# caesar-one/audio-classification-using-a-deep-cnn-combined-with-multi-level-attention

Measured on AMD Instinct MI355X. Metric: 0.96 s clips/sec wave->logits (VGGish+attn), higher is better.
Workload: dtype bf16; 1 GPU; BASELINE config 3: wave->logits forward, 1024 bags x 10 s 16 kHz PCM per GPU = 10240 x 0.96 s clips per step, VGGish + MLA [2,1], random-init portable-seeded weights; f32 front-end/head, bf16 conv+FC; bags_per_gpu=1024, parallelism=dp1 (no collective: independent bags)

## Files before the change

### audio-classification-using-a-deep-cnn-combined-with-multi-level-attention_amd/_lib.py

```python

import ctypes
import os
import re

HERE = os.path.dirname(os.path.abspath(__file__))
LIB_PATH = os.environ.get("MLA_HIP_LIB") or os.path.join(HERE, "libmla_hip.so")
HEADER = os.path.join(os.path.dirname(HERE), "include", "mla_hip.h")

F32, BF16, I16, BF16X3, F64, I32, U8, I24 = 0, 1, 2, 3, 4, 5, 6, 7
E_SHORT = -3

_lib = None


class MlaError(RuntimeError):
    def __init__(self, code, msg):
        super().__init__("libmla_hip error %d: %s" % (code, msg))
        self.code = code


def declared_symbols():
    text = open(HEADER).read()
    text = re.sub(r"/\*.*?\*/", "", text, flags=re.S)
    return sorted(set(re.findall(r"\b(mla_[a-z0-9_]+)\s*\(", text)))


def lib():
    global _lib
    if _lib is None:
        if not os.path.exists(LIB_PATH):
            raise RuntimeError(
                "%s is missing: build it with `python __graft_entry__.py` (hipcc --offload-arch=gfx950). "
                "There is no fallback path." % LIB_PATH)
        import torch
        L = ctypes.CDLL(LIB_PATH)
        L.mla_last_error.restype = ctypes.c_char_p
        L.mla_logmel_table_floats.restype = ctypes.c_int64
        i64, vp, ci = ctypes.c_int64, ctypes.c_void_p, ctypes.c_int
        L.mla_logmel_counts.argtypes = [i64, ctypes.POINTER(i64), ctypes.POINTER(i64)]
        L.mla_logmel_build_tables.argtypes = [vp]
        L.mla_logmel_reference_tables.argtypes = [vp, vp]
        L.mla_logmel_examples.argtypes = [vp, ci, i64, i64, i64, vp, vp, ci, vp]
        L.mla_logmel_conv1.argtypes = [vp, ci, i64, i64, i64, vp, vp, vp, vp, vp]
        L.mla_logmel_bags.argtypes = [vp, ci, i64, i64, i64, vp, vp, ci, ci, vp, vp, ci, vp]
        L.mla_timeline_counts.argtypes = [i64, i64, ctypes.POINTER(i64), ctypes.POINTER(i64), ctypes.POINTER(i64)]
        L.mla_logmel_timeline.argtypes = [vp, ci, i64, i64, i64, vp, vp, i64, vp, vp, ci, vp]
        L.mla_gather_bags.argtypes = [vp, i64, i64, vp, vp, i64, ci, i64, vp, vp]
        cf = ctypes.c_float
        L.mla_stft_magnitude.argtypes = [vp, i64, vp, vp, i64, i64, i64, vp, vp]
        L.mla_mel_log.argtypes = [vp, vp, i64, i64, i64, cf, vp, vp]
        L.mla_dataset_frames.argtypes = [vp, i64, ci, ci, ci, ci, vp, vp]
        L.mla_melspec_frames.restype = i64
        L.mla_melspec_frames.argtypes = [i64, i64]
        L.mla_melspec_table_floats.restype = i64
        L.mla_melspec_table_floats.argtypes = [ctypes.c_double, i64]
        L.mla_melspec_build_tables.argtypes = [ctypes.c_double, i64, vp]
        L.mla_melspec_workspace_bytes.restype = i64
        L.mla_melspec_workspace_bytes.argtypes = [i64, i64, i64]
        L.mla_melspec_db.argtypes = [vp, i64, i64, i64, i64, i64, cf, vp, vp, vp, vp]
        L.mla_melspec_images.argtypes = [vp, vp, i64, i64, i64, i64, cf, i64, i64, i64, vp, vp]
        L.mla_melspec_track_counts.argtypes = [i64, i64] + [ctypes.POINTER(i64)] * 4
        L.mla_melspec_track_db.argtypes = [vp, i64, i64, i64, vp, vp, i64, cf, vp, vp, vp, vp, vp]
        L.mla_melspec_track_images.argtypes = [vp, vp, i64, vp, vp, i64, cf, i64, i64, vp, vp]
        cd = ctypes.c_double
        L.mla_melspec_band_table_floats.restype = i64
        L.mla_melspec_band_table_floats.argtypes = [cd, i64, cd, cd, ci]
        L.mla_melspec_build_band_tables.argtypes = [cd, i64, cd, cd, ci, vp]
        L.mla_melspec_nopad_frames.restype = i64
        L.mla_melspec_nopad_frames.argtypes = [i64, i64]
        L.mla_melspec_nopad_workspace_bytes.restype = i64
        L.mla_melspec_nopad_workspace_bytes.argtypes = [i64, i64, i64]
        L.mla_melspec_nopad_db.argtypes = [vp, i64, i64, i64, i64, i64, cf, vp, i64, vp, vp, vp]
        L.mla_melspec_nopad_bags.argtypes = [vp, vp, i64, i64, i64, i64, cf, i64, i64, i64, vp, ci, vp]
        L.mla_postprocess.argtypes = [vp, vp, vp, i64, vp, vp]
        L.mla_mono_mix.argtypes = [vp, ci, i64, ci, vp, vp]
        L.mla_split_bf16x3.argtypes = [vp, i64, i64, i64, vp, i64, i64, ci, vp]
        L.mla_merge_bf16x3.argtypes = [vp, i64, i64, i64, i64, vp, vp]
        L.mla_linear_bf16x3.argtypes = [vp, i64, vp, i64, vp, vp, i64, i64, i64, i64, i64, ci, ci, vp]
        L.mla_conv_repack_weights.argtypes = [vp, i64, i64, vp, ci, vp]
        L.mla_convert_f32.argtypes = [vp, vp, i64, ci, vp]
        L.mla_convert_bf16_to_f32.argtypes = [vp, vp, i64, vp]
        L.mla_vggish_conv1.argtypes = [vp, ci, i64, vp, vp, vp, ci, vp]
        L.mla_vggish_conv.argtypes = [ci, vp, vp, vp, vp, i64, ci, vp]
        L.mla_linear.argtypes = [vp, i64, vp, i64, vp, vp, i64, i64, i64, i64, ci, ci, ci, vp]
        L.mla_linear_small.argtypes = [vp, i64, vp, i64, vp, vp, i64, i64, i64, i64, vp]
        L.mla_linear_narrow.argtypes = [vp, i64, vp, i64, vp, vp, i64, i64, i64, i64, vp]
        L.mla_linear_splitk.argtypes = [vp, i64, vp, i64, vp, vp, i64, i64, i64, i64, ci, ci, vp, i64, vp]
        L.mla_linear_ksplit.argtypes = [vp, i64, vp, i64, vp, vp, i64, i64, i64, i64, ci, ci, ci, ci, vp, i64, vp]
        L.mla_bn_stats_workspace_bytes.restype = i64
        L.mla_bn_stats.argtypes = [vp, i64, i64, i64, ci, ci, vp, vp, vp, vp, vp, cf, vp]
        L.mla_bn_apply.argtypes = [vp, i64, vp, i64, i64, i64, ci, ci, vp, vp, vp, vp, cf, ci, vp, cf, vp]
        L.mla_attention_pool.argtypes = [vp, i64, ci, ci, vp, vp, vp, vp, vp, vp, vp, vp, cf, vp, i64, vp, vp, vp]
        cd = ctypes.c_double
        L.mla_bn_stats_sums.argtypes = [vp, i64, i64, i64, ci, ci, vp, vp, vp]
        L.mla_bn_stats_finish.argtypes = [vp, ci, cd, vp, vp, vp, vp, cf, vp, vp]
        L.mla_bn_stats_fused.argtypes = [vp, i64, i64, i64, ci, ci, vp, vp, vp, vp, vp, vp, cf, vp, vp]
        L.mla_bn_bwd_sums.argtypes = [vp, i64, vp, i64, vp, i64, ci, cf, i64, i64, ci, ci, vp, vp, cf, vp, vp, vp]
        L.mla_bn_bwd_apply.argtypes = [vp, i64, vp, i64, vp, i64, ci, cf, i64, i64, ci, ci, vp, vp, vp, cf, vp, vp, cd,
                                       vp, i64, ci, vp, vp, vp]
        L.mla_bn_bwd_sums_wide.argtypes = [vp, i64, vp, i64, vp, i64, ci, cf, i64, i64, vp, vp, cf, vp, vp, vp]
        L.mla_bn_bwd_apply_wide.argtypes = [vp, i64, vp, i64, vp, i64, ci, cf, i64, i64, vp, vp, vp, cf, vp, vp, cd,
                                            vp, i64, ci, vp, vp, vp]
        L.mla_attention_pool_bwd.argtypes = [vp, i64, vp, vp, i64, ci, ci, vp, vp, vp]
        L.mla_linear_small_bwd.argtypes = [vp, i64, vp, i64, vp, i64, i64, i64, i64, vp, i64, vp, vp, vp]
        L.mla_transpose_f32.argtypes = [vp, i64, vp, i64, i64, i64, vp]
        L.mla_col_sum.argtypes = [vp, i64, i64, i64, vp, vp, vp]
        L.mla_axpy.argtypes = [cf, vp, vp, i64, vp]
        L.mla_cross_entropy.argtypes = [vp, i64, vp, i64, ci, cf, vp, vp, i64, vp, vp]
        L.mla_adam_step.argtypes = [vp, vp, vp, vp, i64, cf, cf, cf, cf, i64, vp]
        L.mla_conv3x3.argtypes = [vp, vp, vp, vp, i64, ci, ci, ci, ci, ci, ci, ci, vp]
        L.mla_conv3x3_train.argtypes = [vp, vp, vp, vp, vp, i64, ci, ci, ci, ci, ci, vp]
        L.mla_conv_repack_dgrad.argtypes = [vp, i64, i64, vp, vp]
        L.mla_maxpool2x2.argtypes = [vp, vp, i64, ci, ci, ci, vp]
        L.mla_relu_pool_bwd.argtypes = [vp, vp, vp, i64, ci, ci, ci, ci, vp]
        L.mla_relu_pool_bwd_bias.argtypes = [vp, vp, vp, i64, ci, ci, ci, ci, vp, vp, vp]
        L.mla_relu_pool_bwd_bias_workspace_bytes.restype = ctypes.c_int64
        L.mla_conv_wgrad_workspace_floats.restype = i64
        L.mla_conv_wgrad.argtypes = [vp, vp, i64, ci, ci, ci, ci, vp, i64, vp, vp]
        L.mla_conv1_bwd.argtypes = [vp, vp, vp, vp, i64, vp, vp, vp, vp]
        L.mla_conv_repack_dgrad_bf16.argtypes = [vp, i64, i64, vp, vp]
        L.mla_maxpool2x2_bf16.argtypes = [vp, vp, i64, ci, ci, ci, vp]
        L.mla_relu_pool_bwd_bf16_workspace_bytes.restype = i64
        L.mla_relu_pool_bwd_bf16.argtypes = [vp, ci, vp, ci, vp, i64, ci, ci, ci, ci, vp, vp, vp]
        L.mla_conv_wgrad_bf16.argtypes = [vp, vp, i64, ci, ci, ci, ci, vp, i64, vp, vp]
        L.mla_conv1_bwd_bf16.argtypes = [vp, vp, vp, vp, i64, vp, vp, vp, vp]
        L.mla_conv3x3_train_codes.argtypes = [vp, vp, vp, vp, vp, i64, ci, ci, ci, ci, ci, vp]
        L.mla_pool_bwd_codes_bf16.argtypes = [vp, vp, vp, i64, ci, ci, ci, vp, vp, vp]
        L.mla_conv1_bwd_workspace_floats.argtypes = []
        L.mla_conv1_bwd_workspace_floats.restype = i64
        L.mla_conv1_dgrad.argtypes = [vp, vp, vp, vp, ci, i64, vp, vp]
        L.mla_transpose_bf16.argtypes = [vp, i64, vp, i64, i64, i64, vp]
        L.mla_col_sum_bf16.argtypes = [vp, i64, i64, i64, vp, vp, vp]
        L.mla_resample_length.restype = i64
        L.mla_resample_length.argtypes = [i64, cd, cd]
        L.mla_resample.argtypes = [vp, i64, cd, cd, vp, vp, ci, ci, vp, i64, vp]
        L.mla_clips_lds_bytes.restype = i64
        L.mla_clips_lds_bytes.argtypes = [vp, i64, cd, ci, ci]
        L.mla_clips_prepare.argtypes = [vp, ci, i64, i64, vp, vp, vp, vp, vp, vp, vp, vp, vp, vp, cd, i64, vp, i64, ci, ci, vp, vp]
        L.mla_clips_prepare_raw.argtypes = [vp, i64, i64, vp, vp, vp, vp, vp, vp, vp, vp, vp, vp, vp, vp, cd, i64, vp, i64, ci, ci, vp, vp]
        u64 = ctypes.c_uint64
        L.mla_dropout_mask.argtypes = [vp, i64, u64, u64, u64, cf, vp]
        L.mla_dropout_mask_dev.argtypes = [vp, i64, u64, u64, vp, u64, cf, vp]
        L.mla_adam_step_dev.argtypes = [vp, vp, vp, vp, i64, cf, cf, cf, vp, vp]
        L.mla_adam_prepare.argtypes = [vp, cf, cf, cf, i64, vp]
        L.mla_counter_add.argtypes = [vp, i64, vp]
        L.mla_comm_unique_id.argtypes = [vp]
        L.mla_comm_init_rank.argtypes = [ctypes.POINTER(vp), ci, vp, ci]
        L.mla_comm_destroy.argtypes = [vp]
        L.mla_comm_count.argtypes = [vp, ctypes.POINTER(ci)]
        L.mla_comm_library_origin.restype = ctypes.c_char_p
        L.mla_allreduce_flat.argtypes = [vp, i64, ci, vp, vp]
        L.mla_rn_repack.argtypes = [vp, i64, i64, i64, vp, ci, vp]
        L.mla_rn_stem.argtypes = [vp, i64, i64, i64, ci, vp, vp, vp, ci, vp, ci, vp]
        L.mla_rn_conv.argtypes = [vp, i64, i64, i64, i64, vp, i64, i64, i64, vp, vp, vp, ci, vp, ci, vp]
        L.mla_rn_bn_workspace_bytes.restype = i64
        L.mla_rn_bn_workspace_bytes.argtypes = [i64]
        L.mla_rn_bn_stats.argtypes = [vp, i64, i64, ci, vp, vp, vp, cf, cf, vp, vp, vp, vp, vp, vp, vp]
        L.mla_rn_bn_sums.argtypes = [vp, i64, i64, ci, vp, vp, vp]
        L.mla_rn_bn_finish.argtypes = [vp, i64, vp, vp, cf, cf, vp, vp, vp, vp, vp, vp, vp]
        L.mla_rn_bn_eval_coeffs.argtypes = [vp, vp, vp, vp, cf, i64, vp, vp, vp]
        L.mla_rn_bn_apply.argtypes = [vp, i64, i64, vp, vp, vp, ci, vp, ci, vp]
        L.mla_rn_maxpool.argtypes = [vp, i64, i64, i64, i64, vp, ci, vp]
        L.mla_rn_avgpool.argtypes = [vp, i64, i64, i64, vp, ci, vp]
        L.mla_rn_repack_dgrad.argtypes = [vp, i64, i64, i64, vp, ci, vp]
        L.mla_rn_conv_dgrad.argtypes = [vp, i64, i64, i64, i64, vp, i64, i64, i64, i64, i64, vp, vp, ci, vp]
        L.mla_rn_conv_wgrad_workspace_floats.restype = i64
        L.mla_rn_conv_wgrad_workspace_floats.argtypes = [i64, i64, i64, i64, i64, i64, ci]
        L.mla_rn_conv_wgrad.argtypes = [vp, vp, i64, i64, i64, i64, i64, i64, i64, vp, i64, vp, ci, vp]
        L.mla_rn_stem_wgrad_workspace_floats.restype = i64
        L.mla_rn_stem_wgrad_workspace_floats.argtypes = [i64]
        L.mla_rn_stem_wgrad.argtypes = [vp, i64, ci, vp, vp, i64, vp, ci, vp]
        L.mla_rn_bn_bwd_workspace_bytes.restype = i64
        L.mla_rn_bn_bwd_workspace_bytes.argtypes = [i64]
        L.mla_rn_bn_bwd.argtypes = [vp, vp, vp, i64, i64, vp, vp, vp, cf, vp, vp, vp, vp, vp, ci, vp]
        L.mla_rn_bn_bwd_sums.argtypes = [vp, vp, vp, i64, i64, vp, vp, cf, vp, vp, vp, vp, ci, vp]
        L.mla_rn_bn_bwd_apply.argtypes = [vp, vp, vp, i64, i64, vp, vp, vp, cf, vp, vp, vp, vp, ci, vp]
        L.mla_rn_maxpool_bwd.argtypes = [vp, vp, i64, i64, i64, i64, vp, ci, vp]
        L.mla_rn_avgpool_bwd.argtypes = [vp, i64, i64, i64, vp, ci, vp]
        L.mla_rn_act_bwd.argtypes = [vp, vp, vp, i64, i64, vp, vp, ci, vp]
        L.mla_rn_stem_dgrad.argtypes = [vp, i64, vp, vp, vp, ci, vp, ci, vp]
        _lib = L
    return _lib


def check(rc):
    if rc != 0:
        raise MlaError(rc, lib().mla_last_error().decode("utf-8", "replace"))


def stream_ptr():
    import torch
    return ctypes.c_void_p(torch.cuda.current_stream().cuda_stream)
```

### audio-classification-using-a-deep-cnn-combined-with-multi-level-attention_amd/csrc/gemm.hip

```cpp
#include <type_traits>

#include "common.h"
#include "mma_core.h"

namespace {

using namespace mma;

constexpr int kThreads = 512;

#ifndef MLA_GEMM_STAMPS
#define MLA_GEMM_STAMPS 0
#endif
#if MLA_GEMM_STAMPS
__device__ unsigned long long g_gemm_stamps[8][2][8];
#define MLA_GSTAMP(k) do { if (stamp_on) stamps[k] = __builtin_amdgcn_s_memtime(); } while (0)
#else
#define MLA_GSTAMP(k) do { } while (0)
#endif
#ifndef MLA_GEMM_PRIO
#define MLA_GEMM_PRIO 3
#endif
#ifndef MLA_GEMM_STAGGER
#define MLA_GEMM_STAGGER 1
#endif

#ifndef MLA_GEMM_TILE320
#define MLA_GEMM_TILE320 1
#endif
#ifndef MLA_GEMM_RING
#define MLA_GEMM_RING 1
#endif
#ifdef MLA_GEMM_KWRAP
#define MLA_GEMM_KW(s) ((s) & (MLA_GEMM_KWRAP - 1))
#else
#define MLA_GEMM_KW(s) (s)
#endif
template <typename T, typename TO, int MS, int NS, bool RELU, bool DMA = false>
__global__ __launch_bounds__(kThreads, 2) void gemm_kernel(const T* __restrict__ A, int64_t lda,
                                                            const T* __restrict__ W, int64_t ldw,
                                                            const float* __restrict__ bias, TO* __restrict__ out,
                                                            int64_t ldo, int M, int N, int K, float* __restrict__ partial,
                                                            int seg, int osplit) {
    constexpr int PER = Elem<T>::kPerChunk, KC = Elem<T>::kPerRow;
    constexpr int kMS = MS, kBM = 2 * MS * 16;
    constexpr int BN = 4 * NS * 16;
    constexpr int A_BYTES = kBM * kRowBytes, B_BYTES = BN * kRowBytes;
    constexpr int AP = kBM * 8 / kThreads;
    extern __shared__ __attribute__((aligned(16))) char smem[];
    char* sA = smem;
    char* sB = smem + 2 * A_BYTES;

    const int t = threadIdx.x, lane = t & 63, wave = t >> 6, wm = wave >> 2, wn = wave & 3;
    const int r = lane & 15, q = lane >> 4;
    const int m0 = blockIdx.x * kBM, n0 = blockIdx.y * BN;
    const int abase = tile_off(wm * kMS * 16 + r, q);
    const int bbase = tile_off(wn * NS * 16 + r, q);

    f32x4 acc[kMS][NS];
    _Pragma("unroll") for (int i = 0; i < kMS; ++i)
        _Pragma("unroll") for (int j = 0; j < NS; ++j) acc[i][j] = f32x4{0.f, 0.f, 0.f, 0.f};

    constexpr uint32_t ESZ = sizeof(T);
    const int a_rows = M - m0 < kBM ? M - m0 : kBM, w_rows = N - n0 < BN ? N - n0 : BN;
    const __amdgpu_buffer_rsrc_t ra = __builtin_amdgcn_make_buffer_rsrc(const_cast<T*>(A) + size_t(m0) * lda, 0,
                                                                          uint32_t(a_rows) * uint32_t(lda) * ESZ, 0x00020000);
    const __amdgpu_buffer_rsrc_t rw = __builtin_amdgcn_make_buffer_rsrc(const_cast<T*>(W) + size_t(n0) * ldw, 0,
                                                                          uint32_t(w_rows) * uint32_t(ldw) * ESZ, 0x00020000);
    u32x4 areg[AP], breg[NS];
    auto gload = [&](int s) {
        int sa = s;
        if (seg) {
            const int blk = s / (3 * seg), rr = s - blk * 3 * seg;
            sa = blk * 2 * seg + (rr < seg ? rr : rr - seg);
        }
        _Pragma("unroll") for (int p = 0; p < AP; ++p) {
            const int piece = t + kThreads * p, row = piece >> 3, ch = piece & 7;
            const int k = sa * KC + ch * PER;
            const bool ok = m0 + row < M && s * KC + ch * PER < K;
            areg[p] = __builtin_amdgcn_raw_buffer_load_b128(ra, ok ? int((uint32_t(row) * uint32_t(lda) + k) * sizeof(T)) : int(0x7fffff00), 0, 0);
        }
        _Pragma("unroll") for (int p = 0; p < NS; ++p) {
            const int piece = t + kThreads * p, n = piece >> 3, ch = piece & 7;
            const int k = s * KC + ch * PER;
            const bool ok = n0 + n < N && k < K;
            breg[p] = __builtin_amdgcn_raw_buffer_load_b128(rw, ok ? int((uint32_t(n) * uint32_t(ldw) + k) * sizeof(T)) : int(0x7fffff00), 0, 0);
        }
    };
    auto lwrite = [&](int buf) {
        _Pragma("unroll") for (int p = 0; p < AP; ++p) {
            const int piece = t + kThreads * p;
            lds_write16(sA, buf * A_BYTES + tile_off(piece >> 3, piece & 7), areg[p]);
        }
        _Pragma("unroll") for (int p = 0; p < NS; ++p) {
            const int piece = t + kThreads * p;
            lds_write16(sB, buf * B_BYTES + tile_off(piece >> 3, piece & 7), breg[p]);
        }
    };

    auto dma = [&](int s, int buf) {
        int sa = s;
        if (seg) {
            const int blk = s / (3 * seg), rr = s - blk * 3 * seg;
            sa = blk * 2 * seg + (rr < seg ? rr : rr - seg);
        }
        const int slot = lane & 7;
        _Pragma("unroll") for (int p = 0; p < kBM / 64; ++p) {
            const int row = 8 * (wave + 8 * p) + (lane >> 3);
            const int chunk = slot ^ (((row >> 1) & 3) << 1);
            __builtin_amdgcn_raw_ptr_buffer_load_lds(ra, (__attribute__((address_space(3))) void*)(sA + buf * A_BYTES + 8 * (wave + 8 * p) * kRowBytes),
                                                     16, int((uint32_t(row) * uint32_t(lda) + chunk * PER) * ESZ), int(MLA_GEMM_KW(sa) * KC * ESZ), 0, 0);
        }
        _Pragma("unroll") for (int p = 0; p < BN / 64; ++p) {
            const int row = 8 * (wave + 8 * p) + (lane >> 3);
            const int chunk = slot ^ (((row >> 1) & 3) << 1);
            __builtin_amdgcn_raw_ptr_buffer_load_lds(rw, (__attribute__((address_space(3))) void*)(sB + buf * B_BYTES + 8 * (wave + 8 * p) * kRowBytes),
                                                     16, int((uint32_t(row) * uint32_t(ldw) + chunk * PER) * ESZ), int(MLA_GEMM_KW(s) * KC * ESZ), 0, 0);
        }
    };

    const int all_stages = (K + KC - 1) / KC;
    const int per_split = (all_stages + int(gridDim.z) - 1) / int(gridDim.z);
    const int s_begin = int(blockIdx.z) * per_split;
    const int stages = (s_begin + per_split < all_stages ? s_begin + per_split : all_stages);
    if (DMA) {
        dma(s_begin, s_begin & 1);
        asm volatile("s_waitcnt vmcnt(0)" ::: "memory");
    } else {
        gload(s_begin);
        lwrite(s_begin & 1);
    }
    __syncthreads();
    constexpr bool STAGGER = DMA && MLA_GEMM_STAGGER;
    const bool late = STAGGER && __builtin_amdgcn_readfirstlane(wave) >= 4;
    if (STAGGER && late) __builtin_amdgcn_s_setprio(1);
#if MLA_GEMM_STAMPS
    unsigned long long stamps[8] = {0, 0, 0, 0, 0, 0, 0, 0};
#endif
    auto run = [&](auto late_c) {
        constexpr bool LATE = decltype(late_c)::value;
        u32x4 af[kMS], bf[NS];
        for (int s = s_begin; s < stages; ++s) {
            const int buf = s & 1;
#if MLA_GEMM_STAMPS
            const bool stamp_on = s == 100 && (wave == 0 || wave == 4) && blockIdx.x < 8 && blockIdx.y == 0 && kMS == 8;
#endif
            auto stage_next = [&]() {
                if (s + 1 < stages) {
                    if (DMA) dma(s + 1, buf ^ 1);
                    else gload(s + 1);
                }
            };
            auto rd = [&](int ks) {
                _Pragma("unroll") for (int i = 0; i < kMS; ++i)
                    af[i] = lds_read16(sA, buf * A_BYTES + (abase ^ (ks << 6)) + i * 16 * kRowBytes);
                _Pragma("unroll") for (int j = 0; j < NS; ++j)
                    bf[j] = lds_read16(sB, buf * B_BYTES + (bbase ^ (ks << 6)) + j * 16 * kRowBytes);
            };
            auto mm = [&]() {
                __builtin_amdgcn_sched_barrier(0);
                _Pragma("unroll") for (int i = 0; i < kMS; ++i)
                    _Pragma("unroll") for (int j = 0; j < NS; ++j) mma_step<T>(af[i], bf[j], acc[i][j]);
                __builtin_amdgcn_sched_barrier(0);
            };
            if constexpr (!LATE) {
                if (STAGGER && MLA_GEMM_PRIO == 3) __builtin_amdgcn_s_setprio(2);
                MLA_GSTAMP(0);
                rd(0);
                MLA_GSTAMP(1);
                stage_next();
                MLA_GSTAMP(2);
                mm();
                MLA_GSTAMP(3);
                if (STAGGER && MLA_GEMM_PRIO == 3) __builtin_amdgcn_s_setprio(0);
                rd(1);
                MLA_GSTAMP(4);
                mm();
                MLA_GSTAMP(5);
            } else {
                if (MLA_GEMM_PRIO == 3) __builtin_amdgcn_s_setprio(3);
                MLA_GSTAMP(0);
                if (s > s_begin) mm();
                MLA_GSTAMP(1);
                stage_next();
                MLA_GSTAMP(2);
                if (MLA_GEMM_PRIO == 3) __builtin_amdgcn_s_setprio(1);
                rd(0); mm();
                MLA_GSTAMP(3);
                rd(1);
                MLA_GSTAMP(4);
                asm volatile("s_waitcnt lgkmcnt(0)" ::: "memory");
                MLA_GSTAMP(5);
            }
            if (!DMA && s + 1 < stages) lwrite(buf ^ 1);
            if (DMA) asm volatile("s_waitcnt vmcnt(0)" ::: "memory");
            MLA_GSTAMP(6);
            __syncthreads();
            MLA_GSTAMP(7);
        }
        if constexpr (LATE) {
            if (stages > s_begin) {
                __builtin_amdgcn_sched_barrier(0);
                _Pragma("unroll") for (int i = 0; i < kMS; ++i)
                    _Pragma("unroll") for (int j = 0; j < NS; ++j) mma_step<T>(af[i], bf[j], acc[i][j]);
                __builtin_amdgcn_sched_barrier(0);
            }
        }
    };
    if constexpr (STAGGER) {
        if (late) run(std::true_type{});
        else run(std::false_type{});
    } else {
        run(std::false_type{});
    }

#if MLA_GEMM_STAMPS
    if ((wave == 0 || wave == 4) && lane == 0 && blockIdx.x < 8 && blockIdx.y == 0 && kMS == 8 && stages > 100)
        for (int k = 0; k < 8; ++k) g_gemm_stamps[blockIdx.x][wave >> 2][k] = stamps[k];
#endif
    if (partial) {
        float* pout = partial + size_t(blockIdx.z) * M * N;
        _Pragma("unroll") for (int j = 0; j < NS; ++j) {
            const int n = n0 + (wn * NS + j) * 16 + r;
            if (n >= N) continue;
            _Pragma("unroll") for (int i = 0; i < kMS; ++i) {
                const float v[4] = {acc[i][j].x, acc[i][j].y, acc[i][j].z, acc[i][j].w};
                _Pragma("unroll") for (int e = 0; e < 4; ++e) {
                    const int m = m0 + (wm * kMS + i) * 16 + 4 * q + e;
                    if (m < M) pout[size_t(m) * N + n] = v[e];
                }
            }
        }
        return;
    }
    _Pragma("unroll") for (int j = 0; j < NS; ++j) {
        const int n = n0 + (wn * NS + j) * 16 + r;
        if (n >= N) continue;
        const float b = bias ? bias[n] : 0.f;
        _Pragma("unroll") for (int i = 0; i < kMS; ++i) {
            const float v[4] = {acc[i][j].x, acc[i][j].y, acc[i][j].z, acc[i][j].w};
            _Pragma("unroll") for (int e = 0; e < 4; ++e) {
                const int m = m0 + (wm * kMS + i) * 16 + 4 * q + e;
                if (m < M) {
                    float y = v[e] + b;
                    if (RELU) y = mla::nan_relu(y);
                    if (sizeof(TO) == 2 && osplit) {
                        const float hi = bf2f(f2bf(y));
                        store_elem<TO>(out + size_t(m) * ldo + n, hi);
                        store_elem<TO>(out + size_t(m) * ldo + N + n, y - hi);
                    } else {
                        store_elem<TO>(out + size_t(m) * ldo + n, y);
                    }
                }
            }
        }
    }
}

template <typename T, typename TO, bool RELU>
__global__ __launch_bounds__(kThreads, 2) void gemm_ring_kernel(const T* __restrict__ A, int64_t lda, const T* __restrict__ W,
                                                                 int64_t ldw, const float* __restrict__ bias, TO* __restrict__ out,
                                                                 int64_t ldo, int M, int N, int K, float* __restrict__ partial, int seg,
                                                                 int osplit) {
    constexpr int PER = Elem<T>::kPerChunk, KC = Elem<T>::kPerRow;
    constexpr int kMS = 4, NS = 2, kBM = 128, BN = 128, RING = 4;
    constexpr int A_BYTES = kBM * kRowBytes, B_BYTES = BN * kRowBytes, STAGE_BYTES = A_BYTES + B_BYTES;
    extern __shared__ __attribute__((aligned(16))) char smem[];

    const int t = threadIdx.x, lane = t & 63, wave = t >> 6, wm = wave >> 2, wn = wave & 3;
    const int r = lane & 15, q = lane >> 4;
    int bx = blockIdx.x, by = blockIdx.y;
    if (gridDim.y % 8 == 0) {
        const int id = blockIdx.x + gridDim.x * blockIdx.y, per = gridDim.y / 8, j = id >> 3;
        by = (id & 7) * per + j % per;
        bx = j / per;
    }
    const int m0 = bx * kBM, n0 = by * BN;
    const int abase = tile_off(wm * kMS * 16 + r, q);
    const int bbase = tile_off(wn * NS * 16 + r, q);

    f32x4 acc[kMS][NS];
    _Pragma("unroll") for (int i = 0; i < kMS; ++i)
        _Pragma("unroll") for (int j = 0; j < NS; ++j) acc[i][j] = f32x4{0.f, 0.f, 0.f, 0.f};

    constexpr uint32_t ESZ = sizeof(T);
    const int a_rows = M - m0 < kBM ? M - m0 : kBM, w_rows = N - n0 < BN ? N - n0 : BN;
    const __amdgpu_buffer_rsrc_t ra = __builtin_amdgcn_make_buffer_rsrc(const_cast<T*>(A) + size_t(m0) * lda, 0,
                                                                          uint32_t(a_rows) * uint32_t(lda) * ESZ, 0x00020000);
    const __amdgpu_buffer_rsrc_t rw = __builtin_amdgcn_make_buffer_rsrc(const_cast<T*>(W) + size_t(n0) * ldw, 0,
                                                                          uint32_t(w_rows) * uint32_t(ldw) * ESZ, 0x00020000);
    auto dma = [&](int s, int buf) {
        int sa = s;
        if (seg) {
            const int blk = s / (3 * seg), rr = s - blk * 3 * seg;
            sa = blk * 2 * seg + (rr < seg ? rr : rr - seg);
        }
        char* sA = smem + buf * STAGE_BYTES;
        char* sB = sA + A_BYTES;
        const int slot = lane & 7;
        _Pragma("unroll") for (int p = 0; p < 2; ++p) {
            const int row = 8 * (wave + 8 * p) + (lane >> 3);
            const int chunk = slot ^ (((row >> 1) & 3) << 1);
            __builtin_amdgcn_raw_ptr_buffer_load_lds(ra, (__attribute__((address_space(3))) void*)(sA + 8 * (wave + 8 * p) * kRowBytes), 16,
                                                     int((uint32_t(row) * uint32_t(lda) + chunk * PER) * ESZ), int(sa * KC * ESZ), 0, 0);
        }
        _Pragma("unroll") for (int p = 0; p < 2; ++p) {
            const int row = 8 * (wave + 8 * p) + (lane >> 3);
            const int chunk = slot ^ (((row >> 1) & 3) << 1);
            __builtin_amdgcn_raw_ptr_buffer_load_lds(rw, (__attribute__((address_space(3))) void*)(sB + 8 * (wave + 8 * p) * kRowBytes), 16,
                                                     int((uint32_t(row) * uint32_t(ldw) + chunk * PER) * ESZ), int(s * KC * ESZ), 0, 0);
        }
    };

    const int all_stages = K / KC;
    const int per_split = (all_stages + int(gridDim.z) - 1) / int(gridDim.z);
    const int s_begin = int(blockIdx.z) * per_split;
    const int s_end = s_begin + per_split < all_stages ? s_begin + per_split : all_stages;
    _Pragma("unroll") for (int p = 0; p < RING - 1; ++p)
        if (s_begin + p < s_end) dma(s_begin + p, p);
    for (int s = s_begin; s < s_end; ++s) {
        const int left = s_end - 1 - s;
        if (left >= 2) asm volatile("s_waitcnt vmcnt(8)" ::: "memory");
        else if (left == 1) asm volatile("s_waitcnt vmcnt(4)" ::: "memory");
        else asm volatile("s_waitcnt vmcnt(0)" ::: "memory");
        __syncthreads();
        if (s + RING - 1 < s_end) dma(s + RING - 1, (s - s_begin + RING - 1) % RING);
        const char* sA = smem + ((s - s_begin) % RING) * STAGE_BYTES;
        const char* sB = sA + A_BYTES;
        _Pragma("unroll") for (int ks = 0; ks < 2; ++ks) {
            u32x4 af[kMS], bf[NS];
            _Pragma("unroll") for (int i = 0; i < kMS; ++i) af[i] = lds_read16(sA, (abase ^ (ks << 6)) + i * 16 * kRowBytes);
            _Pragma("unroll") for (int j = 0; j < NS; ++j) bf[j] = lds_read16(sB, (bbase ^ (ks << 6)) + j * 16 * kRowBytes);
            _Pragma("unroll") for (int i = 0; i < kMS; ++i)
                _Pragma("unroll") for (int j = 0; j < NS; ++j) mma_step<T>(af[i], bf[j], acc[i][j]);
        }
    }

    if (partial) {
        float* pout = partial + size_t(blockIdx.z) * M * N;
        _Pragma("unroll") for (int j = 0; j < NS; ++j) {
            const int n = n0 + (wn * NS + j) * 16 + r;
            if (n >= N) continue;
            _Pragma("unroll") for (int i = 0; i < kMS; ++i) {
                const float v[4] = {acc[i][j].x, acc[i][j].y, acc[i][j].z, acc[i][j].w};
                _Pragma("unroll") for (int e = 0; e < 4; ++e) {
                    const int m = m0 + (wm * kMS + i) * 16 + 4 * q + e;
                    if (m < M) pout[size_t(m) * N + n] = v[e];
                }
            }
        }
        return;
    }
    _Pragma("unroll") for (int j = 0; j < NS; ++j) {
        const int n = n0 + (wn * NS + j) * 16 + r;
        if (n >= N) continue;
        const float b = bias ? bias[n] : 0.f;
        _Pragma("unroll") for (int i = 0; i < kMS; ++i) {
            const float v[4] = {acc[i][j].x, acc[i][j].y, acc[i][j].z, acc[i][j].w};
            _Pragma("unroll") for (int e = 0; e < 4; ++e) {
                const int m = m0 + (wm * kMS + i) * 16 + 4 * q + e;
                if (m < M) {
                    float y = v[e] + b;
                    if (RELU) y = mla::nan_relu(y);
                    if (sizeof(TO) == 2 && osplit) {
                        const float hi = bf2f(f2bf(y));
                        store_elem<TO>(out + size_t(m) * ldo + n, hi);
                        store_elem<TO>(out + size_t(m) * ldo + N + n, y - hi);
                    } else {
                        store_elem<TO>(out + size_t(m) * ldo + n, y);
                    }
                }
            }
        }
    }
}

template <typename TO>
__global__ __launch_bounds__(256) void splitk_reduce_kernel(const float* __restrict__ partial, int splits, int64_t M, int N,
                                                            const float* __restrict__ bias, int relu, TO* __restrict__ out, int64_t ldo) {
    const int64_t total = M * N;
    for (int64_t i = int64_t(blockIdx.x) * 256 + threadIdx.x; i < total; i += int64_t(gridDim.x) * 256) {
        const int64_t m = i / N;
        const int n = int(i - m * N);
        float v = bias ? bias[n] : 0.f;
        for (int k = 0; k < splits; ++k) v += partial[size_t(k) * total + i];
        if (relu) v = mla::nan_relu(v);
        store_elem<TO>(out + m * ldo + n, v);
    }
}

template <typename T, typename TO, int MS, int NS, bool RELU>
int launch(const void* a, int64_t lda, const void* w, int64_t ldw, const float* bias, void* out, int64_t ldo,
           int64_t M, int64_t N, int64_t K, hipStream_t s, int splits = 1, float* partial = nullptr, int seg = 0, int osplit = 0) {
    constexpr int kBM = 2 * MS * 16, BN = 4 * NS * 16;
    constexpr int lds = 2 * (kBM + BN) * kRowBytes;
    constexpr int KCE = mma::Elem<T>::kPerRow;
    MLA_REQUIRE(uint64_t(kBM) * uint64_t(lda) * sizeof(T) < (1ull << 31) && uint64_t(BN) * uint64_t(ldw) * sizeof(T) < (1ull << 31), MLA_E_SHAPE,
                "GEMM row pitch too large for 32-bit buffer offsets (lda %lld, ldw %lld)", (long long)lda, (long long)ldw);
    const bool use_dma = K % KCE == 0;
    auto kern = use_dma ? gemm_kernel<T, TO, MS, NS, RELU, true> : gemm_kernel<T, TO, MS, NS, RELU, false>;
    MLA_HIP_OK(hipFuncSetAttribute(reinterpret_cast<const void*>(kern), hipFuncAttributeMaxDynamicSharedMemorySize, lds));
    const dim3 grid{unsigned((M + kBM - 1) / kBM), unsigned((N + BN - 1) / BN), unsigned(splits)};
    hipLaunchKernelGGL(kern, grid, dim3(kThreads), lds, s, static_cast<const T*>(a), lda, static_cast<const T*>(w), ldw,
                       bias, static_cast<TO*>(out), ldo, int(M), int(N), int(K), splits > 1 ? partial : nullptr, seg, osplit);
    MLA_LAUNCH_OK("gemm_kernel");
    if (splits > 1) {
        const int64_t total = M * N;
        hipLaunchKernelGGL(splitk_reduce_kernel<TO>, dim3(unsigned((total + 255) / 256 < 4096 ? (total + 255) / 256 : 4096)), dim3(256),
                           0, s, partial, splits, M, int(N), bias, int(RELU), static_cast<TO*>(out), ldo);
        MLA_LAUNCH_OK("splitk_reduce_kernel");
    }
    return MLA_OK;
}

template <typename T, typename TO, bool RELU>
int launch_ring(const void* a, int64_t lda, const void* w, int64_t ldw, const float* bias, void* out, int64_t ldo,
                int64_t M, int64_t N, int64_t K, hipStream_t s, int splits = 1, float* partial = nullptr, int seg = 0, int osplit = 0) {
    constexpr int lds = 4 * (128 + 128) * kRowBytes;
    MLA_REQUIRE(uint64_t(128) * uint64_t(lda) * sizeof(T) < (1ull << 31) && uint64_t(128) * uint64_t(ldw) * sizeof(T) < (1ull << 31), MLA_E_SHAPE,
                "GEMM row pitch too large for 32-bit buffer offsets (lda %lld, ldw %lld)", (long long)lda, (long long)ldw);
    MLA_REQUIRE(K % mma::Elem<T>::kPerRow == 0, MLA_E_SHAPE, "the ring GEMM stages whole %d-element K chunks", mma::Elem<T>::kPerRow);
    auto kern = gemm_ring_kernel<T, TO, RELU>;
    MLA_HIP_OK(hipFuncSetAttribute(reinterpret_cast<const void*>(kern), hipFuncAttributeMaxDynamicSharedMemorySize, lds));
    const dim3 grid{unsigned((M + 127) / 128), unsigned((N + 127) / 128), unsigned(splits)};
    hipLaunchKernelGGL(kern, grid, dim3(kThreads), lds, s, static_cast<const T*>(a), lda, static_cast<const T*>(w), ldw, bias,
                       static_cast<TO*>(out), ldo, int(M), int(N), int(K), splits > 1 ? partial : nullptr, seg, osplit);
    MLA_LAUNCH_OK("gemm_ring_kernel");
    if (splits > 1) {
        const int64_t total = M * N;
        hipLaunchKernelGGL(splitk_reduce_kernel<TO>, dim3(unsigned((total + 255) / 256 < 4096 ? (total + 255) / 256 : 4096)), dim3(256),
                           0, s, partial, splits, M, int(N), bias, int(RELU), static_cast<TO*>(out), ldo);
        MLA_LAUNCH_OK("splitk_reduce_kernel");
    }
    return MLA_OK;
}

template <typename Fn>
int by_relu(bool relu, Fn&& fn) {
    return relu ? fn(std::true_type{}) : fn(std::false_type{});
}

enum class Tile { k64x128, k128x128, kRing, k128x256, k256x256, k320x256 };

template <typename T>
Tile tile_form(int64_t M, int64_t N, int64_t K, int cus, int64_t& m_tall) {
    m_tall = M;
    const bool wide = N > 128 && (N % 256 == 0 || N % 256 > 128);
    const bool tall = wide && M >= 4096 && N >= 1024;
#if MLA_GEMM_TILE320
    if (tall && K % mma::Elem<T>::kPerRow == 0) {
        const int64_t n_tiles = (N + 255) / 256;
        const int64_t t256 = ((M + 255) / 256) * n_tiles, t320 = ((M + 319) / 320) * n_tiles;
        const int64_t full = t256 / cus, rest = t256 - full * cus;
        const double cost256 = 64.0 * double(full) + (rest == 0 ? 0.0 : (full >= 1 && 2 * rest <= cus && (full * cus) % n_tiles == 0 ? 48.0 : 64.0));
        const double cost320 = 72.0 * double((t320 + cus - 1) / cus);
        if (cost320 < cost256) return Tile::k320x256;
    }
#endif
    if (tall) {
        const int64_t n_tiles = (N + 255) / 256, m_tiles = (M + 255) / 256;
        const int64_t full_rounds = m_tiles * n_tiles / cus, rest = m_tiles * n_tiles - full_rounds * cus;
        if (full_rounds >= 1 && rest > 0 && 2 * rest <= cus && (full_rounds * cus) % n_tiles == 0) m_tall = full_rounds * cus / n_tiles * 256;
        return Tile::k256x256;
    }
    if (wide) {
        if (((M + 127) / 128) * ((N + 255) / 256) * 2 <= cus) {
#if MLA_GEMM_RING
            if (K % mma::Elem<T>::kPerRow == 0 && K / mma::Elem<T>::kPerRow >= 8)
                return Tile::kRing;
#endif
            return Tile::k128x128;
        }
        return Tile::k128x256;
    }
    if (((M + 127) / 128) * ((N + 127) / 128) < cus && M > 64)
        return Tile::k64x128;
    return Tile::k128x128;
}

template <typename T, typename TO>
int dispatch(const void* a, int64_t lda, const void* w, int64_t ldw, const float* bias, void* out, int64_t ldo,
             int64_t M, int64_t N, int64_t K, bool relu, hipStream_t s, int seg = 0, int osplit = 0) {
    int64_t m_tall;
    const Tile form = tile_form<T>(M, N, K, mla::cu_count(), m_tall);
    return by_relu(relu, [&](auto r) {
        constexpr bool R = decltype(r)::value;
        switch (form) {
            case Tile::k64x128: return launch<T, TO, 2, 2, R>(a, lda, w, ldw, bias, out, ldo, M, N, K, s, 1, nullptr, seg, osplit);
            case Tile::k128x128: return launch<T, TO, 4, 2, R>(a, lda, w, ldw, bias, out, ldo, M, N, K, s, 1, nullptr, seg, osplit);
#if MLA_GEMM_RING
            case Tile::kRing: return launch_ring<T, TO, R>(a, lda, w, ldw, bias, out, ldo, M, N, K, s, 1, nullptr, seg, osplit);
#endif
            case Tile::k128x256: return launch<T, TO, 4, 4, R>(a, lda, w, ldw, bias, out, ldo, M, N, K, s, 1, nullptr, seg, osplit);
#if MLA_GEMM_TILE320
            case Tile::k320x256: return launch<T, TO, 10, 4, R>(a, lda, w, ldw, bias, out, ldo, M, N, K, s, 1, nullptr, seg, osplit);
#endif
            default: break;
        }
        const int rc = launch<T, TO, 8, 4, R>(a, lda, w, ldw, bias, out, ldo, m_tall, N, K, s, 1, nullptr, seg, osplit);
        if (rc != MLA_OK || m_tall == M) return rc;
        const T* a2 = static_cast<const T*>(a) + m_tall * lda;
        TO* out2 = static_cast<TO*>(out) + m_tall * ldo;
        return launch<T, TO, 4, 4, R>(a2, lda, w, ldw, bias, out2, ldo, M - m_tall, N, K, s, 1, nullptr, seg, osplit);
    });
}

}

#if MLA_GEMM_STAMPS
extern "C" int mla_debug_gemm_stamps(unsigned long long* host_out) {
    return hipMemcpyFromSymbol(host_out, HIP_SYMBOL(g_gemm_stamps), sizeof(g_gemm_stamps)) == hipSuccess ? 0 : -4;
}
#endif

extern "C" int mla_linear_splitk(const float* a, int64_t lda, const float* w, int64_t ldw, const float* bias, float* out,
                                 int64_t ldo, int64_t M, int64_t N, int64_t K, int relu, int splits, float* workspace,
                                 int64_t workspace_floats, mla_stream_t stream) {
    MLA_REQUIRE(a && w && out && workspace && M > 0 && N > 0 && K > 0 && splits >= 1 && splits <= 64, MLA_E_ARG, "bad split-K GEMM arguments");
    MLA_REQUIRE(K % 4 == 0 && lda % 4 == 0 && ldw % 4 == 0 && lda >= K && ldw >= K && ldo >= N, MLA_E_SHAPE, "split-K GEMM: 16-byte rows required");
    MLA_REQUIRE(mla::aligned(a, 16) && mla::aligned(w, 16), MLA_E_ARG, "GEMM operands must be 16-byte aligned");
    MLA_REQUIRE(workspace_floats >= int64_t(splits) * M * N, MLA_E_ARG, "split-K workspace too small");
    hipStream_t s = static_cast<hipStream_t>(stream);
    return by_relu(relu != 0, [&](auto r) {
        return launch<float, float, 4, 2, decltype(r)::value>(a, lda, w, ldw, bias, out, ldo, M, N, K, s, splits, workspace);
    });
}

extern "C" int mla_linear_ksplit(const void* a, int64_t lda, const void* w, int64_t ldw, const float* bias, void* out, int64_t ldo,
                                 int64_t M, int64_t N, int64_t K, int dtype, int out_dtype, int relu, int splits, float* workspace,
                                 int64_t workspace_floats, mla_stream_t stream) {
    MLA_REQUIRE(M >= 0 && N > 0 && K > 0 && splits >= 1 && splits <= 64, MLA_E_ARG, "bad K-split GEMM arguments");
    if (M == 0) return MLA_OK;
    MLA_REQUIRE(a && w && out && workspace, MLA_E_ARG, "null GEMM operand");
    MLA_REQUIRE(dtype == MLA_F32 || dtype == MLA_BF16, MLA_E_DTYPE, "GEMM dtype %d", dtype);
    MLA_REQUIRE(out_dtype == MLA_F32 || (out_dtype == MLA_BF16 && dtype == MLA_BF16), MLA_E_DTYPE, "GEMM out dtype %d for compute dtype %d", out_dtype, dtype);
    const int kc = dtype == MLA_F32 ? 32 : 64;
    MLA_REQUIRE(K % (int64_t(kc) * splits) == 0 && lda % (kc / 8) == 0 && ldw % (kc / 8) == 0 && lda >= K && ldw >= K && ldo >= N, MLA_E_SHAPE,
                "K-split GEMM: K %lld must be a multiple of %d x splits %d (whole stages per range)", (long long)K, kc, splits);
    MLA_REQUIRE(mla::aligned(a, 16) && mla::aligned(w, 16), MLA_E_ARG, "GEMM operands must be 16-byte aligned");
    MLA_REQUIRE(workspace_floats >= int64_t(splits) * M * N, MLA_E_ARG, "K-split workspace too small");
    MLA_REQUIRE(M < (1ll << 31) && N < (1ll << 31) && K < (1ll << 31), MLA_E_SHAPE, "GEMM dimension overflow");
    hipStream_t s = static_cast<hipStream_t>(stream);
    const bool r = relu != 0;
    if (dtype == MLA_F32)
        return r ? launch<float, float, 4, 2, true>(a, lda, w, ldw, bias, out, ldo, M, N, K, s, splits, workspace)
                 : launch<float, float, 4, 2, false>(a, lda, w, ldw, bias, out, ldo, M, N, K, s, splits, workspace);
    if (out_dtype == MLA_F32)
        return r ? launch<mma::bf16_t, float, 4, 2, true>(a, lda, w, ldw, bias, out, ldo, M, N, K, s, splits, workspace)
                 : launch<mma::bf16_t, float, 4, 2, false>(a, lda, w, ldw, bias, out, ldo, M, N, K, s, splits, workspace);
    return r ? launch<mma::bf16_t, mma::bf16_t, 4, 2, true>(a, lda, w, ldw, bias, out, ldo, M, N, K, s, splits, workspace)
             : launch<mma::bf16_t, mma::bf16_t, 4, 2, false>(a, lda, w, ldw, bias, out, ldo, M, N, K, s, splits, workspace);
}

extern "C" int mla_linear(const void* a, int64_t lda, const void* w, int64_t ldw, const float* bias, void* out,
                          int64_t ldo, int64_t M, int64_t N, int64_t K, int dtype, int out_dtype, int relu,
                          mla_stream_t stream) {
    MLA_REQUIRE(M >= 0 && N > 0 && K > 0, MLA_E_ARG, "bad GEMM shape %lld x %lld x %lld", (long long)M, (long long)N, (long long)K);
    if (M == 0) return MLA_OK;
    MLA_REQUIRE(a && w && out, MLA_E_ARG, "null GEMM operand");
    MLA_REQUIRE(dtype == MLA_F32 || dtype == MLA_BF16, MLA_E_DTYPE, "GEMM dtype %d", dtype);
    MLA_REQUIRE(out_dtype == MLA_F32 || (out_dtype == MLA_BF16 && dtype == MLA_BF16), MLA_E_DTYPE,
                "GEMM out dtype %d for compute dtype %d", out_dtype, dtype);
    const int per = dtype == MLA_F32 ? 4 : 8;
    MLA_REQUIRE(K % per == 0 && lda % per == 0 && ldw % per == 0 && lda >= K && ldw >= K && ldo >= N, MLA_E_SHAPE,
                "K / lda / ldw must be multiples of %d elements (16-byte rows): K %lld lda %lld ldw %lld ldo %lld", per,
                (long long)K, (long long)lda, (long long)ldw, (long long)ldo);
    MLA_REQUIRE(mla::aligned(a, 16) && mla::aligned(w, 16), MLA_E_ARG, "GEMM operands must be 16-byte aligned");
    MLA_REQUIRE(M < (1ll << 31) && N < (1ll << 31) && K < (1ll << 31), MLA_E_SHAPE, "GEMM dimension overflow");
    hipStream_t s = static_cast<hipStream_t>(stream);
    if (dtype == MLA_F32) return dispatch<float, float>(a, lda, w, ldw, bias, out, ldo, M, N, K, relu != 0, s);
    if (out_dtype == MLA_F32) return dispatch<mma::bf16_t, float>(a, lda, w, ldw, bias, out, ldo, M, N, K, relu != 0, s);
    return dispatch<mma::bf16_t, mma::bf16_t>(a, lda, w, ldw, bias, out, ldo, M, N, K, relu != 0, s);
}

extern "C" int mla_linear_bf16x3(const void* a, int64_t lda, const void* w, int64_t ldw, const float* bias, void* out,
                                 int64_t ldo, int64_t M, int64_t N, int64_t K, int64_t seg, int out_dtype, int relu,
                                 mla_stream_t stream) {
    MLA_REQUIRE(M >= 0 && N > 0 && K > 0, MLA_E_ARG, "bad GEMM shape %lld x %lld x %lld", (long long)M, (long long)N, (long long)K);
    if (M == 0) return MLA_OK;
    MLA_REQUIRE(a && w && out, MLA_E_ARG, "null GEMM operand");
    MLA_REQUIRE(out_dtype == MLA_F32 || out_dtype == MLA_BF16X3, MLA_E_DTYPE, "split GEMM out dtype %d", out_dtype);
    MLA_REQUIRE(seg > 0 && seg % 64 == 0 && K % seg == 0 && lda >= 2 * K && ldw >= 3 * K && lda % 8 == 0 && ldw % 8 == 0 &&
                ldo >= (out_dtype == MLA_F32 ? N : 2 * N), MLA_E_SHAPE,
                "split GEMM: seg %lld must be a multiple of 64 dividing K %lld; lda %lld >= 2K, ldw %lld >= 3K", (long long)seg,
                (long long)K, (long long)lda, (long long)ldw);
    MLA_REQUIRE(mla::aligned(a, 16) && mla::aligned(w, 16), MLA_E_ARG, "GEMM operands must be 16-byte aligned");
    MLA_REQUIRE(M < (1ll << 31) && N < (1ll << 31) && 3 * K < (1ll << 31), MLA_E_SHAPE, "GEMM dimension overflow");
    hipStream_t s = static_cast<hipStream_t>(stream);
    if (out_dtype == MLA_F32)
        return dispatch<mma::bf16_t, float>(a, lda, w, ldw, bias, out, ldo, M, N, 3 * K, relu != 0, s, int(seg / 64), 0);
    return dispatch<mma::bf16_t, mma::bf16_t>(a, lda, w, ldw, bias, out, ldo, M, N, 3 * K, relu != 0, s, int(seg / 64), 1);
}
```

### audio-classification-using-a-deep-cnn-combined-with-multi-level-attention_amd/csrc/mla_head.hip

```cpp
#include "common.h"

namespace {

constexpr int kStatBlocks = 512;
constexpr int kMaxChannels = 64;
constexpr int kMaxWideChannels = 1024;
constexpr int kWideRowBlocks = 32;
constexpr int kMaxSlots = 64;
constexpr int kMaxClasses = 1024;

__device__ __forceinline__ double wave_sum(double v) {
    _Pragma("unroll") for (int o = 32; o > 0; o >>= 1) v += __shfl_xor(v, o);
    return v;
}

__device__ __forceinline__ float sigmoidf(float v) { return 1.f / (1.f + __expf(-v)); }

__device__ __forceinline__ float grad_through_act(float dy, float yout, int act, float drop_scale) {
    if (act == 1) return yout > 0.f ? dy * drop_scale : 0.f;
    if (act == 2) return dy * yout * (1.f - yout);
    return dy;
}

typedef float f32x4_t __attribute__((ext_vector_type(4)));

struct StatsOp {
    const float* x; int64_t ldx;
    __device__ __forceinline__ void operator()(int64_t r, int c, int, double& a, double& b) const {
        const double v = x[r * ldx + c];
        a = v; b = v * v;
    }
    __device__ __forceinline__ void quad(int64_t r, int c, int, double& a, double& b) const {
        const f32x4_t v = *reinterpret_cast<const f32x4_t*>(x + r * ldx + c);
        _Pragma("unroll") for (int e = 0; e < 4; ++e) { const double d = v[e]; a += d; b += d * d; }
    }
    __device__ __forceinline__ bool vec_ok(int cols) const { return cols % 4 == 0 && ldx % 4 == 0 && (reinterpret_cast<uintptr_t>(x) & 15) == 0; }
};

struct BwdOp {
    const float *x, *dy, *yout, *mean, *var;
    int64_t ldx, ld_dy, ld_y;
    int act;
    float drop_scale, eps;
    __device__ __forceinline__ void operator()(int64_t r, int c, int ch, double& a, double& b) const {
        const float g = grad_through_act(dy[r * ld_dy + c], yout ? yout[r * ld_y + c] : 0.f, act, drop_scale);
        const float xhat = (x[r * ldx + c] - mean[ch]) * (1.0f / sqrtf(var[ch] + eps));
        a = g; b = double(g) * xhat;
    }
    __device__ __forceinline__ void quad(int64_t r, int c, int ch, double& a, double& b) const {
        const f32x4_t d = *reinterpret_cast<const f32x4_t*>(dy + r * ld_dy + c);
        const f32x4_t xv = *reinterpret_cast<const f32x4_t*>(x + r * ldx + c);
        f32x4_t y = f32x4_t{0.f, 0.f, 0.f, 0.f};
        if (yout) y = *reinterpret_cast<const f32x4_t*>(yout + r * ld_y + c);
        const float m = mean[ch], inv = 1.0f / sqrtf(var[ch] + eps);
        _Pragma("unroll") for (int e = 0; e < 4; ++e) {
            const float g = grad_through_act(d[e], y[e], act, drop_scale);
            const float xhat = (xv[e] - m) * inv;
            a += g; b += double(g) * xhat;
        }
    }
    __device__ __forceinline__ bool vec_ok(int cols) const {
        return cols % 4 == 0 && ldx % 4 == 0 && ld_dy % 4 == 0 && (!yout || ld_y % 4 == 0) && (reinterpret_cast<uintptr_t>(x) & 15) == 0 &&
               (reinterpret_cast<uintptr_t>(dy) & 15) == 0 && (reinterpret_cast<uintptr_t>(yout) & 15) == 0;
    }
};

template <typename Op>
__global__ __launch_bounds__(256) void sums_rows_kernel(Op op, int64_t rows, int cols, int period, double* __restrict__ partial) {
    __shared__ double part[4][kMaxChannels][2];
    const int wave = threadIdx.x >> 6, lane = threadIdx.x & 63;
    const bool vec = op.vec_ok(cols);
    for (int i = threadIdx.x; i < 4 * kMaxChannels * 2; i += 256) (&part[0][0][0])[i] = 0.0;
    __syncthreads();
    const int64_t per_block = ((rows + gridDim.x - 1) / gridDim.x + period - 1) / period * period;
    const int64_t r0 = int64_t(blockIdx.x) * per_block;
    const int64_t r1 = r0 + per_block < rows ? r0 + per_block : rows;
    for (int64_t r = r0 + wave; r < r1; r += 4) {
        const int chan = int(r % period);
        double s = 0.0, ss = 0.0;
        if (vec) {
            for (int c = 4 * lane; c < cols; c += 256) op.quad(r, c, chan, s, ss);
        } else {
            for (int c = lane; c < cols; c += 64) {
                double a, b;
                op(r, c, chan, a, b);
                s += a;
                ss += b;
            }
        }
        s = wave_sum(s);
        ss = wave_sum(ss);
        if (lane == 0) {
            part[wave][chan][0] += s;
            part[wave][chan][1] += ss;
        }
    }
    __syncthreads();
    if (threadIdx.x < period) {
        double s = 0.0, ss = 0.0;
        for (int w = 0; w < 4; ++w) { s += part[w][threadIdx.x][0]; ss += part[w][threadIdx.x][1]; }
        partial[(int64_t(blockIdx.x) * period + threadIdx.x) * 2] = s;
        partial[(int64_t(blockIdx.x) * period + threadIdx.x) * 2 + 1] = ss;
    }
}

template <typename Op>
__global__ __launch_bounds__(256) void sums_cols_kernel(Op op, int64_t rows, int cols, double* __restrict__ partial) {
    __shared__ double part[256][2];
    const int groups = 256 / cols, g = threadIdx.x / cols, c = threadIdx.x % cols;
    double s = 0.0, ss = 0.0;
    if (g < groups) {
        const int64_t per_block = (rows + gridDim.x - 1) / gridDim.x;
        const int64_t r0 = int64_t(blockIdx.x) * per_block;
        const int64_t r1 = r0 + per_block < rows ? r0 + per_block : rows;
        for (int64_t r = r0 + g; r < r1; r += groups) {
            double a, b;
            op(r, c, c, a, b);
            s += a;
            ss += b;
        }
    }
    part[threadIdx.x][0] = s;
    part[threadIdx.x][1] = ss;
    __syncthreads();
    if (threadIdx.x < cols) {
        double a = 0.0, b = 0.0;
        for (int gg = 0; gg < groups; ++gg) { a += part[gg * cols + threadIdx.x][0]; b += part[gg * cols + threadIdx.x][1]; }
        partial[(int64_t(blockIdx.x) * cols + threadIdx.x) * 2] = a;
        partial[(int64_t(blockIdx.x) * cols + threadIdx.x) * 2 + 1] = b;
    }
}

template <typename Op>
__global__ __launch_bounds__(256) void sums_cols_wide_kernel(Op op, int64_t rows, int cols, double* __restrict__ partial) {
    __shared__ double part[4][64][2];
    const int g = threadIdx.x >> 6, lane = threadIdx.x & 63;
    const int c = int(blockIdx.x) * 64 + lane;
    double s = 0.0, ss = 0.0;
    if (c < cols) {
        const int64_t per_block = (rows + gridDim.y - 1) / gridDim.y;
        const int64_t r0 = int64_t(blockIdx.y) * per_block;
        const int64_t r1 = r0 + per_block < rows ? r0 + per_block : rows;
        for (int64_t r = r0 + g; r < r1; r += 4) {
            double a, b;
            op(r, c, c, a, b);
            s += a;
            ss += b;
        }
    }
    part[g][lane][0] = s;
    part[g][lane][1] = ss;
    __syncthreads();
    if (g == 0 && c < cols) {
        double a = 0.0, b = 0.0;
        for (int gg = 0; gg < 4; ++gg) { a += part[gg][lane][0]; b += part[gg][lane][1]; }
        partial[(int64_t(blockIdx.y) * cols + c) * 2] = a;
        partial[(int64_t(blockIdx.y) * cols + c) * 2 + 1] = b;
    }
}

__global__ __launch_bounds__(64) void partial_reduce_kernel(const double* __restrict__ partial, int blocks, int channels,
                                                            double* __restrict__ sums) {
    const int c = blockIdx.x, lane = threadIdx.x;
    double s = 0.0, ss = 0.0;
    for (int b = lane; b < blocks; b += 64) { s += partial[(int64_t(b) * channels + c) * 2]; ss += partial[(int64_t(b) * channels + c) * 2 + 1]; }
    s = wave_sum(s);
    ss = wave_sum(ss);
    if (lane == 0) { sums[2 * c] = s; sums[2 * c + 1] = ss; }
}

struct FinishArgs {
    double count; float* mean; float* var; float* run_mean; float* run_var; float momentum; int64_t* tracked;
};
__global__ __launch_bounds__(1024) void reduce_finish_kernel(const double* __restrict__ partial, int blocks, int channels,
                                                             double* __restrict__ sums, FinishArgs f) {
    const int c = threadIdx.x >> 6, lane = threadIdx.x & 63;
    if (threadIdx.x == 0 && f.tracked) *f.tracked += 1;
    if (c >= channels) return;
    double s = 0.0, ss = 0.0;
    for (int b = lane; b < blocks; b += 64) { s += partial[(int64_t(b) * channels + c) * 2]; ss += partial[(int64_t(b) * channels + c) * 2 + 1]; }
    s = wave_sum(s);
    ss = wave_sum(ss);
    if (lane != 0) return;
    sums[2 * c] = s;
    sums[2 * c + 1] = ss;
    const double m = s / f.count;
    double v = ss / f.count - m * m;
    if (v < 0.0) v = 0.0;
    f.mean[c] = float(m);
    f.var[c] = float(v);
    if (f.run_mean && f.momentum >= 0.f) {
        const double unbiased = f.count > 1.0 ? v * f.count / (f.count - 1.0) : v;
        f.run_mean[c] = float((1.0 - f.momentum) * f.run_mean[c] + f.momentum * m);
        f.run_var[c] = float((1.0 - f.momentum) * f.run_var[c] + f.momentum * unbiased);
    }
}

template <typename Op>
int channel_sums(Op op, int64_t rows, int64_t cols, int mode, int period, void* workspace, double* sums, hipStream_t s,
                 const FinishArgs* finish = nullptr) {
    double* partial = static_cast<double*>(workspace);
    const int channels = mode == 0 ? period : int(cols);
    int blocks;
    if (mode == 0) {
        const int64_t groups = rows / period;
        blocks = int(groups < kStatBlocks ? groups : kStatBlocks);
        hipLaunchKernelGGL(sums_rows_kernel<Op>, dim3(blocks), dim3(256), 0, s, op, rows, int(cols), period, partial);
    } else if (cols <= kMaxChannels) {
        blocks = int((rows + 63) / 64 < kStatBlocks ? (rows + 63) / 64 : kStatBlocks);
        hipLaunchKernelGGL(sums_cols_kernel<Op>, dim3(blocks), dim3(256), 0, s, op, rows, int(cols), partial);
    } else {
        blocks = int((rows + 63) / 64 < kWideRowBlocks ? (rows + 63) / 64 : kWideRowBlocks);
        hipLaunchKernelGGL(sums_cols_wide_kernel<Op>, dim3(unsigned((cols + 63) / 64), blocks), dim3(256), 0, s, op, rows, int(cols), partial);
    }
    MLA_LAUNCH_OK("channel sums");
    if (finish && channels <= 16) {
        hipLaunchKernelGGL(reduce_finish_kernel, dim3(1), dim3(64 * channels), 0, s, partial, blocks, channels, sums, *finish);
        MLA_LAUNCH_OK("channel sums reduce + finish");
        return 1;
    }
    hipLaunchKernelGGL(partial_reduce_kernel, dim3(channels), dim3(64), 0, s, partial, blocks, channels, sums);
    MLA_LAUNCH_OK("channel sums reduce");
    return MLA_OK;
}

__global__ void stats_finish_kernel(const double* __restrict__ sums, int channels, double count, float* __restrict__ mean,
                                    float* __restrict__ var, float* __restrict__ run_mean, float* __restrict__ run_var,
                                    float momentum, int64_t* __restrict__ num_batches_tracked) {
    const int c = threadIdx.x;
    if (c == 0 && num_batches_tracked) *num_batches_tracked += 1;
    if (c >= channels) return;
    const double m = sums[2 * c] / count;
    double v = sums[2 * c + 1] / count - m * m;
    if (v < 0.0) v = 0.0;
    mean[c] = float(m);
    var[c] = float(v);
    if (run_mean && momentum >= 0.f) {
        const double unbiased = count > 1.0 ? v * count / (count - 1.0) : v;
        run_mean[c] = float((1.0 - momentum) * run_mean[c] + momentum * m);
        run_var[c] = float((1.0 - momentum) * run_var[c] + momentum * unbiased);
    }
}

template <int MODE>
__global__ __launch_bounds__(256) void bn_apply_kernel(const float* __restrict__ x, int64_t ldx, float* __restrict__ y,
                                                       int64_t ldy, int64_t rows, int cols, int period,
                                                       const float* __restrict__ mean, const float* __restrict__ var,
                                                       const float* __restrict__ gamma, const float* __restrict__ beta,
                                                       float eps, int act, const uint8_t* __restrict__ keep,
                                                       float drop_scale) {
    const int64_t total = rows * cols;
    for (int64_t i = int64_t(blockIdx.x) * 256 + threadIdx.x; i < total; i += int64_t(gridDim.x) * 256) {
        const int64_t r = i / cols;
        const int c = int(i - r * cols);
        const int ch = MODE == 0 ? int(r % period) : c;
        const float inv = 1.0f / sqrtf(var[ch] + eps);
        float v = (x[r * ldx + c] - mean[ch]) * inv * gamma[ch] + beta[ch];
        if (act == 1) v = mla::nan_relu(v);
        else if (act == 2) v = sigmoidf(v);
        if (keep) v *= keep[i] ? drop_scale : 0.f;
        y[r * ldy + c] = v;
    }
}

template <int MODE>
__global__ __launch_bounds__(256) void bn_bwd_apply_kernel(BwdOp op, const float* __restrict__ gamma, int64_t rows, int cols,
                                                           int period, const double* __restrict__ sums_global,
                                                           const double* __restrict__ sums_local, double count,
                                                           float* __restrict__ dx, int64_t ld_dx, int accumulate,
                                                           float* __restrict__ dgamma, float* __restrict__ dbeta) {
    const int channels = MODE == 0 ? period : cols;
    if (blockIdx.x == 0 && dgamma) {
        for (int ch = threadIdx.x; ch < channels; ch += 256) {
            dbeta[ch] = float(sums_local[2 * ch]);
            dgamma[ch] = float(sums_local[2 * ch + 1]);
        }
    }
    if (!dx) return;
    const int64_t total = rows * cols;
    for (int64_t i = int64_t(blockIdx.x) * 256 + threadIdx.x; i < total; i += int64_t(gridDim.x) * 256) {
        const int64_t r = i / cols;
        const int c = int(i - r * cols);
        const int ch = MODE == 0 ? int(r % period) : c;
        double g, gx;
        op(r, c, ch, g, gx);
        const float inv = 1.0f / sqrtf(op.var[ch] + op.eps);
        const float xhat = (op.x[r * op.ldx + c] - op.mean[ch]) * inv;
        const float sg = float(sums_global[2 * ch] / count), sgx = float(sums_global[2 * ch + 1] / count);
        const float v = gamma[ch] * inv * (float(g) - sg - xhat * sgx);
        float* o = dx + r * ld_dx + c;
        *o = accumulate ? *o + v : v;
    }
}

struct BnParams { const float *mean, *var, *gamma, *beta; };

template <int KMAX>
__global__ __launch_bounds__(256) void attention_pool_kernel(const float* __restrict__ z, int64_t bags, int T, int K,
                                                             BnParams nv, BnParams nf, float eps, float* __restrict__ y,
                                                             int64_t ldy, float* __restrict__ att_out,
                                                             float* __restrict__ cla_out) {
    const int t = threadIdx.x & 15;
    const int64_t bag = int64_t(blockIdx.x) * 16 + (threadIdx.x >> 4);
    const bool live = bag < bags && t < T;
    float att[KMAX], cla[KMAX];
    if (live) {
        const float* row = z + (bag * T + t) * K;
        const float iv = 1.0f / sqrtf(nv.var[t] + eps), jf = 1.0f / sqrtf(nf.var[t] + eps);
        float mx = -3.0e38f;
        _Pragma("unroll") for (int k = 0; k < KMAX; ++k)
            if (k < K) {
                const float v = row[k];
                att[k] = (v - nv.mean[t]) * iv * nv.gamma[t] + nv.beta[t];
                cla[k] = sigmoidf((v - nf.mean[t]) * jf * nf.gamma[t] + nf.beta[t]);
                mx = fmaxf(mx, att[k]);
            }
        float den = 0.f;
        _Pragma("unroll") for (int k = 0; k < KMAX; ++k)
            if (k < K) { att[k] = __expf(att[k] - mx); den += att[k]; }
        const float inv = 1.0f / den;
        _Pragma("unroll") for (int k = 0; k < KMAX; ++k)
            if (k < K) {
                att[k] *= inv;
                if (att_out) att_out[(bag * T + t) * K + k] = att[k];
                if (cla_out) cla_out[(bag * T + t) * K + k] = cla[k];
            }
    } else {
        _Pragma("unroll") for (int k = 0; k < KMAX; ++k) { att[k] = 0.f; cla[k] = 0.f; }
    }
    _Pragma("unroll") for (int k = 0; k < KMAX; ++k) {
        if (k < K) {
            float s = att[k];
            _Pragma("unroll") for (int o = 8; o > 0; o >>= 1) s += __shfl_xor(s, o, 16);
            float num = live ? cla[k] * (att[k] / s) : 0.f;
            _Pragma("unroll") for (int o = 8; o > 0; o >>= 1) num += __shfl_xor(num, o, 16);
            if (t == 0 && bag < bags) y[bag * ldy + k] = num;
        }
    }
}

template <int KMAX>
__global__ __launch_bounds__(256) void attention_pool_bwd_kernel(const float* __restrict__ dy, int64_t ld_dy,
                                                                 const float* __restrict__ att_in, const float* __restrict__ cla_in,
                                                                 int64_t bags, int T, int K, float* __restrict__ du_v,
                                                                 float* __restrict__ du_f) {
    const int t = threadIdx.x & 15;
    const int64_t bag = int64_t(blockIdx.x) * 16 + (threadIdx.x >> 4);
    const bool live = bag < bags && t < T;
    float att[KMAX], cla[KMAX], datt[KMAX];
    _Pragma("unroll") for (int k = 0; k < KMAX; ++k) {
        att[k] = (live && k < K) ? att_in[(bag * T + t) * K + k] : 0.f;
        cla[k] = (live && k < K) ? cla_in[(bag * T + t) * K + k] : 0.f;
    }
    float dot = 0.f;
    _Pragma("unroll") for (int k = 0; k < KMAX; ++k) {
        datt[k] = 0.f;
        if (k < K) {
            float s = att[k];
            _Pragma("unroll") for (int o = 8; o > 0; o >>= 1) s += __shfl_xor(s, o, 16);
            float yk = live ? cla[k] * (att[k] / s) : 0.f;
            _Pragma("unroll") for (int o = 8; o > 0; o >>= 1) yk += __shfl_xor(yk, o, 16);
            if (live) {
                const float g = dy[bag * ld_dy + k];
                const float dcla = g * (att[k] / s);
                datt[k] = g * (cla[k] - yk) / s;
                du_f[(bag * T + t) * K + k] = dcla * cla[k] * (1.f - cla[k]);
                dot += datt[k] * att[k];
            }
        }
    }
    if (live) {
        _Pragma("unroll") for (int k = 0; k < KMAX; ++k)
            if (k < K) du_v[(bag * T + t) * K + k] = att[k] * (datt[k] - dot);
    }
}

struct SlotCoef { float mean_v, scale_v, gamma_v, beta_v, mean_f, scale_f, gamma_f, beta_f; };

__device__ __forceinline__ float wave_max_f(float v) {
    _Pragma("unroll") for (int o = 32; o > 0; o >>= 1) v = fmaxf(v, __shfl_xor(v, o));
    return v;
}
__device__ __forceinline__ float wave_sum_f(float v) {
    _Pragma("unroll") for (int o = 32; o > 0; o >>= 1) v += __shfl_xor(v, o);
    return v;
}

__global__ __launch_bounds__(256) void attention_pool_wide_kernel(const float* __restrict__ z, int T, int K, BnParams nv, BnParams nf,
                                                                  float eps, float* __restrict__ y, int64_t ldy,
                                                                  float* __restrict__ att_out, float* __restrict__ cla_out) {
    __shared__ SlotCoef coef[kMaxSlots];
    __shared__ float row_max[kMaxSlots], row_inv[kMaxSlots];
    const int64_t bag = blockIdx.x;
    const int wave = threadIdx.x >> 6, lane = threadIdx.x & 63;
    const float* tile = z + bag * T * K;
    if (threadIdx.x < T) {
        const int t = threadIdx.x;
        coef[t] = SlotCoef{nv.mean[t], 1.0f / sqrtf(nv.var[t] + eps), nv.gamma[t], nv.beta[t],
                           nf.mean[t], 1.0f / sqrtf(nf.var[t] + eps), nf.gamma[t], nf.beta[t]};
    }
    __syncthreads();
    for (int t = wave; t < T; t += 4) {
        const SlotCoef c = coef[t];
        const float* row = tile + int64_t(t) * K;
        float mx = -3.0e38f;
        for (int k = lane; k < K; k += 64) mx = fmaxf(mx, (row[k] - c.mean_v) * c.scale_v * c.gamma_v + c.beta_v);
        mx = wave_max_f(mx);
        float den = 0.f;
        for (int k = lane; k < K; k += 64) den += __expf(((row[k] - c.mean_v) * c.scale_v * c.gamma_v + c.beta_v) - mx);
        den = wave_sum_f(den);
        if (lane == 0) { row_max[t] = mx; row_inv[t] = 1.0f / den; }
    }
    __syncthreads();
    for (int k = threadIdx.x; k < K; k += 256) {
        float S = 0.f, num = 0.f;
        for (int t = 0; t < T; ++t) {
            const SlotCoef c = coef[t];
            const float v = tile[int64_t(t) * K + k];
            const float att = __expf(((v - c.mean_v) * c.scale_v * c.gamma_v + c.beta_v) - row_max[t]) * row_inv[t];
            const float cla = sigmoidf((v - c.mean_f) * c.scale_f * c.gamma_f + c.beta_f);
            if (att_out) att_out[(bag * T + t) * K + k] = att;
            if (cla_out) cla_out[(bag * T + t) * K + k] = cla;
            S += att;
            num = fmaf(cla, att, num);
        }
        y[bag * ldy + k] = num / S;
    }
}

__global__ __launch_bounds__(256) void attention_pool_bwd_wide_kernel(const float* __restrict__ dy, int64_t ld_dy,
                                                                      const float* __restrict__ att_in, const float* __restrict__ cla_in,
                                                                      int T, int K, float* __restrict__ du_v, float* __restrict__ du_f) {
    __shared__ float col_inv[kMaxClasses], col_y[kMaxClasses];
    const int64_t bag = blockIdx.x;
    const int wave = threadIdx.x >> 6, lane = threadIdx.x & 63;
    const int64_t base = bag * T * K;
    for (int k = threadIdx.x; k < K; k += 256) {
        float S = 0.f, num = 0.f;
        for (int t = 0; t < T; ++t) {
            const float a = att_in[base + int64_t(t) * K + k];
            S += a;
            num = fmaf(cla_in[base + int64_t(t) * K + k], a, num);
        }
        col_inv[k] = 1.0f / S;
        col_y[k] = num / S;
    }
    __syncthreads();
    for (int t = wave; t < T; t += 4) {
        const int64_t row = base + int64_t(t) * K;
        float dot = 0.f;
        for (int k = lane; k < K; k += 64) {
            const float g = dy[bag * ld_dy + k], a = att_in[row + k], c = cla_in[row + k];
            du_f[row + k] = g * (a * col_inv[k]) * c * (1.f - c);
            dot = fmaf(g * (c - col_y[k]) * col_inv[k], a, dot);
        }
        dot = wave_sum_f(dot);
        for (int k = lane; k < K; k += 64) {
            const float g = dy[bag * ld_dy + k], a = att_in[row + k], c = cla_in[row + k];
            du_v[row + k] = a * (g * (c - col_y[k]) * col_inv[k] - dot);
        }
    }
}

__global__ __launch_bounds__(256) void linear_small_kernel(const float* __restrict__ a, int64_t lda,
                                                           const float* __restrict__ w, int64_t ldw,
                                                           const float* __restrict__ bias, float* __restrict__ out,
                                                           int64_t ldo, int64_t M, int N, int K) {
    const int64_t i = int64_t(blockIdx.x) * 256 + threadIdx.x;
    if (i >= M * N) return;
    const int64_t m = i / N;
    const int n = int(i - m * N);
    float acc = bias ? bias[n] : 0.f;
    for (int k = 0; k < K; ++k) acc = fmaf(a[m * lda + k], w[int64_t(n) * ldw + k], acc);
    out[m * ldo + n] = acc;
}

__global__ __launch_bounds__(256) void linear_small_wide_kernel(const float* __restrict__ a, int64_t lda, const float* __restrict__ w,
                                                                int64_t ldw, const float* __restrict__ bias, float* __restrict__ out,
                                                                int64_t ldo, int64_t M, int N, int K) {
    extern __shared__ float s_w[];
    for (int i = threadIdx.x; i < N * K; i += 256) {
        const int n = i / K, kk = i - n * K;
        s_w[kk * N + n] = w[int64_t(n) * ldw + kk];
    }
    __syncthreads();
    const int quads = N / 4;
    const int64_t total = M * quads;
    for (int64_t i = int64_t(blockIdx.x) * 256 + threadIdx.x; i < total; i += int64_t(gridDim.x) * 256) {
        const int64_t m = i / quads;
        const int n = int(i - m * quads) * 4;
        float acc[4];
        _Pragma("unroll") for (int e = 0; e < 4; ++e) acc[e] = bias ? bias[n + e] : 0.f;
        for (int kk = 0; kk < K; ++kk) {
            const float av = a[m * lda + kk];
            const f32x4_t wv = *reinterpret_cast<const f32x4_t*>(s_w + kk * N + n);
            _Pragma("unroll") for (int e = 0; e < 4; ++e) acc[e] = fmaf(av, wv[e], acc[e]);
        }
        *reinterpret_cast<f32x4_t*>(out + m * ldo + n) = f32x4_t{acc[0], acc[1], acc[2], acc[3]};
    }
}

typedef float f4 __attribute__((ext_vector_type(4)));

template <int N>
__global__ __launch_bounds__(256) void linear_narrow_kernel(const float* __restrict__ a, int64_t lda, const float* __restrict__ w,
                                                            int64_t ldw, const float* __restrict__ bias, float* __restrict__ out,
                                                            int64_t ldo, int64_t M, int K) {
    extern __shared__ __attribute__((aligned(16))) float sw[];
    const int k4 = K / 4;
    for (int i = threadIdx.x; i < k4 * N; i += 256) {
        const int n = i % N, kk = i / N;
        reinterpret_cast<f4*>(sw)[kk * N + n] = *reinterpret_cast<const f4*>(w + int64_t(n) * ldw + 4 * kk);
    }
    __syncthreads();
    const int l = threadIdx.x & 15, grp = threadIdx.x >> 4;
    for (int64_t m = int64_t(blockIdx.x) * 16 + grp; m < M; m += int64_t(gridDim.x) * 16) {
        float acc[N];
        _Pragma("unroll") for (int n = 0; n < N; ++n) acc[n] = 0.f;
        const f4* row = reinterpret_cast<const f4*>(a + m * lda);
        for (int kk = l; kk < k4; kk += 16) {
            const f4 x = row[kk];
            _Pragma("unroll") for (int n = 0; n < N; ++n) {
                const f4 ww = reinterpret_cast<const f4*>(sw)[kk * N + n];
                acc[n] = fmaf(x.x, ww.x, acc[n]);
                acc[n] = fmaf(x.y, ww.y, acc[n]);
                acc[n] = fmaf(x.z, ww.z, acc[n]);
                acc[n] = fmaf(x.w, ww.w, acc[n]);
            }
        }
        _Pragma("unroll") for (int n = 0; n < N; ++n) {
            float v = acc[n];
            v += __shfl_xor(v, 8, 16);
            v += __shfl_xor(v, 4, 16);
            v += __shfl_xor(v, 2, 16);
            v += __shfl_xor(v, 1, 16);
            acc[n] = v;
        }
        if (l < N) {
            float v = 0.f;
            _Pragma("unroll") for (int n = 0; n < N; ++n) v = l == n ? acc[n] : v;
            out[m * ldo + l] = v + (bias ? bias[l] : 0.f);
        }
    }
}

__global__ __launch_bounds__(256) void linear_small_bwd_kernel(const float* __restrict__ a, int64_t lda,
                                                               const float* __restrict__ w, int64_t ldw,
                                                               const float* __restrict__ dz, int64_t ldz, int64_t M, int N, int K,
                                                               float* __restrict__ da, int64_t ldda, float* __restrict__ dw,
                                                               float* __restrict__ db) {
    const int64_t i = int64_t(blockIdx.x) * 256 + threadIdx.x;
    if (i < M * K) {
        const int64_t m = i / K;
        const int k = int(i - m * K);
        float acc = 0.f;
        for (int n = 0; n < N; ++n) acc = fmaf(dz[m * ldz + n], w[int64_t(n) * ldw + k], acc);
        da[m * ldda + k] = acc;
    }
    const int64_t wv = int64_t(blockIdx.x) * 4 + (threadIdx.x >> 6);
    const int lane = threadIdx.x & 63;
    if (wv < int64_t(N) * K + N) {
        double acc = 0.0;
        if (wv < int64_t(N) * K) {
            const int n = int(wv / K), k = int(wv % K);
            for (int64_t m = lane; m < M; m += 64) acc += double(dz[m * ldz + n]) * a[m * lda + k];
        } else {
            const int n = int(wv - int64_t(N) * K);
            for (int64_t m = lane; m < M; m += 64) acc += dz[m * ldz + n];
        }
        _Pragma("unroll") for (int o = 32; o > 0; o >>= 1) acc += __shfl_down(acc, o, 64);
        if (lane == 0) {
            if (wv < int64_t(N) * K) dw[wv] = float(acc);
            else db[wv - int64_t(N) * K] = float(acc);
        }
    }
}

template <int V>
__global__ __launch_bounds__(256) void gather_bags_kernel(const float* __restrict__ emb, int64_t ld, const int64_t* __restrict__ first_row,
                                                          int64_t windows, int T, int64_t M, float* __restrict__ out) {
    typedef float vec_t __attribute__((ext_vector_type(V)));
    const int64_t per_row = M / V, total = windows * T * per_row;
    for (int64_t i = int64_t(blockIdx.x) * 256 + threadIdx.x; i < total; i += int64_t(gridDim.x) * 256) {
        const int64_t r = i / per_row, p = i - r * per_row, w = r / T;
        const int t = int(r - w * T);
        *reinterpret_cast<vec_t*>(out + r * M + p * V) = *reinterpret_cast<const vec_t*>(emb + (first_row[w] + t) * ld + p * V);
    }
}

}

static_assert(kWideRowBlocks * kMaxWideChannels <= kStatBlocks * kMaxChannels, "the wide column partials must fit the partial area");
extern "C" int64_t mla_bn_stats_workspace_bytes(void) {
    return (int64_t(kStatBlocks) * kMaxChannels + kMaxWideChannels) * 2 * sizeof(double);
}

static inline int max_channels(int mode) { return mode == 0 ? kMaxChannels : kMaxWideChannels; }

extern "C" int mla_bn_stats_sums(const float* x, int64_t rows, int64_t cols, int64_t ldx, int mode, int period, void* workspace,
                                 double* sums, mla_stream_t stream) {
    MLA_REQUIRE(x && workspace && sums && rows > 0 && cols > 0 && ldx >= cols, MLA_E_ARG, "bad bn_stats arguments");
    MLA_REQUIRE(mode == 0 || mode == 1, MLA_E_ARG, "bn_stats mode %d", mode);
    const int channels = mode == 0 ? period : int(cols);
    MLA_REQUIRE(channels >= 1 && channels <= max_channels(mode), MLA_E_SHAPE, "bn_stats supports 1..%d channels (got %d)", max_channels(mode), channels);
    MLA_REQUIRE(mode == 1 || rows % period == 0, MLA_E_SHAPE, "rows %lld not a multiple of period %d", (long long)rows, period);
    return channel_sums(StatsOp{x, ldx}, rows, cols, mode, period, workspace, sums, static_cast<hipStream_t>(stream));
}

extern "C" int mla_bn_stats_finish(const double* sums, int channels, double count, float* mean, float* var_biased,
                                   float* running_mean, float* running_var, float momentum, int64_t* num_batches_tracked,
                                   mla_stream_t stream) {
    MLA_REQUIRE(sums && mean && var_biased && channels >= 1 && channels <= kMaxWideChannels && count > 0, MLA_E_ARG, "bad bn_stats_finish arguments");
    hipLaunchKernelGGL(stats_finish_kernel, dim3(1), dim3(channels <= 64 ? 64 : kMaxWideChannels), 0, static_cast<hipStream_t>(stream), sums, channels, count, mean,
                       var_biased, running_mean, running_var, momentum, num_batches_tracked);
    MLA_LAUNCH_OK("bn stats finish");
    return MLA_OK;
}

extern "C" int mla_bn_stats(const float* x, int64_t rows, int64_t cols, int64_t ldx, int mode, int period, void* workspace,
                            float* mean, float* var_biased, float* running_mean, float* running_var, float momentum,
                            mla_stream_t stream) {
    MLA_REQUIRE(workspace, MLA_E_ARG, "null workspace");
    double* sums = static_cast<double*>(workspace) + int64_t(kStatBlocks) * kMaxChannels * 2;
    const int rc = mla_bn_stats_sums(x, rows, cols, ldx, mode, period, workspace, sums, stream);
    if (rc != MLA_OK) return rc;
    const int channels = mode == 0 ? period : int(cols);
    const double count = mode == 0 ? double(rows / period) * double(cols) : double(rows);
    return mla_bn_stats_finish(sums, channels, count, mean, var_biased, running_mean, running_var, momentum, nullptr, stream);
}

extern "C" int mla_bn_stats_fused(const float* x, int64_t rows, int64_t cols, int64_t ldx, int mode, int period, void* workspace,
                                  double* sums_out, float* mean, float* var_biased, float* running_mean, float* running_var,
                                  float momentum, int64_t* num_batches_tracked, mla_stream_t stream) {
    MLA_REQUIRE(x && workspace && sums_out && mean && var_biased && rows > 0 && cols > 0 && ldx >= cols, MLA_E_ARG, "bad bn_stats arguments");
    MLA_REQUIRE(mode == 0 || mode == 1, MLA_E_ARG, "bn_stats mode %d", mode);
    const int channels = mode == 0 ? period : int(cols);
    MLA_REQUIRE(channels >= 1 && channels <= max_channels(mode), MLA_E_SHAPE, "bn_stats supports 1..%d channels (got %d)", max_channels(mode), channels);
    MLA_REQUIRE(mode == 1 || rows % period == 0, MLA_E_SHAPE, "rows %lld not a multiple of period %d", (long long)rows, period);
    const double count = mode == 0 ? double(rows / period) * double(cols) : double(rows);
    const FinishArgs f{count, mean, var_biased, running_mean, running_var, momentum, num_batches_tracked};
    const int rc = channel_sums(StatsOp{x, ldx}, rows, cols, mode, period, workspace, sums_out, static_cast<hipStream_t>(stream), &f);
    if (rc == 1) return MLA_OK;
    if (rc != MLA_OK) return rc;
    return mla_bn_stats_finish(sums_out, channels, count, mean, var_biased, running_mean, running_var, momentum, num_batches_tracked, stream);
}

extern "C" int mla_bn_apply(const float* x, int64_t ldx, float* y, int64_t ldy, int64_t rows, int64_t cols, int mode,
                            int period, const float* mean, const float* var, const float* gamma, const float* beta,
                            float eps, int act, const uint8_t* keep_mask, float drop_scale, mla_stream_t stream) {
    MLA_REQUIRE(x && y && mean && var && gamma && beta && rows >= 0 && cols > 0, MLA_E_ARG, "bad bn_apply arguments");
    MLA_REQUIRE((mode == 0 && period >= 1) || mode == 1, MLA_E_ARG, "bn_apply mode %d period %d", mode, period);
    MLA_REQUIRE(act >= 0 && act <= 2, MLA_E_ARG, "bn_apply act %d", act);
    if (rows == 0) return MLA_OK;
    const int64_t total = rows * cols;
    const unsigned grid = unsigned((total + 255) / 256 < 8192 ? (total + 255) / 256 : 8192);
    hipStream_t s = static_cast<hipStream_t>(stream);
    if (mode == 0)
        hipLaunchKernelGGL(bn_apply_kernel<0>, dim3(grid), dim3(256), 0, s, x, ldx, y, ldy, rows, int(cols), period, mean, var,
                           gamma, beta, eps, act, keep_mask, drop_scale);
    else
        hipLaunchKernelGGL(bn_apply_kernel<1>, dim3(grid), dim3(256), 0, s, x, ldx, y, ldy, rows, int(cols), period, mean, var,
                           gamma, beta, eps, act, keep_mask, drop_scale);
    MLA_LAUNCH_OK("bn_apply");
    return MLA_OK;
}

static int bn_bwd_sums(const float* x, int64_t ldx, const float* dy, int64_t ld_dy, const float* yout, int64_t ld_y,
                       int act, float drop_scale, int64_t rows, int64_t cols, int mode, int period, const float* mean,
                       const float* var, float eps, void* workspace, double* sums, mla_stream_t stream, int max_cols) {
    MLA_REQUIRE(x && dy && mean && var && workspace && sums && rows > 0 && cols > 0, MLA_E_ARG, "bad bn_bwd_sums arguments");
    MLA_REQUIRE(act == 0 || yout, MLA_E_ARG, "bn_bwd needs the forward output for act %d", act);
    MLA_REQUIRE((mode == 0 && period >= 1 && period <= kMaxChannels && rows % period == 0) || (mode == 1 && cols <= max_cols),
                MLA_E_SHAPE, "bn_bwd channel layout");
    BwdOp op{x, dy, yout, mean, var, ldx, ld_dy, ld_y, act, drop_scale, eps};
    return channel_sums(op, rows, cols, mode, period, workspace, sums, static_cast<hipStream_t>(stream));
}

static int bn_bwd_apply(const float* x, int64_t ldx, const float* dy, int64_t ld_dy, const float* yout, int64_t ld_y,
                        int act, float drop_scale, int64_t rows, int64_t cols, int mode, int period, const float* mean,
                        const float* var, const float* gamma, float eps, const double* sums_global,
                        const double* sums_local, double count, float* dx, int64_t ld_dx, int accumulate,
                        float* dgamma, float* dbeta, mla_stream_t stream, int max_cols) {
    MLA_REQUIRE(x && dy && mean && var && gamma && sums_global && sums_local && count > 0 && rows > 0 && cols > 0, MLA_E_ARG,
                "bad bn_bwd_apply arguments");
    MLA_REQUIRE((dgamma == nullptr) == (dbeta == nullptr), MLA_E_ARG, "dgamma and dbeta go together");
    MLA_REQUIRE(act == 0 || yout, MLA_E_ARG, "bn_bwd needs the forward output for act %d", act);
    MLA_REQUIRE((mode == 0 && period >= 1 && period <= kMaxChannels && rows % period == 0) || (mode == 1 && cols <= max_cols),
                MLA_E_SHAPE, "bn_bwd channel layout");
    BwdOp op{x, dy, yout, mean, var, ldx, ld_dy, ld_y, act, drop_scale, eps};
    const int64_t total = rows * cols;
    const unsigned grid = dx ? unsigned((total + 255) / 256 < 8192 ? (total + 255) / 256 : 8192) : 1u;
    hipStream_t s = static_cast<hipStream_t>(stream);
    if (mode == 0)
        hipLaunchKernelGGL(bn_bwd_apply_kernel<0>, dim3(grid), dim3(256), 0, s, op, gamma, rows, int(cols), period, sums_global,
                           sums_local, count, dx, ld_dx, accumulate, dgamma, dbeta);
    else
        hipLaunchKernelGGL(bn_bwd_apply_kernel<1>, dim3(grid), dim3(256), 0, s, op, gamma, rows, int(cols), period, sums_global,
                           sums_local, count, dx, ld_dx, accumulate, dgamma, dbeta);
    MLA_LAUNCH_OK("bn_bwd_apply");
    return MLA_OK;
}

extern "C" int mla_bn_bwd_sums(const float* x, int64_t ldx, const float* dy, int64_t ld_dy, const float* yout, int64_t ld_y,
                               int act, float drop_scale, int64_t rows, int64_t cols, int mode, int period, const float* mean,
                               const float* var, float eps, void* workspace, double* sums, mla_stream_t stream) {
    return bn_bwd_sums(x, ldx, dy, ld_dy, yout, ld_y, act, drop_scale, rows, cols, mode, period, mean, var, eps, workspace, sums, stream,
                       kMaxChannels);
}

extern "C" int mla_bn_bwd_apply(const float* x, int64_t ldx, const float* dy, int64_t ld_dy, const float* yout, int64_t ld_y,
                                int act, float drop_scale, int64_t rows, int64_t cols, int mode, int period, const float* mean,
                                const float* var, const float* gamma, float eps, const double* sums_global,
                                const double* sums_local, double count, float* dx, int64_t ld_dx, int accumulate,
                                float* dgamma, float* dbeta, mla_stream_t stream) {
    return bn_bwd_apply(x, ldx, dy, ld_dy, yout, ld_y, act, drop_scale, rows, cols, mode, period, mean, var, gamma, eps, sums_global,
                        sums_local, count, dx, ld_dx, accumulate, dgamma, dbeta, stream, kMaxChannels);
}

extern "C" int mla_bn_bwd_sums_wide(const float* x, int64_t ldx, const float* dy, int64_t ld_dy, const float* yout, int64_t ld_y,
                                    int act, float drop_scale, int64_t rows, int64_t cols, const float* mean, const float* var,
                                    float eps, void* workspace, double* sums, mla_stream_t stream) {
    return bn_bwd_sums(x, ldx, dy, ld_dy, yout, ld_y, act, drop_scale, rows, cols, 1, 0, mean, var, eps, workspace, sums, stream,
                       kMaxWideChannels);
}

extern "C" int mla_bn_bwd_apply_wide(const float* x, int64_t ldx, const float* dy, int64_t ld_dy, const float* yout, int64_t ld_y,
                                     int act, float drop_scale, int64_t rows, int64_t cols, const float* mean, const float* var,
                                     const float* gamma, float eps, const double* sums_global, const double* sums_local,
                                     double count, float* dx, int64_t ld_dx, int accumulate, float* dgamma, float* dbeta,
                                     mla_stream_t stream) {
    return bn_bwd_apply(x, ldx, dy, ld_dy, yout, ld_y, act, drop_scale, rows, cols, 1, 0, mean, var, gamma, eps, sums_global,
                        sums_local, count, dx, ld_dx, accumulate, dgamma, dbeta, stream, kMaxWideChannels);
}

extern "C" int mla_attention_pool(const float* z, int64_t bags, int T, int K, const float* v_mean, const float* v_var,
                                  const float* v_gamma, const float* v_beta, const float* f_mean, const float* f_var,
                                  const float* f_gamma, const float* f_beta, float eps, float* y, int64_t ldy,
                                  float* att_out, float* cla_out, mla_stream_t stream) {
    MLA_REQUIRE(z && y && v_mean && v_var && v_gamma && v_beta && f_mean && f_var && f_gamma && f_beta, MLA_E_ARG, "null attention_pool argument");
    MLA_REQUIRE(T >= 1 && T <= kMaxSlots && K >= 1 && K <= kMaxClasses && ldy >= K, MLA_E_SHAPE,
                "attention_pool supports T <= %d, K <= %d (got %d, %d)", kMaxSlots, kMaxClasses, T, K);
    MLA_REQUIRE(bags >= 0 && bags <= 0x7fffffff, MLA_E_ARG, "attention_pool: %lld bags", (long long)bags);
    if (bags == 0) return MLA_OK;
    BnParams nv{v_mean, v_var, v_gamma, v_beta}, nf{f_mean, f_var, f_gamma, f_beta};
    if (T > 16 || K > 16) {
        hipLaunchKernelGGL(attention_pool_wide_kernel, dim3(unsigned(bags)), dim3(256), 0, static_cast<hipStream_t>(stream), z, T, K, nv,
                           nf, eps, y, ldy, att_out, cla_out);
        MLA_LAUNCH_OK("attention_pool (wide)");
        return MLA_OK;
    }
    hipLaunchKernelGGL(attention_pool_kernel<16>, dim3(unsigned((bags + 15) / 16)), dim3(256), 0,
                       static_cast<hipStream_t>(stream), z, bags, T, K, nv, nf, eps, y, ldy, att_out, cla_out);
    MLA_LAUNCH_OK("attention_pool");
    return MLA_OK;
}

extern "C" int mla_attention_pool_bwd(const float* dy, int64_t ld_dy, const float* att, const float* cla, int64_t bags, int T,
                                      int K, float* du_v, float* du_f, mla_stream_t stream) {
    MLA_REQUIRE(dy && att && cla && du_v && du_f && ld_dy >= K, MLA_E_ARG, "bad attention_pool_bwd arguments");
    MLA_REQUIRE(T >= 1 && T <= kMaxSlots && K >= 1 && K <= kMaxClasses, MLA_E_SHAPE,
                "attention_pool_bwd supports T <= %d, K <= %d (got %d, %d)", kMaxSlots, kMaxClasses, T, K);
    MLA_REQUIRE(bags >= 0 && bags <= 0x7fffffff, MLA_E_ARG, "attention_pool_bwd: %lld bags", (long long)bags);
    if (bags == 0) return MLA_OK;
    if (T > 16 || K > 16) {
        hipLaunchKernelGGL(attention_pool_bwd_wide_kernel, dim3(unsigned(bags)), dim3(256), 0, static_cast<hipStream_t>(stream), dy, ld_dy,
                           att, cla, T, K, du_v, du_f);
        MLA_LAUNCH_OK("attention_pool_bwd (wide)");
        return MLA_OK;
    }
    hipLaunchKernelGGL(attention_pool_bwd_kernel<16>, dim3(unsigned((bags + 15) / 16)), dim3(256), 0,
                       static_cast<hipStream_t>(stream), dy, ld_dy, att, cla, bags, T, K, du_v, du_f);
    MLA_LAUNCH_OK("attention_pool_bwd");
    return MLA_OK;
}

extern "C" int mla_linear_small(const float* a, int64_t lda, const float* w, int64_t ldw, const float* bias, float* out,
                                int64_t ldo, int64_t M, int64_t N, int64_t K, mla_stream_t stream) {
    MLA_REQUIRE(a && w && out && M >= 0 && N > 0 && K > 0 && lda >= K && ldw >= K && ldo >= N, MLA_E_ARG, "bad linear_small arguments");
    if (M == 0) return MLA_OK;
    if (N % 4 == 0 && N >= 64 && K <= 64 && N * K * 4 <= 48 * 1024 && ldo % 4 == 0 && mla::aligned(out, 16) && M * N >= (1 << 16)) {
        const int64_t blocks = (M * (N / 4) + 255) / 256;
        hipLaunchKernelGGL(linear_small_wide_kernel, dim3(unsigned(blocks < 1024 ? blocks : 1024)), dim3(256), size_t(N) * K * 4,
                           static_cast<hipStream_t>(stream), a, lda, w, ldw, bias, out, ldo, M, int(N), int(K));
        MLA_LAUNCH_OK("linear_small (wide)");
        return MLA_OK;
    }
    hipLaunchKernelGGL(linear_small_kernel, dim3(unsigned((M * N + 255) / 256)), dim3(256), 0,
                       static_cast<hipStream_t>(stream), a, lda, w, ldw, bias, out, ldo, M, int(N), int(K));
    MLA_LAUNCH_OK("linear_small");
    return MLA_OK;
}

extern "C" int mla_linear_narrow(const float* a, int64_t lda, const float* w, int64_t ldw, const float* bias, float* out,
                                 int64_t ldo, int64_t M, int64_t N, int64_t K, mla_stream_t stream) {
    MLA_REQUIRE(a && w && out && M >= 0 && lda >= K && ldw >= K && ldo >= N, MLA_E_ARG, "bad linear_narrow arguments");
    MLA_REQUIRE(N >= 1 && N <= 16 && K >= 4 && K % 4 == 0 && lda % 4 == 0 && ldw % 4 == 0 && K * N * 4 <= 64 * 1024, MLA_E_SHAPE,
                "linear_narrow: N <= 16, K a multiple of 4 with 16-byte aligned rows (N %lld, K %lld)", (long long)N, (long long)K);
    MLA_REQUIRE(mla::aligned(a, 16) && mla::aligned(w, 16), MLA_E_ARG, "linear_narrow operands must be 16-byte aligned");
    if (M == 0) return MLA_OK;
    const unsigned grid = unsigned((M + 15) / 16 < 2048 ? (M + 15) / 16 : 2048);
    const size_t lds = size_t(K) * N * 4;
    hipStream_t s = static_cast<hipStream_t>(stream);
#define MLA_NARROW_CASE(NN) \
    if (N == NN) { hipLaunchKernelGGL(linear_narrow_kernel<NN>, dim3(grid), dim3(256), lds, s, a, lda, w, ldw, bias, out, ldo, M, int(K)); }
    MLA_NARROW_CASE(1) else MLA_NARROW_CASE(2) else MLA_NARROW_CASE(3) else MLA_NARROW_CASE(4) else MLA_NARROW_CASE(5) else
    MLA_NARROW_CASE(6) else MLA_NARROW_CASE(7) else MLA_NARROW_CASE(8) else MLA_NARROW_CASE(9) else MLA_NARROW_CASE(10) else
    MLA_NARROW_CASE(11) else MLA_NARROW_CASE(12) else MLA_NARROW_CASE(13) else MLA_NARROW_CASE(14) else MLA_NARROW_CASE(15) else
    MLA_NARROW_CASE(16)
#undef MLA_NARROW_CASE
    MLA_LAUNCH_OK("linear_narrow");
    return MLA_OK;
}

extern "C" int mla_gather_bags(const float* emb, int64_t rows, int64_t ld, const int64_t* first_row, const int64_t* host_first_row,
                               int64_t windows, int T, int64_t M, float* out, mla_stream_t stream) {
    MLA_REQUIRE(rows >= 0 && windows >= 0 && T >= 1 && M >= 1 && ld >= M, MLA_E_ARG, "bad gather_bags sizes (rows %lld, windows %lld, T %d, M %lld, ld %lld)",
                (long long)rows, (long long)windows, T, (long long)M, (long long)ld);
    if (windows == 0) return MLA_OK;
    MLA_REQUIRE(emb && first_row && host_first_row && out, MLA_E_ARG, "null emb/first_row/host_first_row/out");
    MLA_REQUIRE(mla::aligned(emb, 4) && mla::aligned(out, 4) && mla::aligned(first_row, 8), MLA_E_ARG, "gather_bags operands are misaligned");
    for (int64_t w = 0; w < windows; ++w) {
        MLA_REQUIRE(host_first_row[w] >= 0 && host_first_row[w] <= rows - T, MLA_E_ARG, "window %lld: rows %lld .. %lld leave emb (%lld rows)",
                    (long long)w, (long long)host_first_row[w], (long long)host_first_row[w] + T - 1, (long long)rows);
    }
    const bool vec = M % 4 == 0 && ld % 4 == 0 && mla::aligned(emb, 16) && mla::aligned(out, 16);
    const int64_t blocks = (windows * T * (vec ? M / 4 : M) + 255) / 256;
    const dim3 grid(unsigned(blocks < 4096 ? blocks : 4096));
    hipStream_t s = static_cast<hipStream_t>(stream);
    if (vec) hipLaunchKernelGGL(gather_bags_kernel<4>, grid, dim3(256), 0, s, emb, ld, first_row, windows, T, M, out);
    else hipLaunchKernelGGL(gather_bags_kernel<1>, grid, dim3(256), 0, s, emb, ld, first_row, windows, T, M, out);
    MLA_LAUNCH_OK("gather_bags");
    return MLA_OK;
}

extern "C" int mla_linear_small_bwd(const float* a, int64_t lda, const float* w, int64_t ldw, const float* dz, int64_t ldz,
                                    int64_t M, int64_t N, int64_t K, float* da, int64_t ldda, float* dw, float* db,
                                    mla_stream_t stream) {
    MLA_REQUIRE(a && w && dz && da && dw && db && M > 0 && N > 0 && K > 0, MLA_E_ARG, "bad linear_small_bwd arguments");
    const int64_t waves = N * K + N;
    const int64_t blocks_da = (M * K + 255) / 256, blocks_dw = (waves + 3) / 4;
    hipLaunchKernelGGL(linear_small_bwd_kernel, dim3(unsigned(blocks_da > blocks_dw ? blocks_da : blocks_dw)), dim3(256), 0,
                       static_cast<hipStream_t>(stream), a, lda, w, ldw, dz, ldz, M, int(N), int(K), da, ldda, dw, db);
    MLA_LAUNCH_OK("linear_small_bwd");
    return MLA_OK;
}
```

### audio-classification-using-a-deep-cnn-combined-with-multi-level-attention_amd/mla_train.py

```python

import torch

from . import ops
from .params import DR


class Ctx:

    def __init__(self, tape=False, dist=None, counter=None, bases=None):
        self.tape = [] if tape else None
        self.dist = dist or ops._local()
        self.counter, self.bases = counter, bases
        self.train = True


def _bn_stats(bn, z, mode, period, train, ctx):
    if train:
        return ops.bn_stats_sync(z, mode, period, ctx.dist, bn.running_mean, bn.running_var, bn.momentum, tracked=bn.num_batches_tracked)
    return bn.running_mean, bn.running_var


def embedded_mapping_forward(em, x, ctx=None):
    ctx = ctx or Ctx()
    B, T, H = x.shape[0], em.slots, em.hidden
    rows = x.detach().reshape(B * T, -1).float().contiguous()
    train = em.training
    mean, var = _bn_stats(em.norm0, rows, 0, T, train, ctx)
    h = ops.bn_apply(rows, 0, T, mean, var, em.norm0.weight.detach(), em.norm0.bias.detach())
    if ctx.tape is not None:
        ctx.tape.append(("norm0", em, rows, mean, var))
    for j in range(em.n_fc):
        if h.shape[1] % 4:
            z = ops.linear_small(h, em.fc[j].weight.detach().contiguous(), em.fc[j].bias.detach().contiguous())
        else:
            z = ops.linear(h, em.fc[j].weight.detach(), em.fc[j].bias.detach())
        mean, var = _bn_stats(em.norms[j], z, 0, T, train, ctx)
        if train and ctx.counter is not None:
            d = em.dropouts[j]
            keep = d.keep_mask_dev(z.numel(), z.device, ctx.dist.rank * z.numel(), ctx.counter, ctx.bases[id(d)])
        else:
            keep = em.dropouts[j].keep_mask(z.numel(), z.device, offset=ctx.dist.rank * z.numel()) if train else None
        h_in = h
        h = ops.bn_apply(z, 0, T, mean, var, em.norms[j].weight.detach(), em.norms[j].bias.detach(), act=1,
                         keep_mask=keep, drop_scale=1.0 / (1.0 - DR))
        if ctx.tape is not None:
            ctx.tape.append(("fc", em, j, h_in, z, mean, var, h))
    return h.reshape(B, T, H)


def attention_forward(am, h, y, ctx=None, level=0):
    ctx = ctx or Ctx()
    B, T, H, K = h.shape[0], am.slots, am.hidden, am.classes
    rows = h.reshape(B * T, H)
    z = ops.linear(rows, am.fcv.weight.detach(), am.fcv.bias.detach())
    if am.training:
        mean, var = ops.bn_stats_sync(z, 0, T, ctx.dist, am.normv.running_mean, am.normv.running_var, am.normv.momentum,
                                      also=((am.normf.running_mean, am.normf.running_var, am.normf.momentum, am.normf.num_batches_tracked),),
                                      tracked=am.normv.num_batches_tracked)
        nv = (mean, var, am.normv.weight.detach(), am.normv.bias.detach())
        nf = (mean, var, am.normf.weight.detach(), am.normf.bias.detach())
    else:
        nv = (am.normv.running_mean, am.normv.running_var, am.normv.weight.detach(), am.normv.bias.detach())
        nf = (am.normf.running_mean, am.normf.running_var, am.normf.weight.detach(), am.normf.bias.detach())
    att, cla = ops.attention_pool(z, B, T, K, nv, nf, y, save=ctx.tape is not None)
    if ctx.tape is not None:
        ctx.tape.append(("att", am, level, rows, z, nv, nf, att, cla))


def mla_forward(mla, x, ctx=None):
    ctx = ctx or Ctx()
    ctx.train = mla.training
    B, K = x.shape[0], mla.classes
    L = len(mla.model)
    conc = torch.empty((B, L * K), dtype=torch.float32, device=x.device)
    cur = x
    for lvl in range(L):
        cur = embedded_mapping_forward(mla.embedded_mappings[lvl], cur, ctx)
        attention_forward(mla.attention_modules[lvl], cur, conc[:, lvl * K:(lvl + 1) * K], ctx, lvl)
    z = ops.linear_small(conc, mla.fc.weight.detach(), mla.fc.bias.detach())
    mean, var = _bn_stats(mla.norm, z, 1, 0, mla.training, ctx)
    out = ops.bn_apply(z, 1, 0, mean, var, mla.norm.weight.detach(), mla.norm.bias.detach(), act=2)
    if ctx.tape is not None:
        ctx.tape.append(("head", mla, conc, z, mean, var, out))
    return out


def mla_apply(mla, x):
    return mla_forward(mla, x, None)


def _linear_backward(x_in, weight, dz, g_w, g_b, want_dx):
    if x_in.shape[1] % 4:
        g_w = g_w if g_w is not None else torch.empty(weight.shape, dtype=torch.float32, device=dz.device)
        g_b = g_b if g_b is not None else torch.empty(weight.shape[0], dtype=torch.float32, device=dz.device)
        dx = ops.linear_small_bwd(x_in.contiguous(), weight.contiguous(), dz.contiguous(), g_w, g_b)
        return dx if want_dx else None
    if g_w is not None:
        dzT = ops.transpose_padded(dz)
        xT = ops.transpose_padded(x_in)
        ops.linear(dzT, xT, None, out=g_w, split_k=True)
    if g_b is not None:
        ops.col_sum(dz, g_b)
    if not want_dx:
        return None
    wT = ops.transpose_padded(weight)
    if dz.shape[1] % 4:
        return ops.linear_small(dz, wT[:, :dz.shape[1]].contiguous(), None)
    return ops.linear(dz, wT, None)


def mla_backward(mla, ctx, dout, grads, need_input_grad=False):
    tape, dist = ctx.tape, ctx.dist
    T, K = mla.slots, mla.classes
    bs = ctx.train
    drop = 1.0 / (1.0 - DR) if bs else 1.0
    kind, _, conc, z, mean, var, out = tape[-1]
    assert kind == "head"
    dz = ops.bn_backward(z, dout, out, 2, 1.0, 1, 0, mean, var, mla.norm.weight.detach(), dist, grads["norm.weight"], grads["norm.bias"],
                         batch_stats=bs)
    dconc = ops.linear_small_bwd(conc, mla.fc.weight.detach(), dz, grads["fc.weight"], grads["fc.bias"])

    levels, cur = [], []
    for e in tape[:-1]:
        cur.append(e)
        if e[0] == "att":
            levels.append(cur)
            cur = []
    dh_next = None
    B = dconc.shape[0]
    for lvl in range(len(levels) - 1, -1, -1):
        entries = levels[lvl]
        _, am, _, h_rows, z_att, nv, nf, att, cla = entries[-1]
        pa = "attention_modules.%d." % lvl
        du_v, du_f = ops.attention_pool_bwd(dconc[:, lvl * K:(lvl + 1) * K], att, cla, B, T, K)
        dz_att = ops.bn_backward(z_att, du_v, None, 0, 1.0, 0, T, nv[0], nv[1], nv[2], dist, grads[pa + "normv.weight"], grads[pa + "normv.bias"],
                                 batch_stats=bs)
        ops.bn_backward(z_att, du_f, None, 0, 1.0, 0, T, nf[0], nf[1], nf[2], dist, grads[pa + "normf.weight"], grads[pa + "normf.bias"],
                        dx=dz_att, accumulate=True, batch_stats=bs)
        dh = _linear_backward(h_rows, am.fcv.weight.detach(), dz_att, grads[pa + "fcv.weight"], grads[pa + "fcv.bias"], True)
        if dh_next is not None:
            ops.axpy(1.0, dh_next, dh)
        em = entries[0][1]
        pe = "embedded_mappings.%d." % lvl
        for e in reversed(entries[1:-1]):
            _, _, j, h_in, z_j, mean_j, var_j, h_out = e
            dzj = ops.bn_backward(z_j, dh, h_out, 1, drop, 0, T, mean_j, var_j, em.norms[j].weight.detach(), dist,
                                  grads[pe + "norms.%d.weight" % j], grads[pe + "norms.%d.bias" % j], batch_stats=bs)
            dh = _linear_backward(h_in, em.fc[j].weight.detach(), dzj, grads[pe + "fc.%d.weight" % j], grads[pe + "fc.%d.bias" % j], True)
        _, _, rows_in, mean0, var0 = entries[0]
        want = lvl > 0 or need_input_grad
        dh_next = ops.bn_backward(rows_in, dh, None, 0, 1.0, 0, T, mean0, var0, em.norm0.weight.detach(), dist,
                                  grads[pe + "norm0.weight"], grads[pe + "norm0.bias"], want_dx=want, batch_stats=bs)
    return dh_next
```

### audio-classification-using-a-deep-cnn-combined-with-multi-level-attention_amd/ops.py

```python

import ctypes
import os

import torch

from . import _lib

DT = {torch.float32: _lib.F32, torch.bfloat16: _lib.BF16, torch.int16: _lib.I16}
BN_EPS = 1e-5

profile = None
_ws = {}


_event_pool = []


def reserve_events(n):
    while len(_event_pool) < n:
        e = torch.cuda.Event(enable_timing=True)
        e.record()
        _event_pool.append(e)
    torch.cuda.synchronize()


def _event():
    return _event_pool.pop() if _event_pool else torch.cuda.Event(enable_timing=True)


def _timed(name, fn, *args):
    if profile is None:
        return fn(*args)
    e0, e1 = _event(), _event()
    e0.record()
    rc = fn(*args)
    e1.record()
    profile.append((name, e0, e1))
    return rc


def _p(t):
    return ctypes.c_void_p(t.data_ptr()) if t is not None else None


def _chk(t, dtype=None):
    assert t.is_cuda and t.is_contiguous(), "HIP ops need contiguous CUDA tensors"
    if dtype is not None:
        assert t.dtype == dtype, (t.dtype, dtype)
    return t


def _chk_rows(t, dtype=None):
    assert t.is_cuda and t.dim() == 2 and (t.is_contiguous() or (t.stride(1) == 1 and t.stride(0) >= t.shape[1])), \
        "HIP ops need CUDA matrices with contiguous rows"
    if dtype is not None:
        assert t.dtype == dtype, (t.dtype, dtype)
    return t


def repack_conv_weight(w, dtype):
    _chk(w, torch.float32)
    cout, cin = w.shape[0], w.shape[1]
    out = torch.empty((cout, 9, cin), dtype=dtype, device=w.device)
    _lib.check(_lib.lib().mla_conv_repack_weights(_p(w), cout, cin, _p(out), DT[dtype], _lib.stream_ptr()))
    return out


def split_conv_weight(w):
    packed = repack_conv_weight(w, torch.float32)
    cout, _, cin = packed.shape
    out = torch.empty((cout, 9, 3 * cin), dtype=torch.bfloat16, device=w.device)
    _lib.check(_lib.lib().mla_split_bf16x3(_p(packed), cout * 9, cin, cin, _p(out), 3 * cin, 64, 3, _lib.stream_ptr()))
    return out


def split_linear_weight(w, seg):
    _chk(w, torch.float32)
    n, k = w.shape
    out = torch.empty((n, 3 * k), dtype=torch.bfloat16, device=w.device)
    _lib.check(_lib.lib().mla_split_bf16x3(_p(w), n, k, k, _p(out), 3 * k, seg, 3, _lib.stream_ptr()))
    return out


def merge_split(x, seg):
    _chk(x, torch.bfloat16)
    rows, c2 = x.shape
    out = torch.empty((rows, c2 // 2), dtype=torch.float32, device=x.device)
    _lib.check(_lib.lib().mla_merge_bf16x3(_p(x), rows, c2 // 2, c2, seg, _p(out), _lib.stream_ptr()))
    return out


def linear_split(a, w, b, seg, relu=True, out_split=True):
    _chk(a, torch.bfloat16); _chk(w, torch.bfloat16)
    M, K = a.shape[0], a.shape[1] // 2
    N = w.shape[0]
    assert w.shape[1] == 3 * K
    out = torch.empty((M, 2 * N), dtype=torch.bfloat16, device=a.device) if out_split else torch.empty((M, N), dtype=torch.float32, device=a.device)
    _lib.check(_timed("linear_%dx%d" % (K, N), _lib.lib().mla_linear_bf16x3, _p(a), a.stride(0), _p(w), w.stride(0), _p(b), _p(out),
                      out.stride(0), M, N, K, seg, _lib.BF16X3 if out_split else _lib.F32, int(relu), _lib.stream_ptr()))
    return out


def to_bf16(w):
    _chk(w, torch.float32)
    out = torch.empty(w.shape, dtype=torch.bfloat16, device=w.device)
    _lib.check(_lib.lib().mla_convert_f32(_p(w), _p(out), w.numel(), _lib.BF16, _lib.stream_ptr()))
    return out


def to_f32(x):
    _chk(x, torch.bfloat16)
    out = torch.empty(x.shape, dtype=torch.float32, device=x.device)
    _lib.check(_lib.lib().mla_convert_bf16_to_f32(_p(x), _p(out), x.numel(), _lib.stream_ptr()))
    return out


def conv1(x, w, b, dtype, split=False):
    _chk(x); _chk(w, torch.float32); _chk(b, torch.float32)
    n = x.shape[0]
    assert tuple(x.shape[1:]) == (96, 64) and tuple(w.shape) == (64, 1, 3, 3)
    out = torch.empty((n, 48, 32, 128 if split else 64), dtype=dtype, device=x.device)
    _lib.check(_timed("conv1", _lib.lib().mla_vggish_conv1, _p(x), DT[x.dtype], n, _p(w), _p(b), _p(out),
                      _lib.BF16X3 if split else DT[dtype], _lib.stream_ptr()))
    return out


FUSED_FRONT = os.environ.get("MLA_FUSED_FRONT", "1") != "0"


def logmel_conv1(pcm, w, b):
    from . import frontend
    assert pcm.dim() == 2 and pcm.is_cuda and pcm.stride(1) == 1 and pcm.dtype in (torch.float32, torch.int16)
    _chk(w, torch.float32); _chk(b, torch.float32)
    assert tuple(w.shape) == (64, 1, 3, 3)
    n_wave, n_samples = pcm.shape
    _, n_ex = frontend.counts(n_samples)
    out = torch.empty((n_wave * n_ex, 48, 32, 64), dtype=torch.bfloat16, device=pcm.device)
    if n_wave * n_ex == 0:
        return out
    tab = frontend.device_tables(pcm.device)
    _lib.check(_timed("logmel", _lib.lib().mla_logmel_conv1, _p(pcm), DT[pcm.dtype], n_wave, n_samples,
                      pcm.stride(0) if n_wave > 1 else n_samples, _p(tab), _p(w), _p(b), _p(out), _lib.stream_ptr()))
    return out


CONV_SHAPES = {2: ((48, 32, 64), (24, 16, 128)), 3: ((24, 16, 128), (24, 16, 256)), 4: ((24, 16, 256), (12, 8, 256)),
               5: ((12, 8, 256), (12, 8, 512)), 6: ((12, 8, 512), (6, 4, 512))}


def conv(layer, x, w_packed, b, split=False):
    _chk(x); _chk(w_packed, x.dtype); _chk(b, torch.float32)
    shp_in, shp_out = CONV_SHAPES[layer]
    ka, kw, ko = (2, 3, 2) if split else (1, 1, 1)
    assert tuple(x.shape[1:]) == shp_in[:2] + (ka * shp_in[2],), (x.shape, shp_in)
    assert tuple(w_packed.shape) == (shp_out[2], 9, kw * shp_in[2])
    n = x.shape[0]
    out = torch.empty((n,) + shp_out[:2] + (ko * shp_out[2],), dtype=x.dtype, device=x.device)
    _lib.check(_timed("conv%d" % layer, _lib.lib().mla_vggish_conv, layer, _p(x), _p(w_packed), _p(b), _p(out), n,
                      _lib.BF16X3 if split else DT[x.dtype], _lib.stream_ptr()))
    return out


KSPLIT = 8


def linear(a, w, b, relu=False, out_dtype=None, out=None, split_k=False):
    _chk(a); _chk(w, a.dtype)
    M, K = a.shape
    N = w.shape[0]
    assert w.shape[1] == K
    out_dtype = out_dtype or a.dtype
    if out is None:
        out = torch.empty((M, N), dtype=out_dtype, device=a.device)
    else:
        assert out.is_contiguous() and out.numel() == M * N and out.dtype == out_dtype
    if (N <= 16 and a.dtype == torch.float32 and out_dtype == torch.float32 and not relu and not split_k and K % 4 == 0
            and K * N * 4 <= 65536 and a.stride(0) % 4 == 0 and w.stride(0) % 4 == 0
            and a.data_ptr() % 16 == 0 and w.data_ptr() % 16 == 0):
        _lib.check(_timed("linear_%dx%d" % (K, N), _lib.lib().mla_linear_narrow, _p(a), a.stride(0), _p(w), w.stride(0), _p(b), _p(out), N,
                          M, N, K, _lib.stream_ptr()))
        return out
    kc = 64 if a.dtype == torch.bfloat16 else 32
    if N <= 128 and K >= 2048 and K % (kc * KSPLIT) == 0 and not split_k and a.stride(0) % 8 == 0 and w.stride(0) % 8 == 0:
        key = "ksplit/" + str(a.device)
        if key not in _ws or _ws[key].numel() < KSPLIT * M * N:
            _ws[key] = torch.empty(max(KSPLIT * M * N, 1 << 22), dtype=torch.float32, device=a.device)
        ws = _ws[key]
        _lib.check(_timed("linear_%dx%d" % (K, N), _lib.lib().mla_linear_ksplit, _p(a), a.stride(0), _p(w), w.stride(0), _p(b), _p(out), N,
                          M, N, K, DT[a.dtype], DT[out_dtype], int(relu), KSPLIT, _p(ws), ws.numel(), _lib.stream_ptr()))
        return out
    tiles = ((M + 127) // 128) * ((N + 127) // 128)
    if split_k and a.dtype == torch.float32 and out_dtype == torch.float32 and tiles <= 64 and K >= 2048:
        splits = int(min(64, max(2, 256 // tiles), K // 512))
        key = "splitk/" + str(a.device)
        if key not in _ws or _ws[key].numel() < splits * M * N:
            _ws[key] = torch.empty(max(splits * M * N, 1 << 22), dtype=torch.float32, device=a.device)
        ws = _ws[key]
        _lib.check(_timed("linear_splitk_%dx%d" % (K, N), _lib.lib().mla_linear_splitk, _p(a), a.stride(0), _p(w), w.stride(0), _p(b),
                          _p(out), N, M, N, K, int(relu), splits, _p(ws), ws.numel(), _lib.stream_ptr()))
        return out
    _lib.check(_timed("linear_%dx%d" % (K, N), _lib.lib().mla_linear, _p(a), a.stride(0), _p(w), w.stride(0), _p(b), _p(out), N,
                      M, N, K, DT[a.dtype], DT[out_dtype], int(relu), _lib.stream_ptr()))
    return out


def linear_small(a, w, b):
    _chk(a, torch.float32); _chk(w, torch.float32)
    M, K = a.shape
    N = w.shape[0]
    out = torch.empty((M, N), dtype=torch.float32, device=a.device)
    _lib.check(_lib.lib().mla_linear_small(_p(a), a.stride(0), _p(w), w.stride(0), _p(b), _p(out), N, M, N, K, _lib.stream_ptr()))
    return out


def _workspace(device):
    key = str(device)
    if key not in _ws:
        _ws[key] = torch.empty(int(_lib.lib().mla_bn_stats_workspace_bytes()) // 8, dtype=torch.float64, device=device)
    return _ws[key]


def bn_stats(x, mode, period, running_mean=None, running_var=None, momentum=-1.0):
    _chk(x, torch.float32)
    rows, cols = x.shape
    ch = period if mode == 0 else cols
    mean = torch.empty(ch, dtype=torch.float32, device=x.device)
    var = torch.empty(ch, dtype=torch.float32, device=x.device)
    _lib.check(_lib.lib().mla_bn_stats(_p(x), rows, cols, x.stride(0), mode, period, _p(_workspace(x.device)), _p(mean),
                                       _p(var), _p(running_mean), _p(running_var), float(momentum), _lib.stream_ptr()))
    return mean, var


def bn_apply(x, mode, period, mean, var, gamma, beta, act=0, keep_mask=None, drop_scale=1.0, out=None):
    _chk_rows(x, torch.float32)
    rows, cols = x.shape
    if out is None:
        out = torch.empty((rows, cols), dtype=torch.float32, device=x.device)
    if keep_mask is not None:
        _chk(keep_mask, torch.uint8)
        assert keep_mask.numel() == rows * cols
    _lib.check(_lib.lib().mla_bn_apply(_p(x), x.stride(0), _p(out), out.stride(0), rows, cols, mode, period, _p(mean), _p(var),
                                       _p(gamma), _p(beta), BN_EPS, act, _p(keep_mask), float(drop_scale), _lib.stream_ptr()))
    return out


def attention_pool(z, bags, T, K, nv, nf, y, save=False):
    _chk(z, torch.float32)
    assert y.dtype == torch.float32 and y.stride(1) == 1
    att = torch.empty_like(z) if save else None
    cla = torch.empty_like(z) if save else None
    _lib.check(_lib.lib().mla_attention_pool(_p(z), bags, T, K, _p(nv[0]), _p(nv[1]), _p(nv[2]), _p(nv[3]), _p(nf[0]), _p(nf[1]),
                                             _p(nf[2]), _p(nf[3]), BN_EPS, _p(y), y.stride(0), _p(att), _p(cla), _lib.stream_ptr()))
    return att, cla



def gather_bags(emb, first_rows, T):
    import numpy as np
    _chk_rows(emb, torch.float32)
    if isinstance(first_rows, torch.Tensor):
        first_rows = first_rows.detach().cpu().numpy()
    fr = np.ascontiguousarray(np.asarray(first_rows), dtype=np.int64).reshape(-1)
    W, (N, M) = fr.shape[0], emb.shape
    out = torch.empty((W * int(T), M), dtype=torch.float32, device=emb.device)
    if W == 0:
        return out
    host = torch.empty(W, dtype=torch.int64, pin_memory=True)
    host.numpy()[:] = fr
    d = host.to(emb.device, non_blocking=True)
    _lib.check(_timed("gather_bags", _lib.lib().mla_gather_bags, _p(emb), N, emb.stride(0) if N > 1 else M, _p(d),
                      fr.ctypes.data_as(ctypes.c_void_p), W, int(T), M, _p(out), _lib.stream_ptr()))
    return out


class Dist:

    def __init__(self, group=None, always=None, sync_bn=True):
        import os
        import torch.distributed as dist
        self.group, self.comm = group, None
        self.sync_bn, self.trace = sync_bn, None
        inited = dist.is_available() and dist.is_initialized()
        self.world = dist.get_world_size(group) if inited else 1
        self.rank = dist.get_rank(group) if inited else 0
        self.backend = dist.get_backend(group) if inited else None
        always = (os.environ.get("MLA_DIST_ALWAYS") == "1") if always is None else always
        self.active = inited and (self.world > 1 or always)
        self.via = None
        self.fallback = None
        if self.active and self.backend == "nccl":
            self.via = os.environ.get("MLA_DIST_COLLECTIVE", "abi")
            if self.via == "abi":
                err = None
                try:
                    self._init_comm(dist)
                except Exception as e:
                    err = "%s: %s" % (type(e).__name__, e)
                ok = torch.tensor([0 if err else 1], dtype=torch.int32, device=torch.device("cuda", torch.cuda.current_device()))
                dist.all_reduce(ok, op=dist.ReduceOp.MIN, group=self.group)
                if int(ok.item()) == 0:
                    self.close()
                    self.via = "torch"
                    self.fallback = err or "another rank could not create its communicator through the C ABI"
        elif self.active:
            self.via = "host"

    def _init_comm(self, dist):
        dev = torch.device("cuda", torch.cuda.current_device())
        uid, err0 = torch.zeros(128, dtype=torch.uint8), None
        if self.rank == 0:
            buf = (ctypes.c_char * 128)()
            try:
                _lib.check(_lib.lib().mla_comm_unique_id(ctypes.cast(buf, ctypes.c_void_p)))
                uid = torch.frombuffer(bytearray(buf.raw), dtype=torch.uint8).clone()
            except Exception as e:
                err0 = e
        uid = uid.to(dev)
        src = dist.get_global_rank(self.group, 0) if self.group is not None else 0
        dist.broadcast(uid, src=src, group=self.group)
        raw = bytes(uid.cpu().numpy().tobytes())
        if err0 is not None or not any(raw):
            raise err0 or RuntimeError("rank 0 could not obtain an RCCL unique id through the C ABI")
        comm = ctypes.c_void_p()
        _lib.check(_lib.lib().mla_comm_init_rank(ctypes.byref(comm), self.world, ctypes.c_char_p(raw), self.rank))
        self.comm = comm
        import atexit
        import weakref
        ref = weakref.ref(self)
        atexit.register(lambda: ref() is not None and ref().close())

    def close(self):
        if self.comm is not None:
            torch.cuda.synchronize()
            _lib.check(_lib.lib().mla_comm_destroy(self.comm))
            self.comm = None


    def _reduce(self, t):
        import torch.distributed as dist
        if self.via == "abi":
            assert t.is_cuda and t.is_contiguous()
            code = {torch.float32: _lib.F32, torch.float64: _lib.F64, torch.int32: _lib.I32}[t.dtype]
            _lib.check(_lib.lib().mla_allreduce_flat(_p(t), t.numel(), code, self.comm, _lib.stream_ptr()))
        elif self.via == "torch":
            dist.all_reduce(t, op=dist.ReduceOp.SUM, group=self.group)
        elif t.is_cuda:
            host = t.cpu()
            dist.all_reduce(host, op=dist.ReduceOp.SUM, group=self.group)
            t.copy_(host)
        else:
            dist.all_reduce(t, op=dist.ReduceOp.SUM, group=self.group)
        return t

    def all_reduce_sum(self, t, tag="other"):
        if not self.active:
            return t
        if self.trace is None:
            return self._reduce(t)
        e0, e1 = _event(), _event()
        e0.record()
        self._reduce(t)
        e1.record()
        self.trace.append((tag, t.numel() * t.element_size(), e0, e1))
        return t

    @property
    def bn_active(self):
        return self.active and self.sync_bn

    @property
    def bn_world(self):
        return self.world if self.bn_active else 1

    def ranks_reported(self):
        if self.comm is not None:
            n = ctypes.c_int(-1)
            _lib.check(_lib.lib().mla_comm_count(self.comm, ctypes.byref(n)))
            return int(n.value)
        import torch.distributed as dist
        return dist.get_world_size(self.group) if self.active else 1

    def describe(self):
        origin = _lib.lib().mla_comm_library_origin().decode() if self.via == "abi" else None
        return {"active": bool(self.active), "backend": self.backend, "transport": {"abi": "mla_allreduce_flat (C ABI -> ncclAllReduce)",
                "torch": "torch.distributed.all_reduce", "host": "torch.distributed.all_reduce through host copies (gloo rehearsal)",
                None: None}[self.via], "rccl_library_origin": origin, "ranks": self.ranks_reported(), "sync_bn": bool(self.sync_bn),
                "fallback": getattr(self, "fallback", None)}


LOCAL = None


def _local():
    global LOCAL
    if LOCAL is None:
        LOCAL = Dist.__new__(Dist)
        LOCAL.group, LOCAL.world, LOCAL.rank, LOCAL.active, LOCAL.comm, LOCAL.via = None, 1, 0, False, None, None
        LOCAL.sync_bn, LOCAL.trace, LOCAL.backend, LOCAL.fallback = True, None, None, None
    return LOCAL


def dropout_mask(n, seed, stream_id, offset, p_drop, device):
    out = torch.empty(n, dtype=torch.uint8, device=device)
    _lib.check(_lib.lib().mla_dropout_mask(_p(out), n, int(seed) & (2 ** 64 - 1), int(stream_id) & (2 ** 64 - 1), int(offset), float(p_drop),
                                           _lib.stream_ptr()))
    return out


def bn_stats_sync(x, mode, period, dist, running_mean=None, running_var=None, momentum=-1.0, also=(), tracked=None):
    _chk(x, torch.float32)
    rows, cols = x.shape
    ch = period if mode == 0 else cols
    sums = torch.empty(2 * ch, dtype=torch.float64, device=x.device)
    L = _lib.lib()
    mean = torch.empty(ch, dtype=torch.float32, device=x.device)
    var = torch.empty(ch, dtype=torch.float32, device=x.device)
    count = (rows // period * cols if mode == 0 else rows) * dist.bn_world
    if dist.bn_active:
        _lib.check(L.mla_bn_stats_sums(_p(x), rows, cols, x.stride(0), mode, period, _p(_workspace(x.device)), _p(sums), _lib.stream_ptr()))
        dist.all_reduce_sum(sums, "syncbn_fwd")
        _lib.check(L.mla_bn_stats_finish(_p(sums), ch, float(count), _p(mean), _p(var), _p(running_mean), _p(running_var),
                                         float(momentum), _p(tracked), _lib.stream_ptr()))
    else:
        _lib.check(L.mla_bn_stats_fused(_p(x), rows, cols, x.stride(0), mode, period, _p(_workspace(x.device)), _p(sums), _p(mean), _p(var),
                                        _p(running_mean), _p(running_var), float(momentum), _p(tracked), _lib.stream_ptr()))
    for rm, rv, mom, trk in also:
        scratch_m, scratch_v = torch.empty_like(mean), torch.empty_like(var)
        _lib.check(L.mla_bn_stats_finish(_p(sums), ch, float(count), _p(scratch_m), _p(scratch_v), _p(rm), _p(rv), float(mom), _p(trk),
                                         _lib.stream_ptr()))
    return mean, var


def bn_backward(x, dy, yout, act, drop_scale, mode, period, mean, var, gamma, dist, dgamma, dbeta, want_dx=True,
                dx=None, accumulate=False, batch_stats=True, count=None):
    _chk_rows(x, torch.float32); _chk_rows(dy, torch.float32)
    if yout is not None:
        _chk_rows(yout, torch.float32)
    rows, cols = x.shape
    ch = period if mode == 0 else cols
    L = _lib.lib()
    local = torch.empty(2 * ch, dtype=torch.float64, device=x.device)
    ld_y = yout.stride(0) if yout is not None else 0
    wide = mode == 1 and cols > 64
    if wide:
        _lib.check(L.mla_bn_bwd_sums_wide(_p(x), x.stride(0), _p(dy), dy.stride(0), _p(yout), ld_y, act, float(drop_scale), rows, cols,
                                          _p(mean), _p(var), BN_EPS, _p(_workspace(x.device)), _p(local), _lib.stream_ptr()))
    else:
        _lib.check(L.mla_bn_bwd_sums(_p(x), x.stride(0), _p(dy), dy.stride(0), _p(yout), ld_y, act, float(drop_scale), rows, cols, mode,
                                     period, _p(mean), _p(var), BN_EPS, _p(_workspace(x.device)), _p(local), _lib.stream_ptr()))
    glob = local
    if not batch_stats:
        glob = torch.zeros_like(local)
    elif dist.bn_active:
        glob = dist.all_reduce_sum(local.clone(), "syncbn_bwd")
    if count is None:
        count = (rows // period * cols if mode == 0 else rows) * dist.bn_world
    if want_dx and dx is None:
        dx = torch.empty((rows, cols), dtype=torch.float32, device=x.device)
    tail = (_p(mean), _p(var), _p(gamma), BN_EPS, _p(glob), _p(local), float(count), _p(dx) if want_dx else None,
            dx.stride(0) if want_dx else 0, int(accumulate), _p(dgamma), _p(dbeta), _lib.stream_ptr())
    head = (_p(x), x.stride(0), _p(dy), dy.stride(0), _p(yout), ld_y, act, float(drop_scale), rows, cols)
    _lib.check(L.mla_bn_bwd_apply_wide(*head, *tail) if wide else L.mla_bn_bwd_apply(*head, mode, period, *tail))
    return dx


def attention_pool_bwd(dy, att, cla, bags, T, K):
    du_v, du_f = torch.empty_like(att), torch.empty_like(att)
    _lib.check(_lib.lib().mla_attention_pool_bwd(_p(dy), dy.stride(0), _p(att), _p(cla), bags, T, K, _p(du_v), _p(du_f), _lib.stream_ptr()))
    return du_v, du_f


def linear_small_bwd(a, w, dz, dw, db):
    M, K = a.shape
    N = w.shape[0]
    da = torch.empty((M, K), dtype=torch.float32, device=a.device)
    _lib.check(_lib.lib().mla_linear_small_bwd(_p(a), a.stride(0), _p(w), w.stride(0), _p(dz), dz.stride(0), M, N, K, _p(da), K,
                                               _p(dw), _p(db), _lib.stream_ptr()))
    return da


def transpose_padded(x):
    _chk_rows(x)
    R, C = x.shape
    if x.dtype == torch.bfloat16:
        ld = (R + 7) // 8 * 8
        out = torch.empty((C, ld), dtype=torch.bfloat16, device=x.device)
        _lib.check(_lib.lib().mla_transpose_bf16(_p(x), x.stride(0), _p(out), ld, R, C, _lib.stream_ptr()))
        return out
    _chk_rows(x, torch.float32)
    ld = (R + 3) // 4 * 4
    out = torch.zeros((C, ld), dtype=torch.float32, device=x.device) if ld != R else torch.empty((C, ld), dtype=torch.float32, device=x.device)
    _lib.check(_lib.lib().mla_transpose_f32(_p(x), x.stride(0), _p(out), ld, R, C, _lib.stream_ptr()))
    return out


def col_sum(x, out):
    _chk_rows(x)
    rows, cols = x.shape
    key = "colsum/" + str(x.device)
    if key not in _ws or _ws[key].numel() < 64 * cols:
        _ws[key] = torch.empty(64 * max(cols, 4096), dtype=torch.float64, device=x.device)
    ws = _ws[key]
    fn = _lib.lib().mla_col_sum_bf16 if x.dtype == torch.bfloat16 else _lib.lib().mla_col_sum
    _lib.check(fn(_p(x), x.stride(0), rows, cols, _p(ws), _p(out), _lib.stream_ptr()))
    return out


def axpy(a, x, y):
    _lib.check(_lib.lib().mla_axpy(float(a), _p(x), _p(y), x.numel(), _lib.stream_ptr()))
    return y


def check_labels(labels, K):
    if not labels.is_cuda and labels.numel():
        lo, hi = int(labels.min()), int(labels.max())
        if lo < 0 or hi >= K:
            raise IndexError("Target %d is out of bounds." % (lo if lo < 0 else hi))


def raise_on_bad_labels(hits):
    n, bad = (int(v) for v in hits.tolist())
    if bad > 0:
        raise IndexError("Target out of bounds: %d label(s) outside [0, num_classes)." % bad)
    return n


def cross_entropy(scores, labels, inv_total, want_grad=True):
    _chk_rows(scores, torch.float32); _chk(labels, torch.int64)
    B, K = scores.shape
    loss = torch.empty(1, dtype=torch.float32, device=scores.device)
    hits = torch.empty(2, dtype=torch.int32, device=scores.device)
    d = torch.empty((B, K), dtype=torch.float32, device=scores.device) if want_grad else None
    _lib.check(_lib.lib().mla_cross_entropy(_p(scores), scores.stride(0), _p(labels), B, K, float(inv_total), _p(loss), _p(d),
                                            K, _p(hits), _lib.stream_ptr()))
    return loss, d, hits


def dropout_mask_dev(n, seed, stream_base, counter, offset, p_drop, device, out=None):
    assert counter.dtype == torch.int64 and counter.is_cuda
    if out is None:
        out = torch.empty(n, dtype=torch.uint8, device=device)
    _lib.check(_lib.lib().mla_dropout_mask_dev(_p(out), n, int(seed) & (2 ** 64 - 1), int(stream_base) & (2 ** 64 - 1), _p(counter), int(offset),
                                               float(p_drop), _lib.stream_ptr()))
    return out


def adam_prepare(scal, lr, beta1, beta2, step):
    assert scal.dtype == torch.float32 and scal.is_cuda and scal.numel() == 2
    _lib.check(_lib.lib().mla_adam_prepare(_p(scal), float(lr), float(beta1), float(beta2), int(step), _lib.stream_ptr()))


def adam_step_dev(p, g, m, v, beta1, beta2, eps, scal, counter):
    L = _lib.lib()
    _lib.check(L.mla_adam_step_dev(_p(p), _p(g), _p(m), _p(v), p.numel(), float(beta1), float(beta2), float(eps), _p(scal), _lib.stream_ptr()))
    _lib.check(L.mla_counter_add(_p(counter), 1, _lib.stream_ptr()))


def adam_step(p, g, m, v, lr, beta1, beta2, eps, step):
    _lib.check(_lib.lib().mla_adam_step(_p(p), _p(g), _p(m), _p(v), p.numel(), float(lr), float(beta1), float(beta2), float(eps),
                                        int(step), _lib.stream_ptr()))



def conv3x3(x, w_packed, b, cout, pool, act):
    _chk(x); _chk(w_packed, x.dtype)
    n, H, W_, cin = x.shape
    out = torch.empty((n, H // 2, W_ // 2, cout) if pool else (n, H, W_, cout), dtype=x.dtype, device=x.device)
    _lib.check(_timed("conv3x3_%d_%d" % (cin, cout), _lib.lib().mla_conv3x3, _p(x), _p(w_packed), _p(b), _p(out), n, H, W_, cin, cout,
                      int(pool), int(act), DT[x.dtype], _lib.stream_ptr()))
    return out


def conv3x3_train(x, w_packed, b, cout):
    _chk(x); _chk(w_packed, x.dtype)
    n, H, W_, cin = x.shape
    a = torch.empty((n, H, W_, cout), dtype=x.dtype, device=x.device)
    pooled = torch.empty((n, H // 2, W_ // 2, cout), dtype=x.dtype, device=x.device)
    _lib.check(_timed("conv3x3_%d_%d" % (cin, cout), _lib.lib().mla_conv3x3_train, _p(x), _p(w_packed), _p(b), _p(a), _p(pooled), n, H, W_,
                      cin, cout, DT[x.dtype], _lib.stream_ptr()))
    return a, pooled


def conv3x3_train_codes(x, w_packed, b, cout):
    _chk(x); _chk(w_packed, x.dtype)
    n, H, W_, cin = x.shape
    codes = torch.empty((n, H // 2, W_ // 2, cout), dtype=torch.uint8, device=x.device)
    pooled = torch.empty((n, H // 2, W_ // 2, cout), dtype=x.dtype, device=x.device)
    _lib.check(_timed("conv3x3_%d_%d" % (cin, cout), _lib.lib().mla_conv3x3_train_codes, _p(x), _p(w_packed), _p(b), _p(codes), _p(pooled),
                      n, H, W_, cin, cout, DT[x.dtype], _lib.stream_ptr()))
    return codes, pooled


def _bias_ws(bf16, device):
    key = ("biasws16/" if bf16 else "biasws/") + str(device)
    if key not in _ws:
        nbytes = _lib.lib().mla_relu_pool_bwd_bf16_workspace_bytes() if bf16 else _lib.lib().mla_relu_pool_bwd_bias_workspace_bytes()
        _ws[key] = torch.empty(int(nbytes) // 8, dtype=torch.float64, device=device)
    return _ws[key]


def pool_bwd_codes(codes, d_out, db=None):
    assert codes.dtype == torch.uint8 and codes.is_cuda and codes.is_contiguous()
    _chk(d_out, torch.bfloat16)
    n, HO, WO, C = codes.shape
    assert tuple(d_out.shape) == tuple(codes.shape)
    dz = torch.empty((n, 2 * HO, 2 * WO, C), dtype=torch.bfloat16, device=codes.device)
    _lib.check(_timed("relu_pool_bwd", _lib.lib().mla_pool_bwd_codes_bf16, _p(codes), _p(d_out), _p(dz), n, 2 * HO, 2 * WO, C,
                      _p(_bias_ws(True, codes.device)), _p(db), _lib.stream_ptr()))
    return dz


def repack_dgrad(w, dtype=torch.float32):
    _chk(w, torch.float32)
    cout, cin = w.shape[0], w.shape[1]
    out = torch.empty((cin, 9, cout), dtype=dtype, device=w.device)
    fn = _lib.lib().mla_conv_repack_dgrad_bf16 if dtype == torch.bfloat16 else _lib.lib().mla_conv_repack_dgrad
    _lib.check(fn(_p(w), cout, cin, _p(out), _lib.stream_ptr()))
    return out


def maxpool2x2(a):
    _chk(a)
    n, H, W_, C = a.shape
    out = torch.empty((n, H // 2, W_ // 2, C), dtype=a.dtype, device=a.device)
    fn = _lib.lib().mla_maxpool2x2_bf16 if a.dtype == torch.bfloat16 else _lib.lib().mla_maxpool2x2
    _lib.check(_timed("maxpool", fn, _p(a), _p(out), n, H, W_, C, _lib.stream_ptr()))
    return out


def relu_pool_bwd(a, d_out, pool, db=None, bf16=False):
    _chk(a); _chk(d_out, a.dtype)
    a4 = a if a.dim() == 4 else a.reshape(a.shape[0], 1, 1, -1)
    n, H, W_, C = a4.shape
    if bf16 or a.dtype == torch.bfloat16:
        dz = torch.empty(a.shape, dtype=torch.bfloat16, device=a.device)
        _lib.check(_timed("relu_pool_bwd", _lib.lib().mla_relu_pool_bwd_bf16, _p(a), DT[a.dtype], _p(d_out), DT[d_out.dtype], _p(dz), n, H, W_, C,
                          int(pool), _p(_bias_ws(True, a.device)), _p(db), _lib.stream_ptr()))
        return dz
    _chk(a, torch.float32)
    dz = torch.empty_like(a)
    if db is None:
        _lib.check(_lib.lib().mla_relu_pool_bwd(_p(a), _p(d_out), _p(dz), n, H, W_, C, int(pool), _lib.stream_ptr()))
        return dz
    _chk(db, torch.float32)
    _lib.check(_timed("relu_pool_bwd", _lib.lib().mla_relu_pool_bwd_bias, _p(a), _p(d_out), _p(dz), n, H, W_, C, int(pool),
                      _p(_bias_ws(False, a.device)), _p(db), _lib.stream_ptr()))
    return dz


_wg_ws = {}


def scratch(device):
    return {(i, k): t for i, d in enumerate((_ws, _wg_ws)) for k, t in d.items() if t.device == device}


def conv_wgrad(dz, a_in, dw):
    _chk(dz); _chk(a_in, dz.dtype)
    n, H, W_, cout = dz.shape
    cin = a_in.shape[3]
    key = str(dz.device)
    if key not in _wg_ws:
        _wg_ws[key] = torch.empty(int(_lib.lib().mla_conv_wgrad_workspace_floats()), dtype=torch.float32, device=dz.device)
    ws = _wg_ws[key]
    assert dw.is_contiguous() and tuple(dw.shape) == (cout, cin, 3, 3) and dw.dtype == torch.float32
    fn = _lib.lib().mla_conv_wgrad_bf16 if dz.dtype == torch.bfloat16 else _lib.lib().mla_conv_wgrad
    _lib.check(_timed("wgrad_%d_%d" % (cin, cout), fn, _p(dz), _p(a_in), n, H, W_, cin, cout, _p(ws), ws.numel(), _p(dw), _lib.stream_ptr()))


def conv1_bwd(x, w, b, d_pooled, dw, db):
    _chk(x, torch.float32); _chk(d_pooled)
    n = x.shape[0]
    ws = torch.empty(int(_lib.lib().mla_conv1_bwd_workspace_floats()), dtype=torch.float32, device=x.device)
    fn = _lib.lib().mla_conv1_bwd_bf16 if d_pooled.dtype == torch.bfloat16 else _lib.lib().mla_conv1_bwd
    _lib.check(_timed("conv1_bwd", fn, _p(x), _p(w), _p(b), _p(d_pooled), n, _p(ws), _p(dw), _p(db), _lib.stream_ptr()))


def conv1_dgrad(x, w, b, d_pooled):
    _chk(x, torch.float32); _chk(w, torch.float32); _chk(b, torch.float32); _chk(d_pooled)
    n = x.shape[0]
    assert tuple(x.shape) == (n, 96, 64) and tuple(d_pooled.shape) == (n, 48, 32, 64) and tuple(w.shape) == (64, 1, 3, 3) and b.numel() == 64
    dx = torch.empty((n, 96, 64), dtype=torch.float32, device=x.device)
    _lib.check(_timed("conv1_dgrad", _lib.lib().mla_conv1_dgrad, _p(x), _p(w), _p(b), _p(d_pooled), DT[d_pooled.dtype], n, _p(dx),
                      _lib.stream_ptr()))
    return dx



def rn_repack(w, dtype):
    _chk(w, torch.float32)
    cout, cin, ks = w.shape[0], w.shape[1], w.shape[2]
    out = torch.empty((cout, ks, ks, cin), dtype=dtype, device=w.device)
    _lib.check(_lib.lib().mla_rn_repack(_p(w), cout, cin, ks, _p(out), DT[dtype], _lib.stream_ptr()))
    return out


def rn_stem(planes, single, w, dtype, scale=None, shift=None, relu=False):
    _chk(planes, torch.float32); _chk(w, torch.float32)
    assert planes.dim() == 3, planes.shape
    n, H, W_ = planes.shape
    out = torch.empty((n, 112, 112, 64), dtype=dtype, device=planes.device)
    _lib.check(_timed("rn_stem", _lib.lib().mla_rn_stem, _p(planes), n, H, W_, int(single), _p(w), _p(scale), _p(shift), int(relu), _p(out),
                      DT[dtype], _lib.stream_ptr()))
    return out


def rn_conv(x, w_packed, stride, scale=None, shift=None, residual=None, relu=False):
    _chk(x); _chk(w_packed, x.dtype)
    n, H, W_, cin = x.shape
    cout, ks = w_packed.shape[0], w_packed.shape[1]
    pad = ks // 2
    Ho, Wo = (H + 2 * pad - ks) // stride + 1, (W_ + 2 * pad - ks) // stride + 1
    out = torch.empty((n, Ho, Wo, cout), dtype=x.dtype, device=x.device)
    if residual is not None:
        _chk(residual, x.dtype)
        assert residual.shape == out.shape, (residual.shape, out.shape)
    _lib.check(_timed("rn_conv%dx%d" % (ks, ks), _lib.lib().mla_rn_conv, _p(x), n, H, W_, cin, _p(w_packed), cout, ks, stride,
                      _p(scale), _p(shift), _p(residual), int(relu), _p(out), DT[x.dtype], _lib.stream_ptr()))
    return out


def _rn_workspace(device, channels):
    key = ("rn_bn", str(device))
    need = int(_lib.lib().mla_rn_bn_workspace_bytes(channels)) // 8
    if key not in _ws or _ws[key].numel() < need:
        _ws[key] = torch.empty(need, dtype=torch.float64, device=device)
    return _ws[key]


def _rn_bn_finish(x, bn, running, want_stats, name, fn, *head):
    C = x.shape[-1]
    dev = x.device
    scale = torch.empty(C, dtype=torch.float32, device=dev)
    shift = torch.empty(C, dtype=torch.float32, device=dev)
    mean = torch.empty(C, dtype=torch.float32, device=dev) if want_stats else None
    var = torch.empty(C, dtype=torch.float32, device=dev) if want_stats else None
    rm, rv = (bn.running_mean, bn.running_var) if running else (None, None)
    _lib.check(_timed(name, fn, *head, _p(bn.weight.detach()), _p(bn.bias.detach()), float(bn.eps), float(bn.momentum), _p(rm), _p(rv),
                      _p(mean), _p(var), _p(scale), _p(shift), _lib.stream_ptr()))
    if running:
        _lib.check(_lib.lib().mla_counter_add(_p(bn.num_batches_tracked), 1, _lib.stream_ptr()))
    return (scale, shift, mean, var) if want_stats else (scale, shift)


def rn_bn_stats(x, bn, running=True, want_stats=False):
    _chk(x)
    C = x.shape[-1]
    return _rn_bn_finish(x, bn, running, want_stats, "rn_bn_stats", _lib.lib().mla_rn_bn_stats, _p(x), x.numel() // C, C, DT[x.dtype],
                         _p(_rn_workspace(x.device, C)))


def rn_bn_stats_sync(x, bn, dist, running=True, want_stats=False):
    if not dist.bn_active:
        return rn_bn_stats(x, bn, running, want_stats)
    _chk(x)
    C = x.shape[-1]
    L = _lib.lib()
    sums = torch.empty(2 * C + 1, dtype=torch.float64, device=x.device)
    _lib.check(_timed("rn_bn_sums", L.mla_rn_bn_sums, _p(x), x.numel() // C, C, DT[x.dtype], _p(_rn_workspace(x.device, C)), _p(sums),
                      _lib.stream_ptr()))
    dist.all_reduce_sum(sums, "syncbn_rn")
    return _rn_bn_finish(x, bn, running, want_stats, "rn_bn_finish", L.mla_rn_bn_finish, _p(sums), C)


def rn_bn_eval_coeffs(bn):
    C = bn.num_features
    dev = bn.weight.device
    scale = torch.empty(C, dtype=torch.float32, device=dev)
    shift = torch.empty(C, dtype=torch.float32, device=dev)
    _lib.check(_lib.lib().mla_rn_bn_eval_coeffs(_p(bn.weight.detach()), _p(bn.bias.detach()), _p(bn.running_mean), _p(bn.running_var),
                                                float(bn.eps), C, _p(scale), _p(shift), _lib.stream_ptr()))
    return scale, shift


def rn_bn_apply(x, scale, shift, residual=None, relu=False, out=None):
    _chk(x)
    C = x.shape[-1]
    out = x if out is None else out
    if residual is not None:
        _chk(residual, x.dtype)
        assert residual.shape == x.shape
    _lib.check(_timed("rn_bn_apply", _lib.lib().mla_rn_bn_apply, _p(x), x.numel() // C, C, _p(scale), _p(shift), _p(residual), int(relu),
                      _p(out), DT[x.dtype], _lib.stream_ptr()))
    return out


def rn_maxpool(x):
    _chk(x)
    n, H, W_, C = x.shape
    out = torch.empty((n, (H - 1) // 2 + 1, (W_ - 1) // 2 + 1, C), dtype=x.dtype, device=x.device)
    _lib.check(_timed("rn_maxpool", _lib.lib().mla_rn_maxpool, _p(x), n, H, W_, C, _p(out), DT[x.dtype], _lib.stream_ptr()))
    return out


def rn_avgpool(x):
    _chk(x)
    n, H, W_, C = x.shape
    out = torch.empty((n, C), dtype=torch.float32, device=x.device)
    _lib.check(_timed("rn_avgpool", _lib.lib().mla_rn_avgpool, _p(x), n, H * W_, C, _p(out), DT[x.dtype], _lib.stream_ptr()))
    return out



def rn_repack_dgrad(w, dtype):
    _chk(w, torch.float32)
    cout, cin, ks = w.shape[0], w.shape[1], w.shape[2]
    out = torch.empty((cin, ks, ks, cout), dtype=dtype, device=w.device)
    _lib.check(_lib.lib().mla_rn_repack_dgrad(_p(w), cout, cin, ks, _p(out), DT[dtype], _lib.stream_ptr()))
    return out


def rn_conv_dgrad(dy, w_dgrad, stride, in_hw, residual=None):
    _chk(dy); _chk(w_dgrad, dy.dtype)
    n, Ho, Wo, cout = dy.shape
    cin, ks = w_dgrad.shape[0], w_dgrad.shape[1]
    H, W_ = in_hw
    out = torch.empty((n, H, W_, cin), dtype=dy.dtype, device=dy.device)
    if residual is not None:
        _chk(residual, dy.dtype)
        assert residual.shape == out.shape, (residual.shape, out.shape)
    _lib.check(_timed("rn_dgrad%dx%d_s%d" % (ks, ks, stride), _lib.lib().mla_rn_conv_dgrad, _p(dy), n, Ho, Wo, cout, _p(w_dgrad), cin, ks,
                      stride, H, W_, _p(residual), _p(out), DT[dy.dtype], _lib.stream_ptr()))
    return out


def rn_conv_wgrad(x, dy, stride, dw):
    _chk(x); _chk(dy, x.dtype); _chk(dw, torch.float32)
    n, H, W_, cin = x.shape
    cout, ks = dw.shape[0], dw.shape[2]
    assert tuple(dw.shape) == (cout, cin, ks, ks) and dy.shape[3] == cout
    L = _lib.lib()
    need = int(L.mla_rn_conv_wgrad_workspace_floats(n, dy.shape[1], dy.shape[2], cin, cout, ks, DT[x.dtype]))
    ws = torch.empty(max(need, 1), dtype=torch.float32, device=x.device)
    _lib.check(_timed("rn_wgrad%dx%d" % (ks, ks), L.mla_rn_conv_wgrad, _p(x), _p(dy), n, H, W_, cin, cout, ks, stride, _p(ws), ws.numel(),
                      _p(dw), DT[x.dtype], _lib.stream_ptr()))


def rn_stem_wgrad(planes, single, dy, dw):
    _chk(planes, torch.float32); _chk(dy); _chk(dw, torch.float32)
    n = planes.shape[0]
    L = _lib.lib()
    ws = torch.empty(int(L.mla_rn_stem_wgrad_workspace_floats(n)), dtype=torch.float32, device=planes.device)
    _lib.check(_timed("rn_stem_wgrad", L.mla_rn_stem_wgrad, _p(planes), n, int(single), _p(dy), _p(ws), ws.numel(), _p(dw), DT[dy.dtype],
                      _lib.stream_ptr()))


def rn_bn_bwd(x, dy, mean, var, bn, y=None, want_dres=False, dgamma=None, dbeta=None):
    _chk(x); _chk(dy, x.dtype)
    if y is not None:
        _chk(y, x.dtype)
    C = x.shape[-1]
    rows = x.numel() // C
    L = _lib.lib()
    ws = torch.empty(int(L.mla_rn_bn_bwd_workspace_bytes(C)) // 8, dtype=torch.float64, device=x.device)
    dx = torch.empty_like(x)
    dres = torch.empty_like(x) if want_dres else None
    _lib.check(_timed("rn_bn_bwd", L.mla_rn_bn_bwd, _p(x), _p(dy), _p(y), rows, C, _p(mean), _p(var), _p(bn.weight.detach()), float(bn.eps),
                      _p(ws), _p(dgamma), _p(dbeta), _p(dx), _p(dres), DT[x.dtype], _lib.stream_ptr()))
    return dx, dres


def rn_bn_bwd_sync(x, dy, mean, var, bn, dist, y=None, want_dres=False, dgamma=None, dbeta=None):
    if not dist.bn_active:
        return rn_bn_bwd(x, dy, mean, var, bn, y=y, want_dres=want_dres, dgamma=dgamma, dbeta=dbeta)
    _chk(x); _chk(dy, x.dtype)
    if y is not None:
        _chk(y, x.dtype)
    C = x.shape[-1]
    rows = x.numel() // C
    L = _lib.lib()
    ws = torch.empty(int(L.mla_rn_bn_bwd_workspace_bytes(C)) // 8, dtype=torch.float64, device=x.device)
    sums = torch.empty(2 * C + 1, dtype=torch.float64, device=x.device)
    _lib.check(_timed("rn_bn_bwd_sums", L.mla_rn_bn_bwd_sums, _p(x), _p(dy), _p(y), rows, C, _p(mean), _p(var), float(bn.eps), _p(ws), _p(sums),
                      _p(dgamma), _p(dbeta), DT[x.dtype], _lib.stream_ptr()))
    dist.all_reduce_sum(sums, "syncbn_rn_bwd")
    dx = torch.empty_like(x)
    dres = torch.empty_like(x) if want_dres else None
    _lib.check(_timed("rn_bn_bwd_apply", L.mla_rn_bn_bwd_apply, _p(x), _p(dy), _p(y), rows, C, _p(mean), _p(var), _p(bn.weight.detach()),
                      float(bn.eps), _p(sums), _p(ws), _p(dx), _p(dres), DT[x.dtype], _lib.stream_ptr()))
    return dx, dres


def rn_maxpool_bwd(x, dy):
    _chk(x); _chk(dy, x.dtype)
    n, H, W_, C = x.shape
    dx = torch.empty_like(x)
    _lib.check(_timed("rn_maxpool_bwd", _lib.lib().mla_rn_maxpool_bwd, _p(x), _p(dy), n, H, W_, C, _p(dx), DT[x.dtype], _lib.stream_ptr()))
    return dx


def rn_avgpool_bwd(d, shape, dtype):
    _chk(d, torch.float32)
    n, H, W_, C = shape
    dx = torch.empty((n, H, W_, C), dtype=dtype, device=d.device)
    _lib.check(_timed("rn_avgpool_bwd", _lib.lib().mla_rn_avgpool_bwd, _p(d), n, H * W_, C, _p(dx), DT[dtype], _lib.stream_ptr()))
    return dx



def rn_act_bwd(dy, scale, y=None, want_dres=False):
    _chk(dy); _chk(scale, torch.float32)
    if y is not None:
        _chk(y, dy.dtype)
        assert y.shape == dy.shape, (y.shape, dy.shape)
    C = dy.shape[-1]
    assert scale.numel() == C, (scale.shape, C)
    dpre = torch.empty_like(dy)
    dres = torch.empty_like(dy) if want_dres else None
    _lib.check(_timed("rn_act_bwd", _lib.lib().mla_rn_act_bwd, _p(dy), _p(y), _p(scale), dy.numel() // C, C, _p(dpre), _p(dres), DT[dy.dtype],
                      _lib.stream_ptr()))
    return dpre, dres


def rn_stem_dgrad(dy, w, single, y=None, scale=None):
    _chk(dy); _chk(w, torch.float32)
    n = dy.shape[0]
    assert tuple(dy.shape) == (n, 112, 112, 64) and tuple(w.shape) == (64, 3, 7, 7), (dy.shape, w.shape)
    assert (y is None) == (scale is None), "y and scale come together"
    if y is not None:
        _chk(y, dy.dtype); _chk(scale, torch.float32)
        assert y.shape == dy.shape and scale.numel() == 64, (y.shape, scale.shape)
    dx = torch.empty((n, 224, 224), dtype=torch.float32, device=dy.device)
    _lib.check(_timed("rn_stem_dgrad", _lib.lib().mla_rn_stem_dgrad, _p(dy), n, _p(y), _p(scale), _p(w), int(single), _p(dx), DT[dy.dtype],
                      _lib.stream_ptr()))
    return dx
```

### include/mla_hip.h

```cpp
#ifndef MLA_HIP_H
#define MLA_HIP_H

#include <stdint.h>

#ifdef __cplusplus
extern "C" {
#endif

#define MLA_OK            0
#define MLA_E_ARG        -1
#define MLA_E_SHAPE      -2
#define MLA_E_SHORT      -3
#define MLA_E_LAUNCH     -4
#define MLA_E_DTYPE      -5

#define MLA_F32   0
#define MLA_BF16  1
#define MLA_I16   2
#define MLA_F64   4
#define MLA_I32   5
#define MLA_U8    6
#define MLA_I24   7
#define MLA_BF16X3 3

typedef void* mla_stream_t;

int         mla_abi_version(void);
const char* mla_last_error(void);


int mla_logmel_counts(int64_t n_samples, int64_t* stft_frames, int64_t* examples);

int64_t mla_logmel_table_floats(void);
int     mla_logmel_build_tables(float* host_out);
int     mla_logmel_reference_tables(double* host_window400, double* host_mel_257x64);

int mla_logmel_examples(const void* pcm, int pcm_dtype, int64_t n_wave, int64_t n_samples,
                        int64_t wave_stride, const float* tables, void* out, int out_dtype,
                        mla_stream_t stream);

int mla_stft_magnitude(const float* signal, int64_t n_samples, const float* window, const float* twiddle,
                       int64_t window_length, int64_t hop_length, int64_t fft_length, float* out,
                       mla_stream_t stream);
int mla_mel_log(const float* spectrogram, const float* mel_matrix, int64_t frames, int64_t bins, int64_t bands,
                float log_offset, float* out, mla_stream_t stream);

int mla_mono_mix(const void* pcm, int pcm_dtype, int64_t n_samples, int channels, float* out, mla_stream_t stream);
int mla_dataset_frames(const float* examples, int64_t clips, int ex_per_clip, int n_frames, int frame_len,
                       int stride, float* out, mla_stream_t stream);
int mla_logmel_bags(const void* pcm, int pcm_dtype, int64_t clips, int64_t n_samples, int64_t row_stride, const int32_t* counts,
                    const int32_t* host_counts, int n_frames, int stride, const float* tables, void* out, int out_dtype,
                    mla_stream_t stream);
int mla_timeline_counts(int64_t n_samples, int64_t hop_slots, int64_t* windows, int64_t* slots, int64_t* samples_read);
int mla_logmel_timeline(const void* pcm, int pcm_dtype, int64_t recordings, int64_t n_samples, int64_t row_stride, const int64_t* desc,
                        const int64_t* host_desc, int64_t total_slots, const float* tables, void* out, int out_dtype,
                        mla_stream_t stream);

int64_t mla_melspec_frames(int64_t n_samples, int64_t hop);
int64_t mla_melspec_table_floats(double sr, int64_t n_mels);
int     mla_melspec_build_tables(double sr, int64_t n_mels, float* host_out);
int64_t mla_melspec_workspace_bytes(int64_t clips, int64_t n_samples, int64_t hop);
int mla_melspec_db(const float* pcm, int64_t clips, int64_t n_samples, int64_t clip_stride, int64_t hop, int64_t n_mels,
                   float amin, const float* tables, float* out_db, float* workspace, mla_stream_t stream);
int mla_melspec_images(const float* db, const float* workspace, int64_t clips, int64_t n_samples, int64_t hop, int64_t n_mels,
                       float top_db, int64_t n_images, int64_t image_w, int64_t image_stride, float* out, mla_stream_t stream);

int mla_melspec_track_counts(int64_t n_samples, int64_t hop_images, int64_t* windows, int64_t* images, int64_t* samples,
                             int64_t* columns);
int mla_melspec_track_db(const float* pcm, int64_t recordings, int64_t n_samples, int64_t row_stride, const int64_t* desc,
                         const int64_t* host_desc, int64_t total_columns, float amin, const float* tables, float* out_db,
                         float* workspace, float* maxima, mla_stream_t stream);
int mla_melspec_track_images(const float* db, const float* maxima, int64_t recordings, const int64_t* desc, const int64_t* host_desc,
                             int64_t total_columns, float top_db, int64_t first, int64_t count, float* out, mla_stream_t stream);


int64_t mla_melspec_band_table_floats(double sr, int64_t n_mels, double fmin, double fmax, int htk);
int     mla_melspec_build_band_tables(double sr, int64_t n_mels, double fmin, double fmax, int htk, float* host_out);
int64_t mla_melspec_nopad_frames(int64_t n_samples, int64_t hop);
int64_t mla_melspec_nopad_workspace_bytes(int64_t clips, int64_t n_samples, int64_t hop);
int mla_melspec_nopad_db(const float* pcm, int64_t clips, int64_t n_samples, int64_t clip_stride, int64_t hop, int64_t n_mels,
                         float amin, const float* tables, int64_t table_floats, float* out_db, float* workspace, mla_stream_t stream);
int mla_melspec_nopad_bags(const float* db, const float* workspace, int64_t clips, int64_t n_samples, int64_t hop, int64_t n_mels,
                           float top_db, int64_t n_images, int64_t image_w, int64_t image_stride, void* out, int out_dtype,
                           mla_stream_t stream);

int mla_postprocess(const float* embeddings, const float* pca_eigen_vectors, const float* pca_means, int64_t rows,
                    float* out, mla_stream_t stream);


int mla_conv_repack_weights(const float* w_oihw, int64_t cout, int64_t cin, void* out, int dtype,
                            mla_stream_t stream);
int mla_convert_f32(const float* in, void* out, int64_t n, int dtype, mla_stream_t stream);
int mla_convert_bf16_to_f32(const void* in, float* out, int64_t n, mla_stream_t stream);
int mla_split_bf16x3(const float* in, int64_t rows, int64_t cols, int64_t ld_in, void* out, int64_t ld_out, int64_t seg,
                     int copies, mla_stream_t stream);
int mla_merge_bf16x3(const void* in, int64_t rows, int64_t cols, int64_t ld_in, int64_t seg, float* out, mla_stream_t stream);
int mla_linear_bf16x3(const void* a, int64_t lda, const void* w, int64_t ldw, const float* bias, void* out, int64_t ldo,
                      int64_t M, int64_t N, int64_t K, int64_t seg, int out_dtype, int relu, mla_stream_t stream);

int mla_vggish_conv1(const void* x, int x_dtype, int64_t n, const float* w, const float* bias, void* out,
                     int dtype, mla_stream_t stream);

int mla_logmel_conv1(const void* pcm, int pcm_dtype, int64_t n_wave, int64_t n_samples, int64_t wave_stride,
                     const float* tables, const float* w, const float* bias, void* out, mla_stream_t stream);

int mla_vggish_conv(int layer, const void* in, const void* w_repacked, const float* bias, void* out,
                    int64_t n, int dtype, mla_stream_t stream);

int mla_linear(const void* a, int64_t lda, const void* w, int64_t ldw, const float* bias, void* out,
               int64_t ldo, int64_t M, int64_t N, int64_t K, int dtype, int out_dtype, int relu,
               mla_stream_t stream);
int mla_linear_ksplit(const void* a, int64_t lda, const void* w, int64_t ldw, const float* bias, void* out, int64_t ldo,
                      int64_t M, int64_t N, int64_t K, int dtype, int out_dtype, int relu, int splits, float* workspace,
                      int64_t workspace_floats, mla_stream_t stream);
int mla_linear_splitk(const float* a, int64_t lda, const float* w, int64_t ldw, const float* bias, float* out,
                      int64_t ldo, int64_t M, int64_t N, int64_t K, int relu, int splits, float* workspace,
                      int64_t workspace_floats, mla_stream_t stream);
int mla_linear_narrow(const float* a, int64_t lda, const float* w, int64_t ldw, const float* bias, float* out,
                      int64_t ldo, int64_t M, int64_t N, int64_t K, mla_stream_t stream);
int mla_linear_small(const float* a, int64_t lda, const float* w, int64_t ldw, const float* bias,
                     float* out, int64_t ldo, int64_t M, int64_t N, int64_t K, mla_stream_t stream);


int64_t mla_bn_stats_workspace_bytes(void);
int mla_bn_stats(const float* x, int64_t rows, int64_t cols, int64_t ldx, int mode, int period,
                 void* workspace, float* mean, float* var_biased, float* running_mean,
                 float* running_var, float momentum, mla_stream_t stream);

int mla_bn_apply(const float* x, int64_t ldx, float* y, int64_t ldy, int64_t rows, int64_t cols, int mode,
                 int period, const float* mean, const float* var, const float* gamma, const float* beta,
                 float eps, int act, const uint8_t* keep_mask, float drop_scale, mla_stream_t stream);

int mla_attention_pool(const float* z, int64_t bags, int T, int K, const float* v_mean, const float* v_var,
                       const float* v_gamma, const float* v_beta, const float* f_mean, const float* f_var,
                       const float* f_gamma, const float* f_beta, float eps, float* y, int64_t ldy,
                       float* att_out, float* cla_out, mla_stream_t stream);

int mla_gather_bags(const float* emb, int64_t rows, int64_t ld, const int64_t* first_row, const int64_t* host_first_row,
                    int64_t windows, int T, int64_t M, float* out, mla_stream_t stream);

int mla_bn_stats_sums(const float* x, int64_t rows, int64_t cols, int64_t ldx, int mode, int period,
                      void* workspace, double* sums, mla_stream_t stream);
int mla_bn_stats_finish(const double* sums, int channels, double count, float* mean, float* var_biased,
                        float* running_mean, float* running_var, float momentum, int64_t* num_batches_tracked ,
                        mla_stream_t stream);
int mla_bn_stats_fused(const float* x, int64_t rows, int64_t cols, int64_t ldx, int mode, int period, void* workspace,
                       double* sums_out, float* mean, float* var_biased, float* running_mean, float* running_var,
                       float momentum, int64_t* num_batches_tracked, mla_stream_t stream);


int mla_bn_bwd_sums(const float* x, int64_t ldx, const float* dy, int64_t ld_dy, const float* yout, int64_t ld_y,
                    int act, float drop_scale, int64_t rows, int64_t cols, int mode, int period, const float* mean,
                    const float* var, float eps, void* workspace, double* sums, mla_stream_t stream);
int mla_bn_bwd_apply(const float* x, int64_t ldx, const float* dy, int64_t ld_dy, const float* yout, int64_t ld_y,
                     int act, float drop_scale, int64_t rows, int64_t cols, int mode, int period, const float* mean,
                     const float* var, const float* gamma, float eps, const double* sums_global,
                     const double* sums_local, double count, float* dx, int64_t ld_dx, int accumulate,
                     float* dgamma, float* dbeta, mla_stream_t stream);
int mla_bn_bwd_sums_wide(const float* x, int64_t ldx, const float* dy, int64_t ld_dy, const float* yout, int64_t ld_y,
                         int act, float drop_scale, int64_t rows, int64_t cols, const float* mean, const float* var,
                         float eps, void* workspace, double* sums, mla_stream_t stream);
int mla_bn_bwd_apply_wide(const float* x, int64_t ldx, const float* dy, int64_t ld_dy, const float* yout, int64_t ld_y,
                          int act, float drop_scale, int64_t rows, int64_t cols, const float* mean, const float* var,
                          const float* gamma, float eps, const double* sums_global, const double* sums_local, double count,
                          float* dx, int64_t ld_dx, int accumulate, float* dgamma, float* dbeta, mla_stream_t stream);

int mla_attention_pool_bwd(const float* dy, int64_t ld_dy, const float* att, const float* cla, int64_t bags, int T,
                           int K, float* du_v, float* du_f, mla_stream_t stream);

int mla_linear_small_bwd(const float* a, int64_t lda, const float* w, int64_t ldw, const float* dz, int64_t ldz,
                         int64_t M, int64_t N, int64_t K, float* da, int64_t ldda, float* dw, float* db,
                         mla_stream_t stream);

int mla_transpose_f32(const float* in, int64_t ld_in, float* out, int64_t ld_out, int64_t rows, int64_t cols,
                      mla_stream_t stream);
int mla_col_sum(const float* x, int64_t ldx, int64_t rows, int64_t cols, void* workspace, float* out,
                mla_stream_t stream);
int mla_axpy(float a, const float* x, float* y, int64_t n, mla_stream_t stream);

int mla_cross_entropy(const float* x, int64_t ldx, const int64_t* labels, int64_t rows, int K, float inv_total,
                      float* loss, float* dx, int64_t ld_dx, int* n_correct, mla_stream_t stream);


int mla_conv3x3(const void* in, const void* w_packed, const float* bias, void* out, int64_t n, int H, int W,
                int cin, int cout, int pool, int act, int dtype, mla_stream_t stream);
int mla_conv3x3_train(const void* in, const void* w_packed, const float* bias, void* out_prepool, void* out_pooled, int64_t n,
                      int H, int W, int cin, int cout, int dtype, mla_stream_t stream);
int mla_conv_repack_dgrad(const float* w_oihw, int64_t cout, int64_t cin, float* out, mla_stream_t stream);
int mla_maxpool2x2(const float* a, float* out, int64_t n, int H, int W, int C, mla_stream_t stream);
int mla_relu_pool_bwd(const float* a, const float* d_out, float* dz, int64_t n, int H, int W, int C, int pool,
                      mla_stream_t stream);
int64_t mla_relu_pool_bwd_bias_workspace_bytes(void);
int mla_relu_pool_bwd_bias(const float* a, const float* d_out, float* dz, int64_t n, int H, int W, int C, int pool,
                           void* workspace, float* db, mla_stream_t stream);
int64_t mla_conv_wgrad_workspace_floats(void);
int mla_conv_wgrad(const float* dz, const float* a_in, int64_t n, int H, int W, int cin, int cout, float* workspace,
                   int64_t workspace_floats, float* dw_oihw, mla_stream_t stream);
int mla_conv1_bwd(const float* x, const float* w, const float* bias, const float* d_pooled, int64_t n, float* workspace,
                  float* dw, float* db, mla_stream_t stream);

int mla_conv_repack_dgrad_bf16(const float* w_oihw, int64_t cout, int64_t cin, void* out_bf16, mla_stream_t stream);
int mla_maxpool2x2_bf16(const void* a, void* out, int64_t n, int H, int W, int C, mla_stream_t stream);
int64_t mla_relu_pool_bwd_bf16_workspace_bytes(void);
int mla_relu_pool_bwd_bf16(const void* a, int a_dtype, const void* d_out, int d_dtype, void* dz, int64_t n, int H, int W,
                           int C, int pool, void* workspace, float* db, mla_stream_t stream);
int mla_conv_wgrad_bf16(const void* dz, const void* a_in, int64_t n, int H, int W, int cin, int cout, float* workspace,
                        int64_t workspace_floats, float* dw_oihw, mla_stream_t stream);
int mla_conv3x3_train_codes(const void* in, const void* w_packed, const float* bias, void* out_codes_u8, void* out_pooled, int64_t n,
                            int H, int W, int cin, int cout, int dtype, mla_stream_t stream);
int mla_pool_bwd_codes_bf16(const void* codes_u8, const void* d_pooled_bf16, void* dz_bf16, int64_t n, int H, int W, int C, void* workspace,
                            float* db, mla_stream_t stream);
int mla_conv1_bwd_bf16(const float* x, const float* w, const float* bias, const void* d_pooled_bf16, int64_t n, float* workspace,
                       float* dw, float* db, mla_stream_t stream);
int64_t mla_conv1_bwd_workspace_floats(void);
int mla_conv1_dgrad(const float* x, const float* w, const float* bias, const void* d_pooled, int d_dtype, int64_t n, float* dx,
                    mla_stream_t stream);
int mla_transpose_bf16(const void* in, int64_t ld_in, void* out, int64_t ld_out, int64_t rows, int64_t cols, mla_stream_t stream);
int mla_col_sum_bf16(const void* x, int64_t ldx, int64_t rows, int64_t cols, void* workspace, float* out, mla_stream_t stream);

int mla_adam_step(float* p, const float* g, float* m, float* v, int64_t n, float lr, float beta1, float beta2,
                  float eps, int64_t step, mla_stream_t stream);
int mla_adam_prepare(float* scal2_dev, float lr, float beta1, float beta2, int64_t step, mla_stream_t stream);
int mla_adam_step_dev(float* p, const float* g, float* m, float* v, int64_t n, float beta1, float beta2, float eps,
                      const float* scal2_dev, mla_stream_t stream);
int mla_counter_add(int64_t* counter_dev, int64_t delta, mla_stream_t stream);

int64_t mla_resample_length(int64_t n_in, double sr_in, double sr_out);
int mla_resample(const float* x, int64_t n_in, double sr_in, double sr_out, const double* win, const double* delta, int nwin,
                 int num_table, float* y, int64_t n_out, mla_stream_t stream);

int64_t mla_clips_lds_bytes(const double* host_rates, int64_t clips, double sr_out, int nwin, int num_table);
int mla_clips_prepare(const void* packed, int pcm_dtype, int64_t packed_elems, int64_t clips, const int64_t* offsets,
                      const int64_t* frames, const int32_t* channels, const double* rates, const int32_t* table_index,
                      const int64_t* host_offsets, const int64_t* host_frames, const int32_t* host_channels,
                      const double* host_rates, const int32_t* host_table_index, double sr_out, int64_t samples_num,
                      const double* tables, int64_t n_tables, int nwin, int num_table, float* out, mla_stream_t stream);
int mla_clips_prepare_raw(const void* packed, int64_t packed_bytes, int64_t clips, const int64_t* offsets, const int64_t* frames,
                          const int32_t* channels, const double* rates, const int32_t* table_index, const int32_t* formats,
                          const int64_t* host_offsets, const int64_t* host_frames, const int32_t* host_channels,
                          const double* host_rates, const int32_t* host_table_index, const int32_t* host_formats, double sr_out,
                          int64_t samples_num, const double* tables, int64_t n_tables, int nwin, int num_table, float* out,
                          mla_stream_t stream);


int         mla_comm_unique_id(void* id_host_128);
int         mla_comm_init_rank(void** comm_out, int nranks, const void* id_host_128, int rank);
int         mla_comm_destroy(void* comm);
int         mla_comm_count(void* comm, int* count);
const char* mla_comm_library_origin(void);

int mla_allreduce_flat(void* buf, int64_t count, int dtype, void* comm, mla_stream_t stream);

int mla_dropout_mask(uint8_t* mask, int64_t n, uint64_t seed, uint64_t stream_id, uint64_t offset, float p_drop,
                     mla_stream_t stream);
int mla_dropout_mask_dev(uint8_t* mask, int64_t n, uint64_t seed, uint64_t stream_base, const int64_t* counter_dev,
                         uint64_t offset, float p_drop, mla_stream_t stream);


int mla_rn_repack(const float* w_oihw, int64_t cout, int64_t cin, int64_t ks, void* out, int dtype, mla_stream_t stream);

int mla_rn_stem(const float* x, int64_t n, int64_t H, int64_t W, int single, const float* w, const float* scale, const float* shift, int relu,
                void* out, int dtype, mla_stream_t stream);

int mla_rn_conv(const void* in, int64_t n, int64_t H, int64_t W, int64_t cin, const void* w_packed, int64_t cout, int64_t ks,
                int64_t stride, const float* scale, const float* shift, const void* residual, int relu, void* out, int dtype,
                mla_stream_t stream);

int64_t mla_rn_bn_workspace_bytes(int64_t channels);
int mla_rn_bn_stats(const void* x, int64_t rows, int64_t channels, int dtype, void* workspace, const float* gamma,
                    const float* beta, float eps, float momentum, float* running_mean, float* running_var, float* mean,
                    float* var_biased, float* scale, float* shift, mla_stream_t stream);
int mla_rn_bn_sums(const void* x, int64_t rows, int64_t channels, int dtype, void* workspace, double* sums, mla_stream_t stream);
int mla_rn_bn_finish(const double* sums, int64_t channels, const float* gamma, const float* beta, float eps, float momentum,
                     float* running_mean, float* running_var, float* mean, float* var_biased, float* scale, float* shift,
                     mla_stream_t stream);
int mla_rn_bn_eval_coeffs(const float* gamma, const float* beta, const float* running_mean, const float* running_var,
                          float eps, int64_t channels, float* scale, float* shift, mla_stream_t stream);
int mla_rn_bn_apply(const void* x, int64_t rows, int64_t channels, const float* scale, const float* shift, const void* residual,
                    int relu, void* out, int dtype, mla_stream_t stream);

int mla_rn_maxpool(const void* in, int64_t n, int64_t H, int64_t W, int64_t channels, void* out, int dtype, mla_stream_t stream);
int mla_rn_avgpool(const void* in, int64_t n, int64_t hw, int64_t channels, float* out, int dtype, mla_stream_t stream);


int mla_rn_repack_dgrad(const float* w_oihw, int64_t cout, int64_t cin, int64_t ks, void* out, int dtype, mla_stream_t stream);
int mla_rn_conv_dgrad(const void* dy, int64_t n, int64_t Ho, int64_t Wo, int64_t cout, const void* w_dgrad, int64_t cin, int64_t ks,
                      int64_t stride, int64_t H, int64_t W, const void* residual, void* dx, int dtype, mla_stream_t stream);
int64_t mla_rn_conv_wgrad_workspace_floats(int64_t n, int64_t Ho, int64_t Wo, int64_t cin, int64_t cout, int64_t ks, int dtype);
int mla_rn_conv_wgrad(const void* x, const void* dy, int64_t n, int64_t H, int64_t W, int64_t cin, int64_t cout, int64_t ks,
                      int64_t stride, float* workspace, int64_t workspace_floats, float* dw_oihw, int dtype, mla_stream_t stream);
int64_t mla_rn_stem_wgrad_workspace_floats(int64_t n);
int mla_rn_stem_wgrad(const float* x, int64_t n, int single, const void* dy, float* workspace, int64_t workspace_floats, float* dw,
                      int dtype, mla_stream_t stream);
int64_t mla_rn_bn_bwd_workspace_bytes(int64_t channels);
int mla_rn_bn_bwd(const void* x, const void* dy, const void* y, int64_t rows, int64_t channels, const float* mean, const float* var_biased,
                  const float* gamma, float eps, void* workspace, float* dgamma, float* dbeta, void* dx, void* dres, int dtype,
                  mla_stream_t stream);
int mla_rn_bn_bwd_sums(const void* x, const void* dy, const void* y, int64_t rows, int64_t channels, const float* mean,
                       const float* var_biased, float eps, void* workspace, double* sums, float* dgamma, float* dbeta, int dtype,
                       mla_stream_t stream);
int mla_rn_bn_bwd_apply(const void* x, const void* dy, const void* y, int64_t rows, int64_t channels, const float* mean,
                        const float* var_biased, const float* gamma, float eps, const double* sums, void* workspace, void* dx, void* dres,
                        int dtype, mla_stream_t stream);
int mla_rn_maxpool_bwd(const void* in, const void* dy, int64_t n, int64_t H, int64_t W, int64_t channels, void* dx, int dtype,
                       mla_stream_t stream);
int mla_rn_avgpool_bwd(const float* d, int64_t n, int64_t hw, int64_t channels, void* dx, int dtype, mla_stream_t stream);


int mla_rn_act_bwd(const void* dy, const void* y, const float* scale, int64_t rows, int64_t channels, void* dpre, void* dres, int dtype,
                   mla_stream_t stream);
int mla_rn_stem_dgrad(const void* dy, int64_t n, const void* y, const float* scale, const float* w, int single, float* dx, int dtype,
                      mla_stream_t stream);

#ifdef __cplusplus
}
#endif
#endif
```

Before: 864,700 clips/s.

## Fuse BatchNorm epilogues into head GEMMs and fuse fcv with attention pooling

```diff
diff --git a/audio-classification-using-a-deep-cnn-combined-with-multi-level-attention_amd/_lib.py b/audio-classification-using-a-deep-cnn-combined-with-multi-level-attention_amd/_lib.py
--- a/audio-classification-using-a-deep-cnn-combined-with-multi-level-attention_amd/_lib.py
+++ b/audio-classification-using-a-deep-cnn-combined-with-multi-level-attention_amd/_lib.py
@@ -83,6 +83,11 @@
         L.mla_vggish_conv1.argtypes = [vp, ci, i64, vp, vp, vp, ci, vp]
         L.mla_vggish_conv.argtypes = [ci, vp, vp, vp, vp, i64, ci, vp]
         L.mla_linear.argtypes = [vp, i64, vp, i64, vp, vp, i64, i64, i64, i64, ci, ci, ci, vp]
+        L.mla_linear_bn.argtypes = [vp, i64, vp, i64, vp, vp, i64, i64, i64, i64, ci, vp, vp, vp, vp, cf, ci, vp, i64, vp, vp, vp, vp, vp]
+        L.mla_fcv_pool_lds_bytes.restype = i64
+        L.mla_fcv_pool_lds_bytes.argtypes = [i64, i64]
+        L.mla_fcv_pool.argtypes = ([vp, i64, vp, i64, vp, i64, ci, ci, i64] + [vp] * 8 + [cf, vp, i64, vp, i64, ci, vp, i64, vp] + [vp] * 4 +
+                                   [vp, i64, vp])
         L.mla_linear_small.argtypes = [vp, i64, vp, i64, vp, vp, i64, i64, i64, i64, vp]
         L.mla_linear_narrow.argtypes = [vp, i64, vp, i64, vp, vp, i64, i64, i64, i64, vp]
         L.mla_linear_splitk.argtypes = [vp, i64, vp, i64, vp, vp, i64, i64, i64, i64, ci, ci, vp, i64, vp]
diff --git a/audio-classification-using-a-deep-cnn-combined-with-multi-level-attention_amd/csrc/bn_affine.h b/audio-classification-using-a-deep-cnn-combined-with-multi-level-attention_amd/csrc/bn_affine.h
--- /dev/null
+++ b/audio-classification-using-a-deep-cnn-combined-with-multi-level-attention_amd/csrc/bn_affine.h
@@ -0,0 +1,26 @@
+#ifndef MLA_BN_AFFINE_H
+#define MLA_BN_AFFINE_H
+
+#include <hip/hip_runtime.h>
+
+#include "nanprop.h"
+
+namespace mla {
+
+__device__ __forceinline__ float sigmoidf(float v) { return 1.f / (1.f + __expf(-v)); }
+
+__device__ __forceinline__ float bn_inv_std(float var, float eps) { return 1.0f / sqrtf(var + eps); }
+
+__device__ __forceinline__ float bn_affine(float x, float mean, float inv_std, float gamma, float beta) {
+    return fmaf((x - mean) * inv_std, gamma, beta);
+}
+
+__device__ __forceinline__ float bn_act(float v, int act) {
+    if (act == 1) return nan_relu(v);
+    if (act == 2) return sigmoidf(v);
+    return v;
+}
+
+}
+
+#endif
diff --git a/audio-classification-using-a-deep-cnn-combined-with-multi-level-attention_amd/csrc/gemm.hip b/audio-classification-using-a-deep-cnn-combined-with-multi-level-attention_amd/csrc/gemm.hip
--- a/audio-classification-using-a-deep-cnn-combined-with-multi-level-attention_amd/csrc/gemm.hip
+++ b/audio-classification-using-a-deep-cnn-combined-with-multi-level-attention_amd/csrc/gemm.hip
@@ -1,5 +1,6 @@
 #include <type_traits>
 
+#include "bn_affine.h"
 #include "common.h"
 #include "mma_core.h"
 
@@ -36,12 +37,21 @@
 #else
 #define MLA_GEMM_KW(s) (s)
 #endif
-template <typename T, typename TO, int MS, int NS, bool RELU, bool DMA = false>
+struct RowAffine {
+    const float *mean, *var, *gamma, *beta;
+    const float *mean2, *var2, *gamma2, *beta2;
+    float* out2;
+    int64_t ldo2;
+    float eps;
+    int period, act;
+};
+
+template <typename T, typename TO, int MS, int NS, bool RELU, bool DMA = false, bool AFF = false>
 __global__ __launch_bounds__(kThreads, 2) void gemm_kernel(const T* __restrict__ A, int64_t lda,
                                                             const T* __restrict__ W, int64_t ldw,
                                                             const float* __restrict__ bias, TO* __restrict__ out,
                                                             int64_t ldo, int M, int N, int K, float* __restrict__ partial,
-                                                            int seg, int osplit) {
+                                                            int seg, int osplit, RowAffine aff) {
     constexpr int PER = Elem<T>::kPerChunk, KC = Elem<T>::kPerRow;
     constexpr int kMS = MS, kBM = 2 * MS * 16;
     constexpr int BN = 4 * NS * 16;
@@ -123,6 +133,15 @@
     const int per_split = (all_stages + int(gridDim.z) - 1) / int(gridDim.z);
     const int s_begin = int(blockIdx.z) * per_split;
     const int stages = (s_begin + per_split < all_stages ? s_begin + per_split : all_stages);
+    if constexpr (AFF) {
+        f32x4* coef = reinterpret_cast<f32x4*>(smem + 2 * (A_BYTES + B_BYTES));
+        if (t < kBM) {
+            const int ch = (m0 + t) % aff.period;
+            coef[2 * t] = f32x4{aff.mean[ch], mla::bn_inv_std(aff.var[ch], aff.eps), aff.gamma[ch], aff.beta[ch]};
+            if (aff.out2)
+                coef[2 * t + 1] = f32x4{aff.mean2[ch], mla::bn_inv_std(aff.var2[ch], aff.eps), aff.gamma2[ch], aff.beta2[ch]};
+        }
+    }
     if (DMA) {
         dma(s_begin, s_begin & 1);
         asm volatile("s_waitcnt vmcnt(0)" ::: "memory");
@@ -233,6 +252,32 @@
         }
         return;
     }
+    if constexpr (AFF) {
+        static_assert(std::is_same<TO, float>::value && !RELU, "the BatchNorm epilogue is float32, its activation comes after the affine");
+        const f32x4* coef = reinterpret_cast<const f32x4*>(smem + 2 * (A_BYTES + B_BYTES));
+        float b[NS];
+        _Pragma("unroll") for (int j = 0; j < NS; ++j) {
+            const int n = n0 + (wn * NS + j) * 16 + r;
+            b[j] = bias && n < N ? bias[n] : 0.f;
+        }
+        _Pragma("unroll") for (int i = 0; i < kMS; ++i) {
+            _Pragma("unroll") for (int e = 0; e < 4; ++e) {
+                const int row = (wm * kMS + i) * 16 + 4 * q + e, m = m0 + row;
+                if (m >= M) continue;
+                const f32x4 c = coef[2 * row];
+                f32x4 c2 = f32x4{0.f, 0.f, 0.f, 0.f};
+                if (aff.out2) c2 = coef[2 * row + 1];
+                _Pragma("unroll") for (int j = 0; j < NS; ++j) {
+                    const int n = n0 + (wn * NS + j) * 16 + r;
+                    if (n >= N) continue;
+                    const float y = mla::bn_act(mla::bn_affine(acc[i][j][e] + b[j], c.x, c.y, c.z, c.w), aff.act);
+                    out[size_t(m) * ldo + n] = y;
+                    if (aff.out2) aff.out2[size_t(m) * aff.ldo2 + n] = mla::bn_affine(y, c2.x, c2.y, c2.z, c2.w);
+                }
+            }
+        }
+        return;
+    }
     _Pragma("unroll") for (int j = 0; j < NS; ++j) {
         const int n = n0 + (wn * NS + j) * 16 + r;
         if (n >= N) continue;
@@ -402,7 +447,7 @@
     MLA_HIP_OK(hipFuncSetAttribute(reinterpret_cast<const void*>(kern), hipFuncAttributeMaxDynamicSharedMemorySize, lds));
     const dim3 grid{unsigned((M + kBM - 1) / kBM), unsigned((N + BN - 1) / BN), unsigned(splits)};
     hipLaunchKernelGGL(kern, grid, dim3(kThreads), lds, s, static_cast<const T*>(a), lda, static_cast<const T*>(w), ldw,
-                       bias, static_cast<TO*>(out), ldo, int(M), int(N), int(K), splits > 1 ? partial : nullptr, seg, osplit);
+                       bias, static_cast<TO*>(out), ldo, int(M), int(N), int(K), splits > 1 ? partial : nullptr, seg, osplit, RowAffine{});
     MLA_LAUNCH_OK("gemm_kernel");
     if (splits > 1) {
         const int64_t total = M * N;
@@ -410,6 +455,23 @@
                            0, s, partial, splits, M, int(N), bias, int(RELU), static_cast<TO*>(out), ldo);
         MLA_LAUNCH_OK("splitk_reduce_kernel");
     }
+    return MLA_OK;
+}
+
+template <int MS>
+int launch_affine(const float* a, int64_t lda, const float* w, int64_t ldw, const float* bias, float* out, int64_t ldo,
+                  int64_t M, int64_t N, int64_t K, const RowAffine& aff, hipStream_t s) {
+    constexpr int NS = 2, kBM = 2 * MS * 16, BN = 4 * NS * 16;
+    constexpr int lds = 2 * (kBM + BN) * kRowBytes + kBM * 32;
+    MLA_REQUIRE(uint64_t(kBM) * uint64_t(lda) * 4 < (1ull << 31) && uint64_t(BN) * uint64_t(ldw) * 4 < (1ull << 31), MLA_E_SHAPE,
+                "GEMM row pitch too large for 32-bit buffer offsets (lda %lld, ldw %lld)", (long long)lda, (long long)ldw);
+    const bool use_dma = K % mma::Elem<float>::kPerRow == 0;
+    auto kern = use_dma ? gemm_kernel<float, float, MS, NS, false, true, true> : gemm_kernel<float, float, MS, NS, false, false, true>;
+    MLA_HIP_OK(hipFuncSetAttribute(reinterpret_cast<const void*>(kern), hipFuncAttributeMaxDynamicSharedMemorySize, lds));
+    const dim3 grid{unsigned((M + kBM - 1) / kBM), unsigned((N + BN - 1) / BN), 1u};
+    hipLaunchKernelGGL(kern, grid, dim3(kThreads), lds, s, a, lda, w, ldw, bias, out, ldo, int(M), int(N), int(K),
+                       static_cast<float*>(nullptr), 0, 0, aff);
+    MLA_LAUNCH_OK("gemm_kernel (BatchNorm epilogue)");
     return MLA_OK;
 }
 
@@ -573,6 +635,28 @@
     return dispatch<mma::bf16_t, mma::bf16_t>(a, lda, w, ldw, bias, out, ldo, M, N, K, relu != 0, s);
 }
 
+extern "C" int mla_linear_bn(const float* a, int64_t lda, const float* w, int64_t ldw, const float* bias, float* out, int64_t ldo,
+                             int64_t M, int64_t N, int64_t K, int period, const float* mean, const float* var, const float* gamma,
+                             const float* beta, float eps, int act, float* out2, int64_t ldo2, const float* mean2,
+                             const float* var2, const float* gamma2, const float* beta2, mla_stream_t stream) {
+    MLA_REQUIRE(M >= 0 && N > 0 && K > 0, MLA_E_ARG, "bad GEMM shape %lld x %lld x %lld", (long long)M, (long long)N, (long long)K);
+    MLA_REQUIRE(period >= 1 && act >= 0 && act <= 2, MLA_E_ARG, "linear_bn period %d act %d", period, act);
+    if (M == 0) return MLA_OK;
+    MLA_REQUIRE(a && w && out && mean && var && gamma && beta, MLA_E_ARG, "null GEMM operand");
+    MLA_REQUIRE(!out2 || (mean2 && var2 && gamma2 && beta2 && out2 != out && ldo2 >= N), MLA_E_ARG, "linear_bn: bad second output");
+    MLA_REQUIRE(K % 4 == 0 && lda % 4 == 0 && ldw % 4 == 0 && lda >= K && ldw >= K && ldo >= N, MLA_E_SHAPE,
+                "K / lda / ldw must be multiples of 4 elements (16-byte rows): K %lld lda %lld ldw %lld ldo %lld",
+                (long long)K, (long long)lda, (long long)ldw, (long long)ldo);
+    MLA_REQUIRE(mla::aligned(a, 16) && mla::aligned(w, 16), MLA_E_ARG, "GEMM operands must be 16-byte aligned");
+    MLA_REQUIRE(M < (1ll << 31) && N < (1ll << 31) && K < (1ll << 31), MLA_E_SHAPE, "GEMM dimension overflow");
+    const RowAffine aff{mean, var, gamma, beta, mean2, var2, gamma2, beta2, out2, ldo2, eps, period, act};
+    hipStream_t s = static_cast<hipStream_t>(stream);
+    int64_t m_tall;
+    if (tile_form<float>(M, N, K, mla::cu_count(), m_tall) == Tile::k64x128)
+        return launch_affine<2>(a, lda, w, ldw, bias, out, ldo, M, N, K, aff, s);
+    return launch_affine<4>(a, lda, w, ldw, bias, out, ldo, M, N, K, aff, s);
+}
+
 extern "C" int mla_linear_bf16x3(const void* a, int64_t lda, const void* w, int64_t ldw, const float* bias, void* out,
                                  int64_t ldo, int64_t M, int64_t N, int64_t K, int64_t seg, int out_dtype, int relu,
                                  mla_stream_t stream) {
diff --git a/audio-classification-using-a-deep-cnn-combined-with-multi-level-attention_amd/csrc/mla_head.hip b/audio-classification-using-a-deep-cnn-combined-with-multi-level-attention_amd/csrc/mla_head.hip
--- a/audio-classification-using-a-deep-cnn-combined-with-multi-level-attention_amd/csrc/mla_head.hip
+++ b/audio-classification-using-a-deep-cnn-combined-with-multi-level-attention_amd/csrc/mla_head.hip
@@ -1,6 +1,9 @@
+#include "bn_affine.h"
 #include "common.h"
 
 namespace {
+
+using mla::sigmoidf;
 
 constexpr int kStatBlocks = 512;
 constexpr int kMaxChannels = 64;
@@ -13,8 +16,6 @@
     _Pragma("unroll") for (int o = 32; o > 0; o >>= 1) v += __shfl_xor(v, o);
     return v;
 }
-
-__device__ __forceinline__ float sigmoidf(float v) { return 1.f / (1.f + __expf(-v)); }
 
 __device__ __forceinline__ float grad_through_act(float dy, float yout, int act, float drop_scale) {
     if (act == 1) return yout > 0.f ? dy * drop_scale : 0.f;
@@ -254,10 +255,7 @@
         const int64_t r = i / cols;
         const int c = int(i - r * cols);
         const int ch = MODE == 0 ? int(r % period) : c;
-        const float inv = 1.0f / sqrtf(var[ch] + eps);
-        float v = (x[r * ldx + c] - mean[ch]) * inv * gamma[ch] + beta[ch];
-        if (act == 1) v = mla::nan_relu(v);
-        else if (act == 2) v = sigmoidf(v);
+        float v = mla::bn_act(mla::bn_affine(x[r * ldx + c], mean[ch], mla::bn_inv_std(var[ch], eps), gamma[ch], beta[ch]), act);
         if (keep) v *= keep[i] ? drop_scale : 0.f;
         y[r * ldy + c] = v;
     }
@@ -296,6 +294,38 @@
 struct BnParams { const float *mean, *var, *gamma, *beta; };
 
 template <int KMAX>
+__device__ __forceinline__ void pool_slot(const float* row, bool live, int t, int K, const BnParams& nv, const BnParams& nf, float eps,
+                                          float (&att)[KMAX], float (&cla)[KMAX]) {
+    if (live) {
+        const float iv = mla::bn_inv_std(nv.var[t], eps), jf = mla::bn_inv_std(nf.var[t], eps);
+        float mx = -3.0e38f;
+        _Pragma("unroll") for (int k = 0; k < KMAX; ++k)
+            if (k < K) {
+                const float v = row[k];
+                att[k] = mla::bn_affine(v, nv.mean[t], iv, nv.gamma[t], nv.beta[t]);
+                cla[k] = sigmoidf(mla::bn_affine(v, nf.mean[t], jf, nf.gamma[t], nf.beta[t]));
+                mx = fmaxf(mx, att[k]);
+            }
+        float den = 0.f;
+        _Pragma("unroll") for (int k = 0; k < KMAX; ++k)
+            if (k < K) { att[k] = __expf(att[k] - mx); den += att[k]; }
+        const float inv = 1.0f / den;
+        _Pragma("unroll") for (int k = 0; k < KMAX; ++k)
+            if (k < K) att[k] *= inv;
+    } else {
+        _Pragma("unroll") for (int k = 0; k < KMAX; ++k) { att[k] = 0.f; cla[k] = 0.f; }
+    }
+}
+
+__device__ __forceinline__ float pool_class(float att, float cla, bool live) {
+    float s = att;
+    _Pragma("unroll") for (int o = 8; o > 0; o >>= 1) s += __shfl_xor(s, o, 16);
+    float num = live ? cla * (att / s) : 0.f;
+    _Pragma("unroll") for (int o = 8; o > 0; o >>= 1) num += __shfl_xor(num, o, 16);
+    return num;
+}
+
+template <int KMAX>
 __global__ __launch_bounds__(256) void attention_pool_kernel(const float* __restrict__ z, int64_t bags, int T, int K,
                                                              BnParams nv, BnParams nf, float eps, float* __restrict__ y,
                                                              int64_t ldy, float* __restrict__ att_out,
@@ -304,36 +334,17 @@
     const int64_t bag = int64_t(blockIdx.x) * 16 + (threadIdx.x >> 4);
     const bool live = bag < bags && t < T;
     float att[KMAX], cla[KMAX];
+    pool_slot<KMAX>(z + (bag * T + t) * K, live, t, K, nv, nf, eps, att, cla);
     if (live) {
-        const float* row = z + (bag * T + t) * K;
-        const float iv = 1.0f / sqrtf(nv.var[t] + eps), jf = 1.0f / sqrtf(nf.var[t] + eps);
-        float mx = -3.0e38f;
         _Pragma("unroll") for (int k = 0; k < KMAX; ++k)
             if (k < K) {
-                const float v = row[k];
-                att[k] = (v - nv.mean[t]) * iv * nv.gamma[t] + nv.beta[t];
-                cla[k] = sigmoidf((v - nf.mean[t]) * jf * nf.gamma[t] + nf.beta[t]);
-                mx = fmaxf(mx, att[k]);
-            }
-        float den = 0.f;
-        _Pragma("unroll") for (int k = 0; k < KMAX; ++k)
-            if (k < K) { att[k] = __expf(att[k] - mx); den += att[k]; }
-        const float inv = 1.0f / den;
-        _Pragma("unroll") for (int k = 0; k < KMAX; ++k)
-            if (k < K) {
-                att[k] *= inv;
                 if (att_out) att_out[(bag * T + t) * K + k] = att[k];
                 if (cla_out) cla_out[(bag * T + t) * K + k] = cla[k];
             }
-    } else {
-        _Pragma("unroll") for (int k = 0; k < KMAX; ++k) { att[k] = 0.f; cla[k] = 0.f; }
     }
     _Pragma("unroll") for (int k = 0; k < KMAX; ++k) {
         if (k < K) {
-            float s = att[k];
-            _Pragma("unroll") for (int o = 8; o > 0; o >>= 1) s += __shfl_xor(s, o, 16);
-            float num = live ? cla[k] * (att[k] / s) : 0.f;
-            _Pragma("unroll") for (int o = 8; o > 0; o >>= 1) num += __shfl_xor(num, o, 16);
+            const float num = pool_class(att[k], cla[k], live);
             if (t == 0 && bag < bags) y[bag * ldy + k] = num;
         }
     }
@@ -503,43 +514,105 @@
 typedef float f4 __attribute__((ext_vector_type(4)));
 
 template <int N>
+__device__ __forceinline__ void narrow_stage_weights(const float* __restrict__ w, int64_t ldw, int k4, float* sw, int threads) {
+    for (int i = threadIdx.x; i < k4 * N; i += threads) {
+        const int n = i % N, kk = i / N;
+        reinterpret_cast<f4*>(sw)[kk * N + n] = *reinterpret_cast<const f4*>(w + int64_t(n) * ldw + 4 * kk);
+    }
+}
+
+template <int N>
+__device__ __forceinline__ void narrow_row(const f4* row, const float* sw, int k4, int l, float (&acc)[N]) {
+    _Pragma("unroll") for (int n = 0; n < N; ++n) acc[n] = 0.f;
+    for (int kk = l; kk < k4; kk += 16) {
+        const f4 x = row[kk];
+        _Pragma("unroll") for (int n = 0; n < N; ++n) {
+            const f4 ww = reinterpret_cast<const f4*>(sw)[kk * N + n];
+            acc[n] = fmaf(x.x, ww.x, acc[n]);
+            acc[n] = fmaf(x.y, ww.y, acc[n]);
+            acc[n] = fmaf(x.z, ww.z, acc[n]);
+            acc[n] = fmaf(x.w, ww.w, acc[n]);
+        }
+    }
+    _Pragma("unroll") for (int n = 0; n < N; ++n) {
+        float v = acc[n];
+        v += __shfl_xor(v, 8, 16);
+        v += __shfl_xor(v, 4, 16);
+        v += __shfl_xor(v, 2, 16);
+        v += __shfl_xor(v, 1, 16);
+        acc[n] = v;
+    }
+}
+
+template <int N>
+__device__ __forceinline__ float narrow_pick(const float (&acc)[N], int l, const float* __restrict__ bias) {
+    float v = 0.f;
+    _Pragma("unroll") for (int n = 0; n < N; ++n) v = l == n ? acc[n] : v;
+    return v + (bias ? bias[l] : 0.f);
+}
+
+template <int N>
 __global__ __launch_bounds__(256) void linear_narrow_kernel(const float* __restrict__ a, int64_t lda, const float* __restrict__ w,
                                                             int64_t ldw, const float* __restrict__ bias, float* __restrict__ out,
                                                             int64_t ldo, int64_t M, int K) {
     extern __shared__ __attribute__((aligned(16))) float sw[];
     const int k4 = K / 4;
-    for (int i = threadIdx.x; i < k4 * N; i += 256) {
-        const int n = i % N, kk = i / N;
-        reinterpret_cast<f4*>(sw)[kk * N + n] = *reinterpret_cast<const f4*>(w + int64_t(n) * ldw + 4 * kk);
-    }
+    narrow_stage_weights<N>(w, ldw, k4, sw, 256);
     __syncthreads();
     const int l = threadIdx.x & 15, grp = threadIdx.x >> 4;
     for (int64_t m = int64_t(blockIdx.x) * 16 + grp; m < M; m += int64_t(gridDim.x) * 16) {
         float acc[N];
-        _Pragma("unroll") for (int n = 0; n < N; ++n) acc[n] = 0.f;
-        const f4* row = reinterpret_cast<const f4*>(a + m * lda);
-        for (int kk = l; kk < k4; kk += 16) {
-            const f4 x = row[kk];
-            _Pragma("unroll") for (int n = 0; n < N; ++n) {
-                const f4 ww = reinterpret_cast<const f4*>(sw)[kk * N + n];
-                acc[n] = fmaf(x.x, ww.x, acc[n]);
-                acc[n] = fmaf(x.y, ww.y, acc[n]);
-                acc[n] = fmaf(x.z, ww.z, acc[n]);
-                acc[n] = fmaf(x.w, ww.w, acc[n]);
+        narrow_row<N>(reinterpret_cast<const f4*>(a + m * lda), sw, k4, l, acc);
+        if (l < N) out[m * ldo + l] = narrow_pick<N>(acc, l, bias);
+    }
+}
+
+constexpr int kPoolBags = 4;
+constexpr int kPoolThreads = 256;
+
+struct HeadFinal {
+    const float* conc; int64_t ldc; int prev;
+    const float *w; int64_t ldw; const float* bias;
+    BnParams norm;
+    float* out; int64_t ldo;
+};
+
+template <int N>
+__global__ __launch_bounds__(kPoolThreads) void fcv_pool_kernel(const float* __restrict__ a, int64_t lda, const float* __restrict__ w,
+                                                       int64_t ldw, const float* __restrict__ bias, int64_t bags, int T, int K,
+                                                       BnParams nv, BnParams nf, float eps, float* __restrict__ y, int64_t ldy,
+                                                       HeadFinal fin) {
+    extern __shared__ __attribute__((aligned(16))) float sw[];
+    const int k4 = K / 4;
+    float* zs = sw + size_t(K) * N;
+    narrow_stage_weights<N>(w, ldw, k4, sw, kPoolThreads);
+    const int l = threadIdx.x & 15, grp = threadIdx.x >> 4;
+    for (int64_t bag0 = int64_t(blockIdx.x) * kPoolBags; bag0 < bags; bag0 += int64_t(gridDim.x) * kPoolBags) {
+        const int nb = bags - bag0 < kPoolBags ? int(bags - bag0) : kPoolBags;
+        __syncthreads();
+        for (int lr = grp; lr < nb * T; lr += kPoolThreads / 16) {
+            float acc[N];
+            narrow_row<N>(reinterpret_cast<const f4*>(a + (bag0 * T + lr) * lda), sw, k4, l, acc);
+            if (l < N) zs[lr * N + l] = narrow_pick<N>(acc, l, bias);
+        }
+        __syncthreads();
+        if (threadIdx.x >= 16 * kPoolBags) continue;
+        const int t = l, b = grp;
+        const int64_t bag = bag0 + b;
+        const bool live = b < nb && t < T;
+        float att[N], cla[N], yk[N];
+        pool_slot<N>(zs + (b * T + t) * N, live, t, N, nv, nf, eps, att, cla);
+        _Pragma("unroll") for (int k = 0; k < N; ++k) yk[k] = pool_class(att[k], cla[k], live);
+        if (!fin.out) {
+            if (t == 0 && b < nb) {
+                _Pragma("unroll") for (int k = 0; k < N; ++k) y[bag * ldy + k] = yk[k];
             }
-        }
-        _Pragma("unroll") for (int n = 0; n < N; ++n) {
-            float v = acc[n];
-            v += __shfl_xor(v, 8, 16);
-            v += __shfl_xor(v, 4, 16);
-            v += __shfl_xor(v, 2, 16);
-            v += __shfl_xor(v, 1, 16);
-            acc[n] = v;
-        }
-        if (l < N) {
-            float v = 0.f;
-            _Pragma("unroll") for (int n = 0; n < N; ++n) v = l == n ? acc[n] : v;
-            out[m * ldo + l] = v + (bias ? bias[l] : 0.f);
+        } else if (b < nb && t < N) {
+            float acc = fin.bias ? fin.bias[t] : 0.f;
+            for (int k = 0; k < fin.prev; ++k) acc = fmaf(fin.conc[bag * fin.ldc + k], fin.w[int64_t(t) * fin.ldw + k], acc);
+            _Pragma("unroll") for (int k = 0; k < N; ++k) acc = fmaf(yk[k], fin.w[int64_t(t) * fin.ldw + fin.prev + k], acc);
+            fin.out[bag * fin.ldo + t] = mla::bn_act(mla::bn_affine(acc, fin.norm.mean[t], mla::bn_inv_std(fin.norm.var[t], eps),
+                                                                    fin.norm.gamma[t], fin.norm.beta[t]), 2);
         }
     }
 }
@@ -812,6 +885,48 @@
     return MLA_OK;
 }
 
+extern "C" int64_t mla_fcv_pool_lds_bytes(int64_t classes, int64_t hidden) {
+    return (hidden * classes + 16 * kPoolBags * classes) * 4;
+}
+
+extern "C" int mla_fcv_pool(const float* h, int64_t ldh, const float* w, int64_t ldw, const float* bias, int64_t bags, int T,
+                            int classes, int64_t hidden, const float* v_mean, const float* v_var, const float* v_gamma,
+                            const float* v_beta, const float* f_mean, const float* f_var, const float* f_gamma, const float* f_beta,
+                            float eps, float* y, int64_t ldy, const float* conc, int64_t ldc, int prev, const float* fc_w,
+                            int64_t fc_ldw, const float* fc_bias, const float* n_mean, const float* n_var, const float* n_gamma,
+                            const float* n_beta, float* scores, int64_t ld_scores, mla_stream_t stream) {
+    const int64_t N = classes, K = hidden;
+    MLA_REQUIRE(h && w && v_mean && v_var && v_gamma && v_beta && f_mean && f_var && f_gamma && f_beta && ldh >= K && ldw >= K, MLA_E_ARG,
+                "bad fcv_pool arguments");
+    MLA_REQUIRE(T >= 1 && T <= 16 && N >= 1 && N <= 16 && K >= 4 && K % 4 == 0 && ldh % 4 == 0 && ldw % 4 == 0 &&
+                mla_fcv_pool_lds_bytes(N, K) <= 64 * 1024, MLA_E_SHAPE,
+                "fcv_pool: T, classes <= 16, hidden a multiple of 4 with 16-byte aligned rows (T %d, classes %lld, hidden %lld)", T,
+                (long long)N, (long long)K);
+    MLA_REQUIRE(mla::aligned(h, 16) && mla::aligned(w, 16), MLA_E_ARG, "fcv_pool operands must be 16-byte aligned");
+    MLA_REQUIRE(bags >= 0 && bags <= 0x7fffffff, MLA_E_ARG, "fcv_pool: %lld bags", (long long)bags);
+    if (scores)
+        MLA_REQUIRE(fc_w && n_mean && n_var && n_gamma && n_beta && prev >= 0 && prev + N <= 64 && fc_ldw >= prev + N && ld_scores >= N &&
+                    (prev == 0 || (conc && ldc >= prev)), MLA_E_ARG, "fcv_pool: bad final-layer arguments (prev %d)", prev);
+    else
+        MLA_REQUIRE(y && ldy >= N, MLA_E_ARG, "fcv_pool: no output");
+    if (bags == 0) return MLA_OK;
+    const BnParams nv{v_mean, v_var, v_gamma, v_beta}, nf{f_mean, f_var, f_gamma, f_beta};
+    const HeadFinal fin{conc, ldc, prev, fc_w, fc_ldw, fc_bias, BnParams{n_mean, n_var, n_gamma, n_beta}, scores, ld_scores};
+    const int64_t blocks = (bags + kPoolBags - 1) / kPoolBags;
+    const unsigned grid = unsigned(blocks < 2048 ? blocks : 2048);
+    const size_t lds = size_t(mla_fcv_pool_lds_bytes(N, K));
+    hipStream_t s = static_cast<hipStream_t>(stream);
+#define MLA_FCV_POOL_CASE(NN) \
+    if (N == NN) { hipLaunchKernelGGL(fcv_pool_kernel<NN>, dim3(grid), dim3(kPoolThreads), lds, s, h, ldh, w, ldw, bias, bags, T, int(K), nv, nf, eps, y, ldy, fin); }
+    MLA_FCV_POOL_CASE(1) else MLA_FCV_POOL_CASE(2) else MLA_FCV_POOL_CASE(3) else MLA_FCV_POOL_CASE(4) else MLA_FCV_POOL_CASE(5) else
+    MLA_FCV_POOL_CASE(6) else MLA_FCV_POOL_CASE(7) else MLA_FCV_POOL_CASE(8) else MLA_FCV_POOL_CASE(9) else MLA_FCV_POOL_CASE(10) else
+    MLA_FCV_POOL_CASE(11) else MLA_FCV_POOL_CASE(12) else MLA_FCV_POOL_CASE(13) else MLA_FCV_POOL_CASE(14) else MLA_FCV_POOL_CASE(15) else
+    MLA_FCV_POOL_CASE(16)
+#undef MLA_FCV_POOL_CASE
+    MLA_LAUNCH_OK("fcv_pool");
+    return MLA_OK;
+}
+
 extern "C" int mla_gather_bags(const float* emb, int64_t rows, int64_t ld, const int64_t* first_row, const int64_t* host_first_row,
                                int64_t windows, int T, int64_t M, float* out, mla_stream_t stream) {
     MLA_REQUIRE(rows >= 0 && windows >= 0 && T >= 1 && M >= 1 && ld >= M, MLA_E_ARG, "bad gather_bags sizes (rows %lld, windows %lld, T %d, M %lld, ld %lld)",
diff --git a/audio-classification-using-a-deep-cnn-combined-with-multi-level-attention_amd/mla_train.py b/audio-classification-using-a-deep-cnn-combined-with-multi-level-attention_amd/mla_train.py
--- a/audio-classification-using-a-deep-cnn-combined-with-multi-level-attention_amd/mla_train.py
+++ b/audio-classification-using-a-deep-cnn-combined-with-multi-level-attention_amd/mla_train.py
@@ -67,7 +67,50 @@
         ctx.tape.append(("att", am, level, rows, z, nv, nf, att, cla))
 
 
+def _eval_bn(bn):
+    return bn.running_mean, bn.running_var, bn.weight.detach(), bn.bias.detach()
+
+
+def mla_infer(mla, x):
+    B, T, K = x.shape[0], mla.slots, mla.classes
+    L = len(mla.model)
+    conc = torch.empty((B, L * K), dtype=torch.float32, device=x.device)
+    rows = x.detach().reshape(B * T, -1).float().contiguous()
+    h = ops.bn_apply(rows, 0, T, *_eval_bn(mla.embedded_mappings[0].norm0))
+    for lvl in range(L):
+        em, am = mla.embedded_mappings[lvl], mla.attention_modules[lvl]
+        nxt = _eval_bn(mla.embedded_mappings[lvl + 1].norm0) if lvl + 1 < L else None
+        h_next = None
+        for j in range(em.n_fc):
+            w, b, bn = em.fc[j].weight.detach(), em.fc[j].bias.detach(), _eval_bn(em.norms[j])
+            if h.shape[1] % 4:
+                h = ops.bn_apply(ops.linear_small(h, w.contiguous(), b.contiguous()), 0, T, *bn, act=1)
+            elif j == em.n_fc - 1 and nxt is not None:
+                h, h_next = ops.linear(h, w, b, bn=(T,) + bn + (1,), bn2=nxt)
+            else:
+                h = ops.linear(h, w, b, bn=(T,) + bn + (1,))
+        if nxt is not None and h_next is None:
+            h_next = ops.bn_apply(h, 0, T, *nxt)
+        fcv_w, fcv_b = am.fcv.weight.detach(), am.fcv.bias.detach()
+        nv, nf = _eval_bn(am.normv), _eval_bn(am.normf)
+        last = lvl == L - 1
+        y = conc[:, lvl * K:(lvl + 1) * K]
+        if ops.fcv_pool_ok(h, fcv_w, T, K):
+            if last and L * K <= 64:
+                return ops.fcv_pool(h, fcv_w, fcv_b, B, T, nv, nf,
+                                    final=(conc, (L - 1) * K, mla.fc.weight.detach(), mla.fc.bias.detach(), _eval_bn(mla.norm)))
+            ops.fcv_pool(h, fcv_w, fcv_b, B, T, nv, nf, y=y)
+        else:
+            ops.attention_pool(ops.linear(h, fcv_w, fcv_b), B, T, K, nv, nf, y)
+        h = h_next
+    z = ops.linear_small(conc, mla.fc.weight.detach(), mla.fc.bias.detach())
+    return ops.bn_apply(z, 1, 0, *_eval_bn(mla.norm), act=2)
+
+
 def mla_forward(mla, x, ctx=None):
+    if ((ctx is None or ctx.tape is None) and mla.classes <= 16 and mla.slots <= 16
+            and not any(m.training for m in mla.modules())):
+        return mla_infer(mla, x)
     ctx = ctx or Ctx()
     ctx.train = mla.training
     B, K = x.shape[0], mla.classes
diff --git a/audio-classification-using-a-deep-cnn-combined-with-multi-level-attention_amd/ops.py b/audio-classification-using-a-deep-cnn-combined-with-multi-level-attention_amd/ops.py
--- a/audio-classification-using-a-deep-cnn-combined-with-multi-level-attention_amd/ops.py
+++ b/audio-classification-using-a-deep-cnn-combined-with-multi-level-attention_amd/ops.py
@@ -164,7 +164,7 @@
 KSPLIT = 8
 
 
-def linear(a, w, b, relu=False, out_dtype=None, out=None, split_k=False):
+def linear(a, w, b, relu=False, out_dtype=None, out=None, split_k=False, bn=None, bn2=None):
     _chk(a); _chk(w, a.dtype)
     M, K = a.shape
     N = w.shape[0]
@@ -174,6 +174,16 @@
         out = torch.empty((M, N), dtype=out_dtype, device=a.device)
     else:
         assert out.is_contiguous() and out.numel() == M * N and out.dtype == out_dtype
+    if bn is not None:
+        assert a.dtype == torch.float32 and out_dtype == torch.float32 and not relu and not split_k
+        period, mean, var, gamma, beta, act = bn
+        out2 = torch.empty((M, N), dtype=torch.float32, device=a.device) if bn2 is not None else None
+        m2, v2, g2, b2 = bn2 if bn2 is not None else (None,) * 4
+        _lib.check(_timed("linear_%dx%d" % (K, N), _lib.lib().mla_linear_bn, _p(a), a.stride(0), _p(w), w.stride(0), _p(b), _p(out), N,
+                          M, N, K, period, _p(mean), _p(var), _p(gamma), _p(beta), BN_EPS, act, _p(out2), N, _p(m2), _p(v2), _p(g2),
+                          _p(b2), _lib.stream_ptr()))
+        return out if bn2 is None else (out, out2)
+    assert bn2 is None
     if (N <= 16 and a.dtype == torch.float32 and out_dtype == torch.float32 and not relu and not split_k and K % 4 == 0
             and K * N * 4 <= 65536 and a.stride(0) % 4 == 0 and w.stride(0) % 4 == 0
             and a.data_ptr() % 16 == 0 and w.data_ptr() % 16 == 0):
@@ -252,6 +262,34 @@
     _lib.check(_lib.lib().mla_attention_pool(_p(z), bags, T, K, _p(nv[0]), _p(nv[1]), _p(nv[2]), _p(nv[3]), _p(nf[0]), _p(nf[1]),
                                              _p(nf[2]), _p(nf[3]), BN_EPS, _p(y), y.stride(0), _p(att), _p(cla), _lib.stream_ptr()))
     return att, cla
+
+
+def fcv_pool_ok(h, w, T, K):
+    H = h.shape[1]
+    return (T <= 16 and K <= 16 and H % 4 == 0 and h.dtype == torch.float32 and h.stride(0) % 4 == 0 and w.stride(0) % 4 == 0
+            and h.data_ptr() % 16 == 0 and w.data_ptr() % 16 == 0 and _lib.lib().mla_fcv_pool_lds_bytes(K, H) <= 65536)
+
+
+def fcv_pool(h, w, b, bags, T, nv, nf, y=None, final=None):
+    _chk(h, torch.float32); _chk(w, torch.float32)
+    K, H = w.shape
+    assert h.shape == (bags * T, H)
+    scores = None
+    conc = fc_w = fc_b = None
+    prev, norm = 0, (None,) * 4
+    if final is not None:
+        conc, prev, fc_w, fc_b, norm = final
+        _chk(fc_w, torch.float32)
+        assert fc_w.shape == (K, prev + K) and conc.dtype == torch.float32 and conc.stride(1) == 1 and conc.shape[1] >= prev
+        scores = torch.empty((bags, K), dtype=torch.float32, device=h.device)
+    else:
+        assert y.dtype == torch.float32 and y.stride(1) == 1 and y.shape == (bags, K)
+    _lib.check(_timed("fcv_pool_%dx%d" % (H, K), _lib.lib().mla_fcv_pool, _p(h), h.stride(0), _p(w), w.stride(0), _p(b), bags, T, K, H,
+                      _p(nv[0]), _p(nv[1]), _p(nv[2]), _p(nv[3]), _p(nf[0]), _p(nf[1]), _p(nf[2]), _p(nf[3]), BN_EPS,
+                      _p(y) if final is None else None, y.stride(0) if final is None else 0, _p(conc),
+                      conc.stride(0) if conc is not None else 0, prev, _p(fc_w), fc_w.stride(0) if fc_w is not None else 0, _p(fc_b),
+                      _p(norm[0]), _p(norm[1]), _p(norm[2]), _p(norm[3]), _p(scores), K, _lib.stream_ptr()))
+    return scores
 
 
 
diff --git a/include/mla_hip.h b/include/mla_hip.h
--- a/include/mla_hip.h
+++ b/include/mla_hip.h
@@ -110,6 +110,10 @@
 int mla_linear(const void* a, int64_t lda, const void* w, int64_t ldw, const float* bias, void* out,
                int64_t ldo, int64_t M, int64_t N, int64_t K, int dtype, int out_dtype, int relu,
                mla_stream_t stream);
+int mla_linear_bn(const float* a, int64_t lda, const float* w, int64_t ldw, const float* bias, float* out, int64_t ldo,
+                  int64_t M, int64_t N, int64_t K, int period, const float* mean, const float* var, const float* gamma,
+                  const float* beta, float eps, int act, float* out2, int64_t ldo2, const float* mean2, const float* var2,
+                  const float* gamma2, const float* beta2, mla_stream_t stream);
 int mla_linear_ksplit(const void* a, int64_t lda, const void* w, int64_t ldw, const float* bias, void* out, int64_t ldo,
                       int64_t M, int64_t N, int64_t K, int dtype, int out_dtype, int relu, int splits, float* workspace,
                       int64_t workspace_floats, mla_stream_t stream);
@@ -135,6 +139,14 @@
                        const float* v_gamma, const float* v_beta, const float* f_mean, const float* f_var,
                        const float* f_gamma, const float* f_beta, float eps, float* y, int64_t ldy,
                        float* att_out, float* cla_out, mla_stream_t stream);
+
+int64_t mla_fcv_pool_lds_bytes(int64_t classes, int64_t hidden);
+int mla_fcv_pool(const float* h, int64_t ldh, const float* w, int64_t ldw, const float* bias, int64_t bags, int T, int classes,
+                 int64_t hidden, const float* v_mean, const float* v_var, const float* v_gamma, const float* v_beta,
+                 const float* f_mean, const float* f_var, const float* f_gamma, const float* f_beta, float eps, float* y,
+                 int64_t ldy, const float* conc, int64_t ldc, int prev, const float* fc_w, int64_t fc_ldw, const float* fc_bias,
+                 const float* n_mean, const float* n_var, const float* n_gamma, const float* n_beta, float* scores,
+                 int64_t ld_scores, mla_stream_t stream);
 
 int mla_gather_bags(const float* emb, int64_t rows, int64_t ld, const int64_t* first_row, const int64_t* host_first_row,
                     int64_t windows, int T, int64_t M, float* out, mla_stream_t stream);
```

Measured after the change: 870,000 clips/s, median of 6. No clear change (+0.6%).
